# r4dl/StopThePop-Rasterization

Hardware: AMD Instinct MI355X
Metric: fwd+bwd frames/sec at 1920×1080, 1M Gaussians; PSNR vs reference (higher is better)
Workload: dtype f32

## Files before the change

include/stp_raster.h:

```cpp
#ifndef STP_RASTER_H_INCLUDED
#define STP_RASTER_H_INCLUDED

#include <stddef.h>
#include <stdint.h>

#ifdef __cplusplus
extern "C" {
#endif

#define STP_ABI_VERSION 7
#define STP_GRAD_RECORD_FLOATS 16
#define STP_GRAD_RECORD_USED 9
#define STP_GRAD_RECORD_ABS 9
#define STP_GRAD_RECORD_STATS 11
#define STP_GRAD_RECORD_INVDEPTH 14

typedef struct StpSettings {
    int32_t sort_mode;
    int32_t sort_order;
    int32_t queue_tile_4x4;
    int32_t queue_tile_2x2;
    int32_t queue_per_pixel;
    int32_t rect_bounding;
    int32_t tight_opacity_bounding;
    int32_t tile_based_culling;
    int32_t hierarchical_4x4_culling;
    int32_t load_balancing;
    int32_t proper_ewa_scaling;
    int32_t tile_y0;
    int32_t tile_y1;
    int32_t record_blend_log;
    int32_t debug_visualization;
} StpSettings;

#define STP_DEBUG_DISABLED 0
#define STP_DEBUG_DEPTH 1

typedef enum StpStatus {
    STP_OK = 0,
    STP_ERR_INVALID_ARGUMENT = -1,
    STP_ERR_NEEDS_SCALE_ROTATION = -2,
    STP_ERR_QUEUE_SIZE = -3,
    STP_ERR_SORT_MODE = -4,
    STP_ERR_NO_BACKWARD = -5,
    STP_ERR_HIP = -6,
    STP_ERR_ALLOC = -7,
    STP_ERR_PREFILTERED = -8
} StpStatus;

typedef void* (*stp_alloc_fn)(void* user, size_t bytes);

int stp_forward(stp_alloc_fn geometry_alloc, void* geometry_user,
                stp_alloc_fn binning_alloc, void* binning_user,
                stp_alloc_fn image_alloc, void* image_user,
                int P, int D, int M,
                const float* background, int width, int height,
                const StpSettings* settings,
                const float* means3D, const float* shs, const float* colors_precomp,
                const float* opacities, const float* scales, float scale_modifier,
                const float* rotations, const float* cov3D_precomp,
                const float* viewmatrix, const float* projmatrix, const float* inv_viewprojmatrix,
                const float* cam_pos, float tan_fovx, float tan_fovy, int prefiltered,
                float* out_color, int* radii, int debug, void* stream);

void stp_set_forward_split(int tile_row, void* event);

int stp_backward(int P, int D, int M, int R,
                 const float* background, int width, int height,
                 const StpSettings* settings,
                 const float* means3D, const float* shs, const float* opacities, const float* colors_precomp,
                 const float* scales, float scale_modifier, const float* rotations, const float* cov3D_precomp,
                 const float* viewmatrix, const float* projmatrix, const float* inv_viewprojmatrix,
                 const float* cam_pos, float tan_fovx, float tan_fovy,
                 const float* pixel_colors, const int* radii,
                 char* geom_buffer, char* binning_buffer, char* image_buffer,
                 const float* dL_dpix,
                 float* dL_dmean2D , float* grad_records , float* dL_dopacity ,
                 float* dL_dcolor , float* dL_dmean3D , float* dL_dcov3D ,
                 float* dL_dsh , float* dL_dscale , float* dL_drot ,
                 int debug, void* stream);

int stp_backward_phases(int phases, int P, int D, int M, int R,
                        const float* background, int width, int height,
                        const StpSettings* settings,
                        const float* means3D, const float* shs, const float* opacities, const float* colors_precomp,
                        const float* scales, float scale_modifier, const float* rotations, const float* cov3D_precomp,
                        const float* viewmatrix, const float* projmatrix, const float* inv_viewprojmatrix,
                        const float* cam_pos, float tan_fovx, float tan_fovy,
                        const float* pixel_colors, const int* radii,
                        char* geom_buffer, char* binning_buffer, char* image_buffer,
                        const float* dL_dpix,
                        float* dL_dmean2D, float* grad_records, float* dL_dopacity, float* dL_dcolor,
                        float* dL_dmean3D, float* dL_dcov3D, float* dL_dsh, float* dL_dscale, float* dL_drot,
                        int debug, void* stream);

size_t stp_camera_grad_workspace_bytes(int P);
void stp_set_backward_camera_grads(float* dL_dviewmatrix, float* dL_dprojmatrix, float* dL_dcampos, void* workspace, size_t workspace_bytes);

void stp_set_backward_absgrad(float* dL_dmean2D_abs );

void stp_set_backward_blend_stats(float* blend_stats );

void stp_set_forward_background(const float* bg_image , float* out_alpha );
void stp_set_backward_background(const float* bg_image , const float* dL_dalpha ,
                                 float* dL_dbackground );

void stp_set_forward_invdepth(float* out_invdepth );
void stp_set_backward_invdepth(const float* invdepth , const float* dL_dinvdepth );

void stp_set_forward_split_sh(const float* dc );
void stp_set_backward_split_sh(const float* dc , float* dL_ddc );

void stp_set_forward_sh_stash(int enable);

void stp_set_forward_raw_params(int mask);
void stp_set_backward_raw_params(int mask);
int stp_activate_params(int P, const float* scaling, const float* rotation, const float* opacity, float* scales, float* rotations,
                        float* opacities, void* stream);

int stp_mark_visible(int P, const float* means3D, const float* viewmatrix, const float* projmatrix,
                     uint8_t* present, void* stream);

typedef struct { float* param; const float* grad; float* exp_avg; float* exp_avg_sq; long long numel; float lr, eps; } StpAdamTensor;
int stp_sparse_adam(int n_tensors, const StpAdamTensor* tensors, int N, const void* visible, int visible_kind ,
                    float beta1, float beta2, void* stream);

int stp_mcmc_relocation(int n, const float* opacity_old, const float* scale_old, const void* N, int n_kind , int n_max,
                        float* opacity_new, float* scale_new, void* stream);
int stp_mcmc_add_noise(int P, float* xyz, const float* scales, const float* rotations, const float* opacities, const float* noise,
                       float noise_scale, float k, float x0, int raw, void* stream);

typedef struct { float grad_threshold, split_size, min_opacity, max_screen_size, max_world_size, split_shrink; int32_t raw, prune_big; } StpDensifyRule;
typedef struct { const float *param, *exp_avg, *exp_avg_sq; float *param_out, *exp_avg_out, *exp_avg_sq_out; int32_t row; int32_t role; } StpDensifyTensor;
int stp_densify_stats(int P, float* grad_accum, float* denom, float* max_radii2D , const float* grad2d, int grad_stride ,
                      const void* visible, int visible_kind, void* stream);
int stp_densify_plan(int P, const float* grad_accum, const float* denom, const float* scaling, const float* opacity,
                     const float* max_radii2D , const StpDensifyRule* rule, uint8_t* plan, void* stream);
size_t stp_densify_scratch_bytes(int P);
int stp_densify_scan(int P, const uint8_t* plan, void* scratch, size_t scratch_bytes, uint32_t* offsets , int64_t counts[3] , void* stream);
int stp_densify_apply(int P, const uint8_t* plan, const uint32_t* offsets, const int64_t counts[3], int n_tensors, const StpDensifyTensor* tensors,
                      const float* noise , float split_shrink, int raw, void* stream);

#define STP_KNN_BOX 256
size_t stp_knn_scratch_bytes(int P);
int stp_knn_mean_dist2(int P, const float* points , void* scratch, size_t scratch_bytes, float* mean_dist2 , void* stream);

#define STP_PHOTOMETRIC_TILE_W 64
#define STP_PHOTOMETRIC_TILE_H 16
size_t stp_photometric_workspace_floats(int planes, int H, int W);
int stp_photometric_forward(int planes, int H, int W, const float* image, const float* target,
                            float* out2 , float* maps ,
                            float* workspace, void* stream);
int stp_photometric_backward(int planes, int H, int W, const float* image, const float* target, const float* maps,
                             const float* dL_dout2 , float* dL_dimage, void* stream);

size_t stp_geometry_buffer_size(int P, const StpSettings* settings);
size_t stp_geometry_buffer_size_stash(int P, const StpSettings* settings);
size_t stp_binning_buffer_size(int R);
size_t stp_image_buffer_size(int width, int height);
size_t stp_blend_log_bytes(int width, int height);
size_t stp_blend_log_bytes_rows(int width, int height, int tile_y0, int tile_y1);
int stp_blend_log_depth(const void* image_buffer);
void stp_forget_buffer(const void* buffer);
size_t stp_blend_log_bytes_depth(int width, int height, int tile_y0, int tile_y1, int depth);

int stp_geometry_layout(int P, const StpSettings* settings, const char* name, size_t* offset, size_t* count);
int stp_binning_layout(int R, const char* name, size_t* offset, size_t* count);
int stp_binning_layout_count(const void* binning_buffer, int R);
void stp_reset_size_guesses(void);
void stp_set_run_ahead(int mode);
int stp_get_run_ahead(void);
int stp_image_layout(int width, int height, const char* name, size_t* offset, size_t* count);
int stp_image_layout_rows(int width, int height, int tile_y0, int tile_y1, const char* name, size_t* offset, size_t* count);
int stp_image_layout_depth(int width, int height, int tile_y0, int tile_y1, int log_depth, const char* name, size_t* offset, size_t* count);

void stp_timing_enable(int enabled);
int stp_timing_read(float* ms6);
int stp_timing_history(float* ms6, int capacity);
int stp_timing_history_host(float* ms6, int capacity);
size_t stp_timing_text(char* buf, size_t size);

int stp_hbm_probe(int kind, void* dst, const void* src, size_t bytes, int blocks, void* stream);

const char* stp_last_error(void);
int stp_abi_version(void);

#ifdef __cplusplus
}
#endif
#endif
```

stopthepop-rasterization_amd/csrc/host/stp_bind_raster.h:

```cpp
#pragma once

#include <tuple>

#include "stp_scratch_pool.h"
#include "stp_tensor_checks.h"

namespace {
StpSettings settings_from_dict(const py::dict& d, bool record_log)
{
    StpSettings s{};
    const py::dict ss = d["sort_settings"].cast<py::dict>(), cs = d["culling_settings"].cast<py::dict>(), q = ss["queue_sizes"].cast<py::dict>();
    s.sort_mode = ss["sort_mode"].cast<int>();
    s.sort_order = ss["sort_order"].cast<int>();
    s.queue_tile_4x4 = q["tile_4x4"].cast<int>();
    s.queue_tile_2x2 = q["tile_2x2"].cast<int>();
    s.queue_per_pixel = q["per_pixel"].cast<int>();
    s.rect_bounding = cs["rect_bounding"].cast<bool>();
    s.tight_opacity_bounding = cs["tight_opacity_bounding"].cast<bool>();
    s.tile_based_culling = cs["tile_based_culling"].cast<bool>();
    s.hierarchical_4x4_culling = cs["hierarchical_4x4_culling"].cast<bool>();
    s.load_balancing = d["load_balancing"].cast<bool>();
    s.proper_ewa_scaling = d["proper_ewa_scaling"].cast<bool>();
    if (setting_present(d, "_tile_rows")) {
        const py::tuple tr = py::tuple(d["_tile_rows"]);
        s.tile_y0 = tr[0].cast<int>();
        s.tile_y1 = tr[1].cast<int>();
    }
    s.record_blend_log = record_log ? 1 : 0;
    return s;
}

struct FrameInputs { torch::Tensor bg, m3, sh, col, op, sc, ro, c3, vm, pm, inv, cam; };
FrameInputs prep_frame(const torch::Device& dev, const torch::Tensor& background, const torch::Tensor& means3D, const torch::Tensor& sh,
                       const torch::Tensor& colors, const torch::Tensor& opacity, const torch::Tensor& scales, const torch::Tensor& rotations,
                       const torch::Tensor& cov3D_precomp, const torch::Tensor& viewmatrix, const torch::Tensor& projmatrix,
                       const torch::Tensor& inv_viewprojmatrix, const torch::Tensor& campos)
{
    return {prep(background, dev), prep(means3D, dev), prep(sh, dev), prep(colors, dev), prep(opacity, dev), prep(scales, dev), prep(rotations, dev),
            prep(cov3D_precomp, dev), prep(viewmatrix, dev), prep(projmatrix, dev), prep(inv_viewprojmatrix, dev), prep(campos, dev)};
}

bool per_pixel_background(const torch::Tensor& bg, int H, int W)
{
    return bg.defined() && bg.dim() == 3 && bg.size(0) == 3 && bg.size(1) == H && bg.size(2) == W;
}

int split_sh_total(const torch::Tensor& dc, const torch::Tensor& sh, const torch::Tensor& means3D)
{
    const int64_t P = means3D.size(0);
    if (!((dc.dim() == 3 && dc.size(1) == 1 && dc.size(2) == 3) || (dc.dim() == 2 && dc.size(1) == 3)))
        throw std::runtime_error("dc must have dimensions (num_points, 1, 3) or (num_points, 3)");
    if (dc.size(0) != P) throw std::runtime_error("dc must have one row per Gaussian: " + std::to_string(dc.size(0)) + " rows for " + std::to_string(P) + " points");
    if (dc.scalar_type() != torch::kFloat32) throw std::runtime_error("dc must be a float32 tensor");
    if (dc.device() != means3D.device()) throw std::runtime_error("dc must be on the device of means3D");
    if (sh.numel() == 0) return 1;
    if (!(sh.dim() == 3 && sh.size(0) == P && sh.size(2) == 3))
        throw std::runtime_error("with dc, shs is the rest of the coefficients and must have dimensions (num_points, M - 1, 3)");
    if (sh.scalar_type() != torch::kFloat32 || sh.device() != means3D.device()) throw std::runtime_error("with dc, shs must be a float32 tensor on the device of means3D");
    return (int)sh.size(1) + 1;
}

std::tuple<int, torch::Tensor, torch::Tensor, torch::Tensor, torch::Tensor, torch::Tensor, torch::Tensor, torch::Tensor>
rasterize_gaussians(const torch::Tensor& background, const torch::Tensor& means3D, const torch::Tensor& colors, const torch::Tensor& opacity,
                    const torch::Tensor& scales, const torch::Tensor& rotations, const float scale_modifier, const torch::Tensor& cov3D_precomp,
                    const torch::Tensor& viewmatrix, const torch::Tensor& projmatrix, const torch::Tensor& inv_viewprojmatrix, const float tan_fovx,
                    const float tan_fovy, const int image_height, const int image_width, const torch::Tensor& sh, const int degree,
                    const torch::Tensor& campos, const bool prefiltered, const py::dict& settings, const bool render_depth, const bool debug,
                    const bool record_log, const bool alpha, const bool invdepth, const c10::optional<torch::Tensor>& dc, const int raw)
{
    need_library();
    if (raw != 0) require(g_api.set_forward_raw_params, "raw");
    TORCH_CHECK(means3D.dim() == 2 && means3D.size(1) == 3, "means3D must have dimensions (num_points, 3)");
    TORCH_CHECK(means3D.is_cuda(), GPU_ONLY);
    const bool split = dc.has_value() && dc->defined() && colors.numel() == 0;
    if (split) require(g_api.set_forward_split_sh, "dc");
    const int M_split = split ? split_sh_total(*dc, sh, means3D) : 0;
    const torch::Device dev = means3D.device();
    const int P = (int)means3D.size(0), H = image_height, W = image_width;
    const auto fopt = means3D.options().dtype(torch::kFloat32), iopt = means3D.options().dtype(torch::kInt32), bopt = means3D.options().dtype(torch::kByte);
    const bool zero = P == 0 || setting_present(settings, "_tile_rows");
    torch::Tensor out_color = zero ? torch::zeros({3, H, W}, fopt) : torch::empty({3, H, W}, fopt);
    torch::Tensor radii = zero ? torch::zeros({P}, iopt) : torch::empty({P}, iopt);
    const bool bg_pixels = per_pixel_background(background, H, W);
    if (alpha || bg_pixels) require(g_api.set_forward_background, "alpha / background");
    torch::Tensor out_alpha;
    if (alpha) out_alpha = zero ? torch::zeros({1, H, W}, fopt) : torch::empty({1, H, W}, fopt);
    if (invdepth) {
        require(g_api.set_forward_invdepth, "invdepth");
        if (render_depth) throw std::runtime_error("the inverse-depth output is not available with render_depth (the debug depth visualisation)");
    }
    torch::Tensor out_invdepth;
    if (invdepth) out_invdepth = zero ? torch::zeros({1, H, W}, fopt) : torch::empty({1, H, W}, fopt);
    const bool sh_stash = (setting_flag(settings, "_record_blend_log") || setting_flag(settings, "_sh_stash")) && !setting_flag(settings, "_no_sh_stash") &&
                          !render_depth && g_api.set_forward_sh_stash != nullptr;
    Resizer geom{torch::empty({0}, bopt), false, false, 0}, binning{torch::empty({0}, bopt), true, false, 1}, img{torch::empty({0}, bopt), true, false, 2};
    int rendered = 0;
    if (P != 0) {
        const int M = split ? M_split : sh.numel() != 0 ? (int)sh.size(1) : 0;
        StpSettings s = settings_from_dict(settings, record_log);
        if (render_depth) {
            s.debug_visualization = STP_DEBUG_DEPTH;
            s.record_blend_log = 0;
        }
        const FrameInputs in = prep_frame(dev, background, means3D, sh, colors, opacity, scales, rotations, cov3D_precomp, viewmatrix, projmatrix,
                                          inv_viewprojmatrix, campos);
        torch::Tensor dc_;
        if (split) dc_ = prep(*dc, dev);
        const c10::hip::HIPGuard guard(dev.index());
        void* const stream = current_stream(dev);
        int rc;
        {
            py::gil_scoped_release nogil;
            if (alpha || bg_pixels)
                g_api.set_forward_background(bg_pixels ? fptr(in.bg) : nullptr, alpha ? out_alpha.data_ptr<float>() : nullptr);
            if (invdepth) g_api.set_forward_invdepth(out_invdepth.data_ptr<float>());
            if (split) g_api.set_forward_split_sh(dc_.data_ptr<float>());
            if (sh_stash) g_api.set_forward_sh_stash(1);
            if (raw != 0) g_api.set_forward_raw_params(raw);
            rc = g_api.forward(&Resizer::call, &geom, &Resizer::call, &binning, &Resizer::call, &img, P, degree, M, fptr(in.bg), W, H, &s, fptr(in.m3),
                               fptr(in.sh), fptr(in.col), fptr(in.op), fptr(in.sc), scale_modifier, fptr(in.ro), fptr(in.c3), fptr(in.vm), fptr(in.pm),
                               fptr(in.inv), fptr(in.cam), tan_fovx, tan_fovy, prefiltered ? 1 : 0, out_color.data_ptr<float>(), radii.data_ptr<int>(),
                               debug ? 1 : 0, stream);
        }
        rendered = checked(rc);
        remember_storage(geom.t);
        remember_storage(binning.t);
        remember_storage(img.t);
    }
    return std::make_tuple(rendered, out_color, radii, geom.t, binning.t, img.t, out_alpha, out_invdepth);
}

std::vector<torch::Tensor>
rasterize_gaussians_backward(const torch::Tensor& background, const torch::Tensor& means3D, const torch::Tensor& radii, const torch::Tensor& opacities,
                             const torch::Tensor& colors, const torch::Tensor& scales, const torch::Tensor& rotations, const float scale_modifier,
                             const torch::Tensor& cov3D_precomp, const torch::Tensor& viewmatrix, const torch::Tensor& projmatrix,
                             const torch::Tensor& inv_viewprojmatrix, const float tan_fovx, const float tan_fovy, const torch::Tensor& pixel_colors,
                             const torch::Tensor& dL_dout_color, const torch::Tensor& sh, const int degree, const torch::Tensor& campos,
                             const torch::Tensor& geomBuffer, const int R, const torch::Tensor& binningBuffer, const torch::Tensor& imageBuffer,
                             const py::dict& settings, const bool debug, const bool record_log, const int phases, const c10::optional<torch::Tensor>& partial,
                             const c10::optional<std::vector<torch::Tensor>>& outputs, const bool camera_grads, const bool absgrad, const bool blend_stats,
                             const c10::optional<torch::Tensor>& dL_dalpha, const bool bg_grad,
                             const c10::optional<torch::Tensor>& dL_dinvdepth, const c10::optional<torch::Tensor>& invdepth,
                             const c10::optional<torch::Tensor>& dc, const int raw_mask)
{
    need_library();
    TORCH_CHECK(means3D.is_cuda(), GPU_ONLY);
    const int raw = (phases & 2) ? raw_mask : 0;
    if (raw != 0) require(g_api.set_backward_raw_params, "raw");
    const bool split = dc.has_value() && dc->defined() && colors.numel() == 0 && (phases & 2);
    if (split) require(g_api.set_backward_split_sh, "dc");
    const int M_split = split ? split_sh_total(*dc, sh, means3D) : 0;
    if (camera_grads) {
        require(g_api.set_backward_camera_grads, "camera gradients");
        require(g_api.camera_grad_workspace_bytes, "camera gradients");
        TORCH_CHECK(phases & 2, "camera gradients come from the per-Gaussian half (phases bit 1)");
    }
    if (absgrad) {
        require(g_api.set_backward_absgrad, "absgrad");
        TORCH_CHECK((phases & 3) == 3, "absgrad needs both halves of the backward in one call (phases bits 0 and 1)");
    }
    if (blend_stats) {
        require(g_api.set_backward_blend_stats, "blend_stats");
        TORCH_CHECK((phases & 3) == 3, "blend_stats needs both halves of the backward in one call (phases bits 0 and 1)");
    }
    const torch::Device dev = means3D.device();
    const int P = (int)means3D.size(0);
    const int H = (int)dL_dout_color.size(1), W = (int)dL_dout_color.size(2);
    const bool bg_pixels = per_pixel_background(background, H, W);
    const bool have_dalpha = dL_dalpha.has_value() && dL_dalpha->defined();
    if (bg_pixels || have_dalpha || bg_grad) {
        require(g_api.set_backward_background, "alpha / background");
        TORCH_CHECK(phases & 1, "alpha gradient / per-pixel background / background gradient belong to the render half (phases bit 0)");
        TORCH_CHECK(!have_dalpha || dL_dalpha->numel() == (int64_t)H * W, "dL_dalpha must have H * W elements");
    }
    const bool have_dinv = dL_dinvdepth.has_value() && dL_dinvdepth->defined();
    if (have_dinv) {
        require(g_api.set_backward_invdepth, "invdepth");
        TORCH_CHECK((phases & 3) == 3, "the inverse-depth gradient needs both halves of the backward in one call (phases bits 0 and 1)");
        TORCH_CHECK(invdepth.has_value() && invdepth->defined(), "dL_dinvdepth needs the forward's invdepth");
        TORCH_CHECK(dL_dinvdepth->numel() == (int64_t)H * W && invdepth->numel() == (int64_t)H * W, "dL_dinvdepth and invdepth must have H * W elements");
    }
    const int M = split ? M_split : sh.numel() != 0 ? (int)sh.size(1) : 0;
    const auto fopt = means3D.options().dtype(torch::kFloat32);
    const int rec_floats = (phases & 4) ? STP_GRAD_RECORD_USED : STP_GRAD_RECORD_FLOATS;
    const torch::Tensor records = partial.has_value() ? *partial : torch::zeros({P, rec_floats}, fopt);
    TORCH_CHECK(records.dim() == 2 && records.size(0) == P && records.size(1) == rec_floats && records.scalar_type() == torch::kFloat32 &&
                    records.is_contiguous(), "partial must be a contiguous float32 (P,", rec_floats, ") tensor");
    torch::Tensor dL_dmeans2D, dL_dcolors, dL_dopacity, dL_dmeans3D, dL_dcov3D, dL_dsh, dL_dscales, dL_drotations, dL_ddc;
    if ((phases & 2) && outputs.has_value()) {
        TORCH_CHECK(outputs->size() == (split ? 9u : 8u), "outputs: the eight gradient tensors of an earlier chunk (and its dL_ddc behind them with dc)");
        if (split) {
            dL_ddc = (*outputs)[8];
            TORCH_CHECK(dL_ddc.scalar_type() == torch::kFloat32 && dL_ddc.is_contiguous() && dL_ddc.numel() == (int64_t)P * 3 &&
                            (*outputs)[5].is_contiguous() && (*outputs)[5].numel() == (int64_t)P * (M - 1) * 3,
                        "outputs: dL_dsh must be a contiguous (P,M-1,3) and dL_ddc a contiguous (P,3) float32 tensor with dc");
        }
        dL_dmeans2D = (*outputs)[0]; dL_dcolors = (*outputs)[1]; dL_dopacity = (*outputs)[2]; dL_dmeans3D = (*outputs)[3];
        dL_dcov3D = (*outputs)[4]; dL_dsh = (*outputs)[5]; dL_dscales = (*outputs)[6]; dL_drotations = (*outputs)[7];
    } else if (phases & 2) {
        const bool have_scales = scales.numel() != 0, may_omit = g_api.set_forward_sh_stash != nullptr;
        const bool no_dcolors = may_omit && setting_flag(settings, "_no_grad_colors") && colors.numel() == 0;
        const bool no_dcov3D = may_omit && setting_flag(settings, "_no_grad_cov3D") && cov3D_precomp.numel() == 0;
        dL_dmeans2D = torch::empty({P, 3}, fopt); if (!no_dcolors) dL_dcolors = torch::empty({P, 3}, fopt); dL_dopacity = torch::empty({P, 1}, fopt);
        dL_dmeans3D = torch::empty({P, 3}, fopt); if (!no_dcov3D) dL_dcov3D = torch::empty({P, 6}, fopt); dL_dsh = torch::empty({P, split ? M - 1 : M, 3}, fopt);
        if (split) dL_ddc = torch::empty({P, 3}, fopt);
        dL_dscales = have_scales ? torch::empty({P, 3}, fopt) : torch::zeros({P, 3}, fopt);
        dL_drotations = have_scales ? torch::empty({P, 4}, fopt) : torch::zeros({P, 4}, fopt);
    }
    const StpSettings s = settings_from_dict(settings, record_log);
    torch::Tensor dL_dview, dL_dproj, dL_dcam, cam_ws;
    if (camera_grads) {
        dL_dview = torch::empty(viewmatrix.sizes(), fopt); dL_dproj = torch::empty(projmatrix.sizes(), fopt); dL_dcam = torch::empty(campos.sizes(), fopt);
        TORCH_CHECK(dL_dview.numel() == 16 && dL_dproj.numel() == 16 && dL_dcam.numel() == 3, "camera gradients: viewmatrix and projmatrix must have 16 elements, campos 3");
        cam_ws = torch::empty({(int64_t)g_api.camera_grad_workspace_bytes(P)}, means3D.options().dtype(torch::kByte));
    }
    torch::Tensor dL_dmeans2D_abs, stats;
    if (absgrad) dL_dmeans2D_abs = torch::empty({P, 3}, fopt);
    if (blend_stats) stats = torch::empty({P, 3}, fopt);
    torch::Tensor dL_dbg, dal_, bgpix_;
    if (bg_grad) {
        const std::vector<int64_t> shape = bg_pixels ? std::vector<int64_t>{3, H, W} : std::vector<int64_t>{3};
        dL_dbg = (P == 0 || (bg_pixels && setting_present(settings, "_tile_rows"))) ? torch::zeros(shape, fopt) : torch::empty(shape, fopt);
    }
    if (have_dalpha) dal_ = prep(*dL_dalpha, dev);
    if (bg_pixels) bgpix_ = prep(background, dev);
    torch::Tensor dinv_, inv_out_;
    if (have_dinv) { dinv_ = prep(*dL_dinvdepth, dev); inv_out_ = prep(*invdepth, dev); }
    torch::Tensor dc_;
    if (split && P != 0) dc_ = prep(*dc, dev);
    auto make_requests = [&] {
        if ((bg_pixels || have_dalpha || bg_grad) && P != 0)
            g_api.set_backward_background(bg_pixels ? bgpix_.data_ptr<float>() : nullptr, have_dalpha ? dal_.data_ptr<float>() : nullptr,
                                          bg_grad ? dL_dbg.data_ptr<float>() : nullptr);
        if (have_dinv && P != 0) g_api.set_backward_invdepth(inv_out_.data_ptr<float>(), dinv_.data_ptr<float>());
        if (split && P != 0) g_api.set_backward_split_sh(dc_.data_ptr<float>(), dL_ddc.data_ptr<float>());
        if (raw != 0 && P != 0) g_api.set_backward_raw_params(raw);
        if (blend_stats && P != 0) g_api.set_backward_blend_stats(stats.data_ptr<float>());
        if (absgrad && P != 0) g_api.set_backward_absgrad(dL_dmeans2D_abs.data_ptr<float>());
        if (camera_grads) g_api.set_backward_camera_grads(dL_dview.data_ptr<float>(), dL_dproj.data_ptr<float>(), dL_dcam.data_ptr<float>(), cam_ws.data_ptr(), (size_t)cam_ws.numel());
    };
    if (P == 0 && camera_grads) {
        const c10::hip::HIPGuard guard(dev.index());
        void* const stream = current_stream(dev);
        make_requests();
        checked(g_api.backward_phases(phases, 0, degree, M, R, nullptr, W, H, &s, nullptr, nullptr, nullptr, nullptr, nullptr, scale_modifier, nullptr,
                                      nullptr, nullptr, nullptr, nullptr, nullptr, tan_fovx, tan_fovy, nullptr, nullptr, nullptr, nullptr, nullptr,
                                      nullptr, nullptr, nullptr, nullptr, nullptr, nullptr, nullptr, nullptr, nullptr, nullptr, debug ? 1 : 0, stream));
    }
    if (P != 0) {
        const FrameInputs in = prep_frame(dev, background, means3D, sh, colors, opacities, scales, rotations, cov3D_precomp, viewmatrix, projmatrix,
                                          inv_viewprojmatrix, campos);
        const torch::Tensor pix_ = prep(pixel_colors, dev), dl_ = prep(dL_dout_color, dev);
        const torch::Tensor radii_ = radii.contiguous();
        auto optf = [](const torch::Tensor& t) -> float* { return t.defined() && t.numel() != 0 ? t.data_ptr<float>() : nullptr; };
        auto optb = [](const torch::Tensor& t) -> char* { return t.defined() && t.numel() != 0 ? reinterpret_cast<char*>(t.data_ptr()) : nullptr; };
        const c10::hip::HIPGuard guard(dev.index());
        void* const stream = current_stream(dev);
        forget_unless_same_storage(geomBuffer);
        forget_unless_same_storage(binningBuffer);
        forget_unless_same_storage(imageBuffer);
        make_requests();
        checked(g_api.backward_phases(phases, P, degree, M, R, fptr(in.bg), W, H, &s, fptr(in.m3), fptr(in.sh), fptr(in.op), fptr(in.col), fptr(in.sc),
                                      scale_modifier, fptr(in.ro), fptr(in.c3), fptr(in.vm), fptr(in.pm), fptr(in.inv), fptr(in.cam), tan_fovx, tan_fovy,
                                      fptr(pix_), radii_.numel() ? radii_.data_ptr<int>() : nullptr, optb(geomBuffer), optb(binningBuffer),
                                      optb(imageBuffer), fptr(dl_), optf(dL_dmeans2D), records.data_ptr<float>(), optf(dL_dopacity), optf(dL_dcolors),
                                      optf(dL_dmeans3D), optf(dL_dcov3D), optf(dL_dsh), optf(dL_dscales), optf(dL_drotations), debug ? 1 : 0, stream));
    }
    if ((phases & 3) == 1) { if (bg_grad) return {records, dL_dbg}; return {records}; }
    std::vector<torch::Tensor> result{dL_dmeans2D, dL_dcolors, dL_dopacity, dL_dmeans3D, dL_dcov3D, dL_dsh, dL_dscales, dL_drotations};
    if (camera_grads) result.insert(result.end(), {dL_dview, dL_dproj, dL_dcam});
    if (absgrad) result.push_back(dL_dmeans2D_abs);
    if (blend_stats) result.push_back(stats);
    if (bg_grad) result.push_back(dL_dbg);
    if (split) result.push_back(dL_ddc);
    return result;
}

torch::Tensor mark_visible(const torch::Tensor& means3D, const torch::Tensor& viewmatrix, const torch::Tensor& projmatrix)
{
    need_library();
    TORCH_CHECK(means3D.is_cuda(), GPU_ONLY);
    const torch::Device dev = means3D.device();
    const int P = (int)means3D.size(0);
    torch::Tensor present = torch::zeros({P}, means3D.options().dtype(torch::kBool));
    if (P != 0) {
        const torch::Tensor m3_ = prep(means3D, dev), vm_ = prep(viewmatrix, dev), pm_ = prep(projmatrix, dev);
        const c10::hip::HIPGuard guard(dev.index());
        checked(g_api.mark_visible(P, fptr(m3_), fptr(vm_), fptr(pm_), reinterpret_cast<uint8_t*>(present.data_ptr()), current_stream(dev)));
    }
    return present;
}
}
```

stopthepop-rasterization_amd/csrc/host/stp_exports.h:

```cpp
#pragma once

#include <dlfcn.h>

#include <cstddef>
#include <cstring>
#include <stdexcept>
#include <string>

#include "../../../include/stp_raster.h"

#define STP_CORE "the C ABI of include/stp_raster.h"
#define STP_EXPORTS(X)                                                                     \
    X(forward, true, STP_CORE)                                                             \
    X(backward_phases, true, STP_CORE)                                                     \
    X(mark_visible, true, STP_CORE)                                                        \
    X(last_error, true, STP_CORE)                                                          \
    X(abi_version, true, STP_CORE)                                                         \
    X(forget_buffer, true, STP_CORE)                                                       \
    X(set_forward_split, true, STP_CORE)                                                   \
    X(camera_grad_workspace_bytes, false, "camera gradients")                              \
    X(set_backward_camera_grads, false, "camera gradients")                                \
    X(set_backward_absgrad, false, "absgrad")                                              \
    X(set_backward_blend_stats, false, "blend statistics")                                 \
    X(set_forward_background, false, "the alpha output and per-pixel background")          \
    X(set_backward_background, false, "the alpha output and per-pixel background")         \
    X(set_forward_invdepth, false, "the inverse-depth output")                             \
    X(set_backward_invdepth, false, "the inverse-depth output")                            \
    X(set_forward_split_sh, false, "split SH inputs")                                      \
    X(set_backward_split_sh, false, "split SH inputs")                                     \
    X(set_forward_raw_params, false, "raw parameter inputs")                               \
    X(set_backward_raw_params, false, "raw parameter inputs")                              \
    X(activate_params, false, "raw parameter inputs")                                      \
    X(set_forward_sh_stash, false, "the SH stash")  \
    X(sparse_adam, false, "the sparse Adam step")                                          \
    X(mcmc_relocation, false, "the 3DGS-MCMC kernels")                                     \
    X(mcmc_add_noise, false, "the 3DGS-MCMC kernels")                                      \
    X(knn_scratch_bytes, false, "the nearest-neighbour kernels")                           \
    X(knn_mean_dist2, false, "the nearest-neighbour kernels")                              \
    X(densify_stats, false, "the densification kernels")                                   \
    X(densify_plan, false, "the densification kernels")                                    \
    X(densify_scratch_bytes, false, "the densification kernels")                           \
    X(densify_scan, false, "the densification kernels")                                    \
    X(densify_apply, false, "the densification kernels")                                   \
    X(photometric_workspace_floats, false, "the photometric loss")                         \
    X(photometric_forward, false, "the photometric loss")                                  \
    X(photometric_backward, false, "the photometric loss")

namespace {
struct Api {
    void* handle = nullptr;
#define X(name, required, feature) decltype(&stp_##name) name = nullptr;
    STP_EXPORTS(X)
#undef X
} g_api;

struct Export { const char* symbol; bool required; const char* feature; size_t slot; };
const Export g_exports[] = {
#define X(name, required, feature) {"stp_" #name, required, feature, offsetof(Api, name)},
    STP_EXPORTS(X)
#undef X
};

[[noreturn]] void raise_missing(const Export& e, const std::string& who)
{
    throw std::runtime_error(who + ": the loaded libstp_raster.so does not export " + e.symbol + " (a library built before " + e.feature + "): rebuild it");
}

template <class F> void require(const F& fn, const char* who)
{
    if (fn) return;
    const size_t slot = reinterpret_cast<const char*>(&fn) - reinterpret_cast<const char*>(&g_api);
    for (const Export& e : g_exports)
        if (e.slot == slot) raise_missing(e, who);
    throw std::logic_error(std::string(who) + ": require() takes a member of g_api");
}

int load_library(const std::string& path)
{
    void* h = dlopen(path.c_str(), RTLD_NOW | RTLD_LOCAL);
    if (!h) throw std::runtime_error(std::string("cannot load ") + path + ": " + dlerror());
    Api a;
    a.handle = h;
    for (const Export& e : g_exports) {
        void* fn = dlsym(h, e.symbol);
        if (!fn && e.required) raise_missing(e, path);
        std::memcpy(reinterpret_cast<char*>(&a) + e.slot, &fn, sizeof fn);
    }
    if (a.abi_version() != STP_ABI_VERSION) throw std::runtime_error(path + ": ABI version mismatch");
    g_api = a;
    return a.abi_version();
}

void need_library()
{
    if (!g_api.forward) throw std::runtime_error("libstp_raster.so is not loaded (diff_gaussian_rasterization._C._load() does it); there is no CPU fallback");
}

[[noreturn]] void raise_last(int rc)
{
    const char* msg = g_api.last_error();
    throw std::runtime_error((msg && *msg) ? std::string(msg) : "libstp_raster error " + std::to_string(rc));
}
}
```

stopthepop-rasterization_amd/csrc/stp_api.hip:

```cpp
#include "stp_internal.h"

#include <mutex>
#include <string>
#include <utility>

namespace stp {

static thread_local std::string g_last_error;

int fail(int code, const std::string& msg) { g_last_error = msg; return code; }
int fail_hip(hipError_t e, const char* what) { return fail(STP_ERR_HIP, std::string(what) + ": " + hipGetErrorString(e)); }

int check_settings(const StpSettings& s, bool backward)
{
    if (s.sort_mode < MODE_GLOBAL || s.sort_mode > MODE_HIER) return fail(STP_ERR_SORT_MODE, "invalid sort mode");
    if (s.sort_order < ORDER_Z || s.sort_order > ORDER_PTD_MAX) return fail(STP_ERR_SORT_MODE, "invalid sort order");
    if (backward && s.sort_mode == MODE_FULL) return fail(STP_ERR_NO_BACKWARD, "Backward not supported for full per-pixel sort");
    if (s.sort_mode == MODE_HIER) {
        const int h = s.queue_per_pixel, m = s.queue_tile_2x2;
        if (!(m == 8 || m == 12 || m == 20)) return fail(STP_ERR_QUEUE_SIZE, "Not supported mid queue size");
        const bool head_ok = backward ? (h == 4 || h == 8 || h == 12 || h == 16) : (h == 4 || h == 8 || h == 16);
        if (!head_ok) return fail(STP_ERR_QUEUE_SIZE, "Not supported head queue size");
    }
    return 0;
}

void fill_frame(FrameParams& f, int P, int D, int M, const float* background, int width, int height, const StpSettings& s,
                const float* means3D, const float* shs, const float* colors_precomp, const float* opacities,
                const float* scales, float scale_modifier, const float* rotations, const float* cov3D_precomp,
                const float* viewmatrix, const float* projmatrix, const float* inv_viewprojmatrix, const float* cam_pos,
                float tan_fovx, float tan_fovy, int prefiltered)
{
    f.P = P; f.D = D; f.M = M; f.W = width; f.H = height;
    f.gx = (width + TILE - 1) / TILE; f.gy = (height + TILE - 1) / TILE;
    f.ty0 = s.tile_y0; f.ty1 = s.tile_y1;
    clamp_tile_rows(height, f.ty0, f.ty1);
    f.focal_y = (float)height / (2.0f * tan_fovy);
    f.focal_x = (float)width / (2.0f * tan_fovx);
    f.tan_fovx = tan_fovx; f.tan_fovy = tan_fovy; f.scale_modifier = scale_modifier; f.s = s;
    f.background = background; f.means3D = means3D; f.shs = shs; f.colors_precomp = colors_precomp; f.opacities = opacities;
    f.scales = scales; f.rotations = rotations; f.cov3D_precomp = cov3D_precomp; f.viewmatrix = viewmatrix; f.projmatrix = projmatrix;
    f.inv_viewprojmatrix = inv_viewprojmatrix; f.cam_pos = cam_pos; f.prefiltered = prefiltered;
    f.wild_cov = 1;
    f.log_depth = 0; f.log_need = nullptr; f.log_tag = 0;
}

int check_raw_params(int mask, const float* opacities, const float* scales, const float* rotations)
{
    if (mask < 0 || mask > 7) return fail(STP_ERR_INVALID_ARGUMENT, "raw parameters: mask " + std::to_string(mask) + " is outside 0..7 (bit 0 opacities, bit 1 scales, bit 2 rotations)");
    if ((mask & 1) && !opacities) return fail(STP_ERR_INVALID_ARGUMENT, "raw parameters: bit 0 (opacities) is set but opacities is NULL");
    if ((mask & 2) && !scales) return fail(STP_ERR_INVALID_ARGUMENT, "raw parameters: bit 1 (scales) is set but scales is NULL");
    if ((mask & 4) && !rotations) return fail(STP_ERR_INVALID_ARGUMENT, "raw parameters: bit 2 (rotations) is set but rotations is NULL");
    return 0;
}

struct BackwardBackground { const float* bg_image = nullptr; const float* dL_dalpha = nullptr; float* dL_dbackground = nullptr; };
struct BackwardInvdepth { const float* invdepth = nullptr; const float* dL_dinvdepth = nullptr; };
struct BackwardSplitSh { const float* dc = nullptr; float* dL_ddc = nullptr; };
struct BackwardRequests { CameraGradRequest cam; float* absgrad = nullptr; float* blend_stats = nullptr; BackwardBackground background; BackwardInvdepth invdepth; BackwardSplitSh split_sh; int raw_params = 0;  };
struct PendingRequests { ForwardRequests forward; BackwardRequests backward; };
static thread_local PendingRequests t_pending;

ForwardRequests take_forward_requests() { return std::exchange(t_pending.forward, ForwardRequests{}); }
static BackwardRequests take_backward_requests(int phases)
{
    BackwardRequests& p = t_pending.backward;
    BackwardRequests r;
    if (phases & 2) { r.cam = std::exchange(p.cam, CameraGradRequest{}); r.split_sh = std::exchange(p.split_sh, BackwardSplitSh{}); r.raw_params = std::exchange(p.raw_params, 0); }
    r.absgrad = std::exchange(p.absgrad, nullptr); r.blend_stats = std::exchange(p.blend_stats, nullptr);
    r.invdepth = std::exchange(p.invdepth, BackwardInvdepth{});
    if (phases & 1) r.background = std::exchange(p.background, BackwardBackground{});
    return r;
}
static void keep_for_per_gaussian_call(const BackwardRequests& r)
{
    t_pending.backward.absgrad = r.absgrad; t_pending.backward.blend_stats = r.blend_stats; t_pending.backward.invdepth = r.invdepth;
}

}

using namespace stp;

extern "C" {

int stp_abi_version(void) { return STP_ABI_VERSION; }
const char* stp_last_error(void) { return g_last_error.c_str(); }

void stp_set_forward_split(int tile_row, void* event) { t_pending.forward.split = ForwardSplit{tile_row, (hipEvent_t)event, event != nullptr}; }
void stp_set_forward_background(const float* bg_image, float* out_alpha) { t_pending.forward.background = ForwardBackground{bg_image, out_alpha}; }
size_t stp_camera_grad_workspace_bytes(int P) { return camera_grad_workspace_bytes(P); }
void stp_set_backward_camera_grads(float* dL_dviewmatrix, float* dL_dprojmatrix, float* dL_dcampos, void* workspace, size_t workspace_bytes)
{
    t_pending.backward.cam = CameraGradRequest{};
    if (!dL_dviewmatrix || !dL_dprojmatrix || !dL_dcampos) return;
    t_pending.backward.cam = CameraGradRequest{dL_dviewmatrix, dL_dprojmatrix, dL_dcampos, workspace, workspace_bytes};
}
void stp_set_backward_absgrad(float* dL_dmean2D_abs) { t_pending.backward.absgrad = dL_dmean2D_abs; }
void stp_set_backward_blend_stats(float* blend_stats) { t_pending.backward.blend_stats = blend_stats; }
void stp_set_backward_background(const float* bg_image, const float* dL_dalpha, float* dL_dbackground) { t_pending.backward.background = BackwardBackground{bg_image, dL_dalpha, dL_dbackground}; }
void stp_set_forward_invdepth(float* out_invdepth) { t_pending.forward.out_invdepth = out_invdepth; }
void stp_set_backward_invdepth(const float* invdepth, const float* dL_dinvdepth) { t_pending.backward.invdepth = BackwardInvdepth{invdepth, dL_dinvdepth}; }
void stp_set_forward_split_sh(const float* dc) { t_pending.forward.sh_dc = dc; }
void stp_set_forward_sh_stash(int enable) { t_pending.forward.sh_stash = enable != 0; }
void stp_set_backward_split_sh(const float* dc, float* dL_ddc) { t_pending.backward.split_sh = dc ? BackwardSplitSh{dc, dL_ddc} : BackwardSplitSh{}; }
void stp_set_forward_raw_params(int mask) { t_pending.forward.raw_params = mask; }
void stp_set_backward_raw_params(int mask) { t_pending.backward.raw_params = mask; }

namespace {
constexpr int BG_RING = 8;
struct BackgroundSlot { float* partials = nullptr; hipEvent_t done = nullptr; bool used = false; };
struct BackgroundScratch { BackgroundSlot slot[BG_RING]; unsigned next = 0; bool ready = false; };
BackgroundScratch g_background_scratch[MAX_DEVICES];
std::mutex g_background_mutex;
int acquire_background_scratch(BackgroundSlot** out, hipStream_t st)
{
    int device = 0;
    if (hipGetDevice(&device) != hipSuccess || device < 0 || device >= MAX_DEVICES) return fail(STP_ERR_HIP, "hipGetDevice failed");
    BackgroundScratch& r = g_background_scratch[device];
    if (!r.ready) {
        const size_t bytes = background_grad_partials() * sizeof(float);
        char* base = nullptr;
        if (hipMalloc(reinterpret_cast<void**>(&base), bytes * BG_RING) != hipSuccess) return fail(STP_ERR_HIP, "cannot create the background-gradient scratch");
        for (int i = 0; i < BG_RING; i++) {
            r.slot[i].partials = reinterpret_cast<float*>(base + bytes * i);
            if (hipEventCreateWithFlags(&r.slot[i].done, hipEventDisableTiming) != hipSuccess) { (void)hipFree(base); return fail(STP_ERR_HIP, "cannot create the background-gradient scratch"); }
        }
        r.ready = true;
    }
    BackgroundSlot& s = r.slot[r.next++ % BG_RING];
    if (s.used) STP_TRY(hipStreamWaitEvent(st, s.done, 0), "wait for the background-gradient scratch");
    *out = &s;
    return 0;
}
}

int stp_backward_phases(int phases, int P, int D, int M, int R, const float* background, int width, int height, const StpSettings* settings,
                 const float* means3D, const float* shs, const float* opacities, const float* colors_precomp, const float* scales,
                 float scale_modifier, const float* rotations, const float* cov3D_precomp, const float* viewmatrix,
                 const float* projmatrix, const float* inv_viewprojmatrix, const float* cam_pos, float tan_fovx, float tan_fovy,
                 const float* pixel_colors, const int* radii, char* geom_buffer, char* binning_buffer, char* image_buffer,
                 const float* dL_dpix, float* dL_dmean2D, float* grad_records, float* dL_dopacity, float* dL_dcolor,
                 float* dL_dmean3D, float* dL_dcov3D, float* dL_dsh, float* dL_dscale, float* dL_drot, int debug, void* stream)
{
    hipStream_t st = (hipStream_t)stream;
    const BackwardRequests req = take_backward_requests(phases);
    const CameraGradRequest& cam = req.cam;
    float* const absgrad = req.absgrad;
    float* const blend_stats = req.blend_stats;
    const BackwardBackground& bbg = req.background;
    if (absgrad) {
        if (phases & 4)
            return fail(STP_ERR_INVALID_ARGUMENT, "absgrad is not available with compact gradient records (phases bit 2): the 36-byte record has no room for the two extra sums");
        if (((phases >> 8) & 0xFF) > 1)
            return fail(STP_ERR_INVALID_ARGUMENT, "absgrad is not available from a chunked per-Gaussian half (phases bits 8-23)");
    }
    if (blend_stats) {
        if (phases & 4)
            return fail(STP_ERR_INVALID_ARGUMENT, "blend statistics are not available with compact gradient records (phases bit 2): the 36-byte record has no room for the three extra terms");
        if (((phases >> 8) & 0xFF) > 1)
            return fail(STP_ERR_INVALID_ARGUMENT, "blend statistics are not available from a chunked per-Gaussian half (phases bits 8-23)");
    }
    const BackwardInvdepth& binv = req.invdepth;
    if (binv.invdepth || binv.dL_dinvdepth) {
        if (!binv.invdepth || !binv.dL_dinvdepth)
            return fail(STP_ERR_INVALID_ARGUMENT, "inverse depth: the forward's invdepth and dL_dinvdepth must both be given");
        if (phases & 4)
            return fail(STP_ERR_INVALID_ARGUMENT, "the inverse-depth gradient is not available with compact gradient records (phases bit 2): the 36-byte record has no room for the extra sum");
        if (((phases >> 8) & 0xFF) > 1)
            return fail(STP_ERR_INVALID_ARGUMENT, "the inverse-depth gradient is not available from a chunked per-Gaussian half (phases bits 8-23)");
    }
    const BackwardSplitSh& bsh = req.split_sh;
    if (bsh.dc && colors_precomp) shs = nullptr;
    if (bsh.dc && !colors_precomp) {
        if (!bsh.dL_ddc) return fail(STP_ERR_INVALID_ARGUMENT, "split SH: dL_ddc must be given with dc");
        if (M > 1 && (!shs || !dL_dsh)) return fail(STP_ERR_INVALID_ARGUMENT, "split SH: M > 1 needs the rest of the coefficients (shs) and their gradient (dL_dsh)");
    }
    if (cam.dL_dview) {
        if (!cam.workspace || (reinterpret_cast<uintptr_t>(cam.workspace) & 15) != 0 || cam.workspace_bytes < camera_grad_workspace_bytes(P))
            return fail(STP_ERR_INVALID_ARGUMENT, "camera gradients: the workspace is null, not 16-byte aligned or smaller than stp_camera_grad_workspace_bytes(P)");
        if (((phases >> 8) & 0xFF) > 1)
            return fail(STP_ERR_INVALID_ARGUMENT, "camera gradients are not available from a chunked per-Gaussian half (phases bits 8-23)");
    }
    if (int rc = check_raw_params(req.raw_params, opacities, scales, rotations)) return rc;
    if (!settings) return fail(STP_ERR_INVALID_ARGUMENT, "null settings");
    if (P == 0) {
        if (cam.dL_dview) STP_TRY(launch_camera_grad_finalize(0, cam, st), "camera gradient launch");
        if (bbg.dL_dbackground && (!bbg.bg_image || (width > 0 && height > 0)))
            STP_TRY(hipMemsetAsync(bbg.dL_dbackground, 0, sizeof(float) * 3 * (bbg.bg_image ? (size_t)width * (size_t)height : (size_t)1), st), "background gradient fill");
        return 0;
    }
    if (int rc = check_settings(*settings, true)) return rc;
    if (!geom_buffer || !image_buffer || (R > 0 && !binning_buffer)) return fail(STP_ERR_INVALID_ARGUMENT, "null scratch buffer");
    if (!grad_records) return fail(STP_ERR_INVALID_ARGUMENT, "null gradient record buffer");
    if ((phases & 1) && (!dL_dpix || !pixel_colors)) return fail(STP_ERR_INVALID_ARGUMENT, "null image gradient");
    if ((phases & 2) && (!dL_dmean2D || !dL_dopacity || !dL_dmean3D || !dL_dscale || !dL_drot))
        return fail(STP_ERR_INVALID_ARGUMENT, "null gradient buffer");

    FrameParams f;
    fill_frame(f, P, D, M, background, width, height, *settings, means3D, shs, colors_precomp, opacities, scales, scale_modifier,
               rotations, cov3D_precomp, viewmatrix, projmatrix, inv_viewprojmatrix, cam_pos, tan_fovx, tan_fovy, 0);
    const bool with_inv = requires_depth_along_ray(*settings);
    bool with_stash = false;
    if ((phases & 2) && !colors_precomp && (shs || bsh.dc) && M > 0) { if (int rc = stash_of(geom_buffer, P, (int64_t)R, &with_stash, (hipStream_t)stream, true)) return rc; }
    float* sh_stash = nullptr;
    GeometryState g = carve_geometry(geom_buffer, (size_t)P, with_inv, nullptr, nullptr, nullptr, with_stash ? &sh_stash : nullptr);
    uint32_t bin_cap = 0, log_depth = 0;
    if (R > 0) { if (int rc = layout_of(binning_buffer, (uint32_t)R, &bin_cap, (hipStream_t)stream, true)) return rc; }
    if (uses_blend_log(*settings)) { if (int rc = log_depth_of(image_buffer, (int64_t)R, &log_depth, (hipStream_t)stream, true)) return rc; }
    BinningState b = carve_binning(binning_buffer, (size_t)bin_cap, nullptr);
    ImageState img = carve_image(image_buffer, width, height, f.ty0, f.ty1, (int)log_depth, nullptr);
    if (!radii) radii = g.internal_radii;

    BackwardParams bw;
    bw.cam = cam;
    bw.absgrad = absgrad;
    bw.blend_stats = blend_stats;
    bw.bg_image = bbg.bg_image; bw.dL_dalpha = bbg.dL_dalpha; bw.dL_dbackground = bbg.dL_dbackground;
    bw.invdepth = binv.invdepth; bw.dL_dinvdepth = binv.dL_dinvdepth;
    bw.sh_stash = sh_stash;
    if (bsh.dc && !colors_precomp) { f.sh_dc = bsh.dc; bw.dL_ddc = bsh.dL_ddc; }
    f.raw_params = req.raw_params;
    bw.pixel_colors = pixel_colors; bw.dL_dpix = dL_dpix; bw.dL_dmean2D = dL_dmean2D; bw.grad_rec = grad_records;
    bw.grad_stride = (phases & 4) ? STP_GRAD_RECORD_USED : STP_GRAD_RECORD_FLOATS;
    bw.clear_rec = (phases & 8) ? 1 : 0;
    bw.chunks = (phases >> 8) & 0xFF; bw.chunk = (phases >> 16) & 0xFF;
    if (bw.chunks > 1 && (bw.chunk >= bw.chunks || (phases & 1))) return fail(STP_ERR_INVALID_ARGUMENT, "chunked per-Gaussian half: chunk index out of range, or combined with the render half");
    bw.dL_dopacity = dL_dopacity; bw.dL_dcolor = dL_dcolor; bw.dL_dmean3D = dL_dmean3D; bw.dL_dcov3D = dL_dcov3D; bw.dL_dsh = dL_dsh;
    bw.dL_dscale = dL_dscale; bw.dL_drot = dL_drot;

    std::unique_lock<std::mutex> bg_lock;
    BackgroundSlot* bg_slot = nullptr;
    if ((phases & 1) && bw.dL_dbackground && !bw.bg_image) {
        bg_lock = std::unique_lock<std::mutex>(g_background_mutex);
        if (int rc = acquire_background_scratch(&bg_slot, st)) return rc;
    }
    if (phases & 1) {
        timer_begin_backward();
        timer_mark(5, st);
        std::string err;
        hipError_t e = launch_render_backward(f, g, b, img, bw, st, &err);
        if (e != hipSuccess) {
            if (!err.empty()) return fail(settings->sort_mode == MODE_FULL ? STP_ERR_NO_BACKWARD : STP_ERR_QUEUE_SIZE, err);
            return fail_hip(e, "backward render launch");
        }
        STP_DEBUG_SYNC("backward render");
        if (bw.dL_dbackground) {
            STP_TRY(launch_background_grad(f, img, bw, bg_slot ? bg_slot->partials : nullptr, st), "background gradient launch");
            if (bg_slot) {
                bg_slot->used = hipEventRecord(bg_slot->done, st) == hipSuccess;
                if (!bg_slot->used) STP_TRY(hipStreamSynchronize(st), "synchronize behind the background gradient");
                bg_lock.unlock();
            }
            STP_DEBUG_SYNC("background gradient");
        }
        timer_mark(6, st);
    }
    if (phases & 2) {
        if (!(phases & 1)) timer_mark(6, st);
        STP_TRY(launch_preprocess_backward(f, g, radii, bw, st), "backward preprocess launch");
        STP_DEBUG_SYNC("backward preprocess");
        timer_mark(7, st);
    }
    if (!(phases & 2)) keep_for_per_gaussian_call(req);
    return 0;
}

int stp_backward(int P, int D, int M, int R, const float* background, int width, int height, const StpSettings* settings,
                 const float* means3D, const float* shs, const float* opacities, const float* colors_precomp, const float* scales,
                 float scale_modifier, const float* rotations, const float* cov3D_precomp, const float* viewmatrix,
                 const float* projmatrix, const float* inv_viewprojmatrix, const float* cam_pos, float tan_fovx, float tan_fovy,
                 const float* pixel_colors, const int* radii, char* geom_buffer, char* binning_buffer, char* image_buffer,
                 const float* dL_dpix, float* dL_dmean2D, float* grad_records, float* dL_dopacity, float* dL_dcolor,
                 float* dL_dmean3D, float* dL_dcov3D, float* dL_dsh, float* dL_dscale, float* dL_drot, int debug, void* stream)
{
    return stp_backward_phases(3, P, D, M, R, background, width, height, settings, means3D, shs, opacities, colors_precomp, scales,
                               scale_modifier, rotations, cov3D_precomp, viewmatrix, projmatrix, inv_viewprojmatrix, cam_pos, tan_fovx,
                               tan_fovy, pixel_colors, radii, geom_buffer, binning_buffer, image_buffer, dL_dpix, dL_dmean2D, grad_records,
                               dL_dopacity, dL_dcolor, dL_dmean3D, dL_dcov3D, dL_dsh, dL_dscale, dL_drot, debug, stream);
}

int stp_activate_params(int P, const float* scaling, const float* rotation, const float* opacity, float* scales, float* rotations, float* opacities,
                        void* stream)
{
    if (P < 0) return fail(STP_ERR_INVALID_ARGUMENT, "stp_activate_params: negative P");
    if (P >= (1 << 29)) return fail(STP_ERR_INVALID_ARGUMENT, "stp_activate_params: P must be below 2^29");
    if (!scaling != !scales || !rotation != !rotations || !opacity != !opacities)
        return fail(STP_ERR_INVALID_ARGUMENT, "stp_activate_params: an input and its output must be given, or be NULL, together");
    if (P == 0) return 0;
    hipError_t e = hipSuccess;
    const int launches = launch_activate_params(P, scaling, rotation, opacity, scales, rotations, opacities, (hipStream_t)stream, &e);
    if (e != hipSuccess) return fail_hip(e, "activate_params launch");
    return launches;
}

int stp_mark_visible(int P, const float* means3D, const float* viewmatrix, const float* projmatrix, uint8_t* present, void* stream)
{
    (void)projmatrix;
    if (P == 0) return 0;
    if (!means3D || !viewmatrix || !present) return fail(STP_ERR_INVALID_ARGUMENT, "null input");
    STP_TRY(launch_mark_visible(P, means3D, viewmatrix, present, (hipStream_t)stream), "mark_visible launch");
    return 0;
}

int stp_sparse_adam(int n_tensors, const StpAdamTensor* tensors, int N, const void* visible, int visible_kind, float beta1, float beta2, void* stream)
{
    if (n_tensors < 0 || N < 0) return fail(STP_ERR_INVALID_ARGUMENT, "stp_sparse_adam: negative count");
    if (visible_kind != 0 && visible_kind != 1)
        return fail(STP_ERR_INVALID_ARGUMENT, "stp_sparse_adam: unknown visible_kind " + std::to_string(visible_kind) + " (0: N bytes, 1: N int32 radii)");
    if (n_tensors > 0 && !tensors) return fail(STP_ERR_INVALID_ARGUMENT, "stp_sparse_adam: null tensor table");
    bool any = false;
    for (int k = 0; k < n_tensors; k++) {
        const StpAdamTensor& t = tensors[k];
        const std::string which = "stp_sparse_adam: tensor " + std::to_string(k);
        if (t.numel < 0) return fail(STP_ERR_INVALID_ARGUMENT, which + ": negative numel");
        if (t.numel >= (1ll << 31)) return fail(STP_ERR_INVALID_ARGUMENT, which + ": numel " + std::to_string(t.numel) + " >= 2^31");
        if (t.numel == 0) continue;
        if (N == 0 || t.numel % N != 0)
            return fail(STP_ERR_INVALID_ARGUMENT, which + ": numel " + std::to_string(t.numel) + " is not a multiple of N = " + std::to_string(N));
        if (!t.param || !t.grad || !t.exp_avg || !t.exp_avg_sq) return fail(STP_ERR_INVALID_ARGUMENT, which + ": null pointer");
        any = true;
    }
    if (!any) return 0;
    if (!visible) return fail(STP_ERR_INVALID_ARGUMENT, "stp_sparse_adam: null visible");
    hipError_t e;
    const int launches = launch_sparse_adam(n_tensors, tensors, N, visible, visible_kind, beta1, beta2, (hipStream_t)stream, &e);
    if (e != hipSuccess) return fail_hip(e, "sparse_adam launch");
    return launches;
}

int stp_mcmc_relocation(int n, const float* opacity_old, const float* scale_old, const void* N, int n_kind, int n_max, float* opacity_new,
                        float* scale_new, void* stream)
{
    if (n < 0) return fail(STP_ERR_INVALID_ARGUMENT, "stp_mcmc_relocation: negative n");
    if (n_kind != 0 && n_kind != 1)
        return fail(STP_ERR_INVALID_ARGUMENT, "stp_mcmc_relocation: unknown n_kind " + std::to_string(n_kind) + " (0: int32, 1: int64)");
    if (n_max < 2 || n_max > 51)
        return fail(STP_ERR_INVALID_ARGUMENT, "stp_mcmc_relocation: n_max " + std::to_string(n_max) + " outside [2, 51] (N is clamped to [1, n_max - 1])");
    if (n == 0) return 0;
    if (!opacity_old || !scale_old || !N || !opacity_new || !scale_new) return fail(STP_ERR_INVALID_ARGUMENT, "stp_mcmc_relocation: null pointer");
    hipError_t e;
    const int launches = launch_mcmc_relocation(n, opacity_old, scale_old, N, n_kind, n_max, opacity_new, scale_new, (hipStream_t)stream, &e);
    if (e != hipSuccess) return fail_hip(e, "mcmc_relocation launch");
    return launches;
}

int stp_mcmc_add_noise(int P, float* xyz, const float* scales, const float* rotations, const float* opacities, const float* noise, float noise_scale,
                       float k, float x0, int raw, void* stream)
{
    if (P < 0) return fail(STP_ERR_INVALID_ARGUMENT, "stp_mcmc_add_noise: negative P");
    if (raw != 0 && raw != 1) return fail(STP_ERR_INVALID_ARGUMENT, "stp_mcmc_add_noise: raw must be 0 or 1, got " + std::to_string(raw));
    if (P == 0) return 0;
    if (!xyz || !scales || !rotations || !opacities || !noise) return fail(STP_ERR_INVALID_ARGUMENT, "stp_mcmc_add_noise: null pointer");
    hipError_t e;
    const int launches = launch_mcmc_add_noise(P, xyz, scales, rotations, opacities, noise, noise_scale, k, x0, raw, (hipStream_t)stream, &e);
    if (e != hipSuccess) return fail_hip(e, "mcmc_add_noise launch");
    return launches;
}

size_t stp_knn_scratch_bytes(int P) { return knn_scratch_bytes(P); }

int stp_knn_mean_dist2(int P, const float* points, void* scratch, size_t scratch_bytes, float* mean_dist2, void* stream)
{
    if (P < 0) return fail(STP_ERR_INVALID_ARGUMENT, "stp_knn_mean_dist2: negative P");
    if (P == 0) return 0;
    if (P < 4)
        return fail(STP_ERR_INVALID_ARGUMENT, "stp_knn_mean_dist2: P = " + std::to_string(P) + ": the mean over three neighbours needs at least 4 points");
    if (!points || !scratch || !mean_dist2) return fail(STP_ERR_INVALID_ARGUMENT, "stp_knn_mean_dist2: null pointer");
    const size_t need = knn_scratch_bytes(P);
    if (scratch_bytes < need)
        return fail(STP_ERR_INVALID_ARGUMENT, "stp_knn_mean_dist2: scratch of " + std::to_string(scratch_bytes) + " bytes, stp_knn_scratch_bytes(P) = " + std::to_string(need));
    if (reinterpret_cast<uintptr_t>(scratch) & 15u) return fail(STP_ERR_INVALID_ARGUMENT, "stp_knn_mean_dist2: scratch is not 16-byte aligned");
    hipError_t e;
    const int launches = launch_knn_mean_dist2(P, points, scratch, mean_dist2, (hipStream_t)stream, &e);
    if (e != hipSuccess) return fail_hip(e, "knn_mean_dist2");
    return launches;
}

static int check_densify_P(const char* who, int P)
{
    if (P < 0) return fail(STP_ERR_INVALID_ARGUMENT, std::string(who) + ": negative P");
    if (3ll * P >= (1ll << 31)) return fail(STP_ERR_INVALID_ARGUMENT, std::string(who) + ": 3 P = " + std::to_string(3ll * P) + " >= 2^31");
    return 0;
}

int stp_densify_stats(int P, float* grad_accum, float* denom, float* max_radii2D, const float* grad2d, int grad_stride, const void* visible,
                      int visible_kind, void* stream)
{
    if (const int rc = check_densify_P("stp_densify_stats", P)) return rc;
    if (grad_stride != 2 && grad_stride != 3)
        return fail(STP_ERR_INVALID_ARGUMENT, "stp_densify_stats: grad_stride must be 2 or 3, got " + std::to_string(grad_stride));
    if (visible_kind != 0 && visible_kind != 1)
        return fail(STP_ERR_INVALID_ARGUMENT, "stp_densify_stats: unknown visible_kind " + std::to_string(visible_kind) + " (0: P bytes, 1: P int32 radii)");
    if (max_radii2D && visible_kind == 0)
        return fail(STP_ERR_INVALID_ARGUMENT, "stp_densify_stats: max_radii2D needs the radii (visible_kind 1): bytes hold no radius to read");
    if (P == 0) return 0;
    if (!grad_accum || !denom || !grad2d || !visible) return fail(STP_ERR_INVALID_ARGUMENT, "stp_densify_stats: null pointer");
    hipError_t e;
    const int launches = launch_densify_stats(P, grad_accum, denom, max_radii2D, grad2d, grad_stride, visible, visible_kind, (hipStream_t)stream, &e);
    if (e != hipSuccess) return fail_hip(e, "densify_stats launch");
    return launches;
}

int stp_densify_plan(int P, const float* grad_accum, const float* denom, const float* scaling, const float* opacity, const float* max_radii2D,
                     const StpDensifyRule* rule, uint8_t* plan, void* stream)
{
    if (const int rc = check_densify_P("stp_densify_plan", P)) return rc;
    if (!rule) return fail(STP_ERR_INVALID_ARGUMENT, "stp_densify_plan: null rule");
    if (P == 0) return 0;
// ... 119 lines not shown
```

stopthepop-rasterization_amd/csrc/stp_forward.hip:

```cpp
#include "stp_internal.h"

#include <atomic>
#include <cstring>
#include <mutex>
#include <string>

using namespace stp;

namespace {
struct Mailbox { volatile uint32_t* host = nullptr; uint32_t* dev = nullptr; hipEvent_t ev = nullptr; hipEvent_t done = nullptr; int device = 0; uint32_t ticket = 0; };
constexpr int MAILBOX_RING = 8;
struct MailboxRing { Mailbox slot[MAILBOX_RING]; std::atomic<unsigned> next{0}; std::atomic<bool> ready{false};
                     uint32_t* log_need = nullptr;  };
MailboxRing g_mailboxes[MAX_DEVICES];
std::mutex g_mailbox_mutex;
constexpr int GUESS_SLOTS = 16;
struct SizeGuess { std::atomic<uint64_t> key{0}; std::atomic<uint32_t> R{0}; std::atomic<uint32_t> log_need{0}; };
SizeGuess g_guess[MAX_DEVICES][GUESS_SLOTS];
uint64_t guess_key(const FrameParams& f)
{
    uint64_t k = 0x9E3779B97F4A7C15ull;
    for (uint64_t v : {(uint64_t)f.P, (uint64_t)f.W, (uint64_t)f.H, (uint64_t)f.ty0, (uint64_t)f.ty1, (uint64_t)f.s.sort_mode,
                       (uint64_t)(f.s.tile_based_culling * 8 + f.s.rect_bounding * 4 + f.s.tight_opacity_bounding * 2 + (f.s.sort_order == ORDER_PTD_MAX))})
        k = (k ^ v) * 0xBF58476D1CE4E5B9ull, k ^= k >> 29;
    return k | 1ull;
}

struct SideStream { hipStream_t stream = nullptr; std::atomic<bool> ready{false}; };
SideStream g_side[MAX_DEVICES];
SideStream* side_stream(int device)
{
    if (!switches().side_stream || device < 0 || device >= MAX_DEVICES) return nullptr;
    SideStream& s = g_side[device];
    if (!s.ready.load(std::memory_order_acquire)) {
        std::lock_guard<std::mutex> lock(g_mailbox_mutex);
        if (!s.ready.load(std::memory_order_relaxed)) {
            if (hipStreamCreateWithFlags(&s.stream, hipStreamNonBlocking) != hipSuccess) { (void)hipGetLastError(); return nullptr; }
            s.ready.store(true, std::memory_order_release);
        }
    }
    return &s;
}
struct SideJoin {
    hipEvent_t done; hipStream_t st; bool pending;
    hipError_t join() { if (!pending) return hipSuccess; pending = false; return hipStreamWaitEvent(st, done, 0); }
    ~SideJoin() { (void)join(); }
};

inline void cpu_relax()
{
#if defined(__x86_64__) || defined(__i386__)
    __builtin_ia32_pause();
#elif defined(__aarch64__)
    asm volatile("yield" ::: "memory");
#else
    std::atomic_signal_fence(std::memory_order_seq_cst);
#endif
}

constexpr uint32_t RUN_AHEAD_AUTO_MAX = 1u << 18;
std::atomic<int> g_run_ahead{[] { const char* e = std::getenv("STP_RUN_AHEAD"); return (e && (e[0] == '0' || e[0] == '1')) ? e[0] - '0' : 2; }()};

int log_depth_for(const SizeGuess& slot, uint64_t key)
{
    const int fixed = switches().fixed_log_depth;
    if (fixed > 0) return blend_log_clamp_depth((fixed + 1) & ~1);
    const uint32_t need = slot.key.load(std::memory_order_acquire) == key ? slot.log_need.load(std::memory_order_relaxed) : 0u;
    if (need == 0) return blend_log_default_depth();
    return blend_log_clamp_depth((int)((need + need / 8 + 4 + 15) & ~15u));
}

int acquire_mailbox(Mailbox* out)
{
    int device = 0;
    if (hipGetDevice(&device) != hipSuccess || device < 0 || device >= MAX_DEVICES) return fail(STP_ERR_HIP, "hipGetDevice failed");
    MailboxRing& ring = g_mailboxes[device];
    if (!ring.ready.load(std::memory_order_acquire)) {
        std::lock_guard<std::mutex> lock(g_mailbox_mutex);
        if (!ring.ready.load(std::memory_order_relaxed)) {
            for (int i = 0; i < MAILBOX_RING; i++) {
                void* h = nullptr; void* d = nullptr;
                if (hipHostMalloc(&h, 64, hipHostMallocMapped | hipHostMallocCoherent) != hipSuccess || hipHostGetDevicePointer(&d, h, 0) != hipSuccess ||
                    hipEventCreateWithFlags(&ring.slot[i].ev, hipEventDisableTiming) != hipSuccess ||
                    hipEventCreateWithFlags(&ring.slot[i].done, hipEventDisableTiming) != hipSuccess)
                    return fail(STP_ERR_HIP, "cannot create the num_rendered mailbox");
                std::memset(h, 0, 64);
                ring.slot[i].host = static_cast<volatile uint32_t*>(h);
                ring.slot[i].dev = static_cast<uint32_t*>(d);
                ring.slot[i].device = device;
            }
            if (hipMalloc(reinterpret_cast<void**>(&ring.log_need), sizeof(uint32_t) * 64) != hipSuccess || hipMemset(ring.log_need, 0, sizeof(uint32_t) * 64) != hipSuccess)
                return fail(STP_ERR_HIP, "cannot create the blend-log depth words");
            ring.ready.store(true, std::memory_order_release);
        }
    }
    const unsigned seq = ring.next.fetch_add(1u);
    *out = ring.slot[seq % MAILBOX_RING];
    out->ticket = seq + 1u == 0u ? 1u : seq + 1u;
    return 0;
}

struct ForwardCall {
    const hipStream_t st; const int debug;
    FrameParams f;
    GeometryState g{}; ImageState img{}; char* img_ptr = nullptr; char* geom_base = nullptr; float* sh_stash = nullptr;
    Mailbox mb;
    SizeGuess* gslot = nullptr; uint64_t gkey = 0;
    uint32_t* log_need_word = nullptr; uint32_t log_tag = 0; int log_depth = 0; bool with_log = false;
    SideStream* side = nullptr;
    bool colour_started = true;
    char* bin_ptr = nullptr; size_t bin_have = 0;
    uint32_t cap = 0; bool ahead = false, run_ahead = false;
    int* radii; float* const out_color;
    struct Split { const ForwardSplit s; hipStream_t st; bool recorded; ~Split() { if (s.armed && !recorded) (void)hipEventRecord(s.event, st); } } split;
    SideJoin colours;

    ForwardCall(hipStream_t stream, int debug_, const ForwardSplit& split_, int* radii_, float* out_color_)
        : st(stream), debug(debug_), radii(radii_), out_color(out_color_), split{split_, stream, false}, colours{nullptr, stream, false} {}
    int carve_geometry_and_image(stp_alloc_fn geometry_alloc, void* geometry_user, stp_alloc_fn image_alloc, void* image_user, bool with_inv, bool with_stash);
    int launch_up_to_mailbox(); int colour_on_side();
    int request_binning(stp_alloc_fn binning_alloc, void* binning_user);
    int wait_mailbox(); int read_mailbox(int* R_out, bool* wild_out);
    int binning_and_render(const GeometryState& gd, const BinningState& b, int L, uint32_t dup_cap);
};

int ForwardCall::carve_geometry_and_image(stp_alloc_fn geometry_alloc, void* geometry_user, stp_alloc_fn image_alloc, void* image_user, bool with_inv, bool with_stash)
{
    size_t geom_bytes = 0;
    carve_geometry(nullptr, (size_t)f.P, with_inv, &geom_bytes, nullptr, nullptr, with_stash ? &sh_stash : nullptr);
    char* geom_ptr = (char*)geometry_alloc(geometry_user, geom_bytes);
    if (!geom_ptr) return fail(STP_ERR_ALLOC, "geometry allocator returned NULL");
    g = carve_geometry(geom_ptr, (size_t)f.P, with_inv, nullptr, nullptr, nullptr, with_stash ? &sh_stash : nullptr);
    geom_base = geom_ptr;
    if (!radii) radii = g.internal_radii;

    if (int rc = acquire_mailbox(&mb)) return rc;
    colours.done = mb.done;
    gkey = guess_key(f);
    const unsigned gidx = (unsigned)((gkey >> 1) % GUESS_SLOTS);
    gslot = &g_guess[mb.device][gidx];
    log_need_word = g_mailboxes[mb.device].log_need + gidx;
    size_t img_bytes = 0;
    with_log = uses_blend_log(f.s);
    log_depth = with_log ? log_depth_for(*gslot, gkey) : 0;
    f.log_depth = log_depth;
    f.log_need = with_log ? log_need_word : nullptr;
    log_tag = (uint32_t)((gkey >> 40) & 0xFFFFu) | 1u;
    f.log_tag = log_tag;
    carve_image(nullptr, f.W, f.H, f.ty0, f.ty1, log_depth, &img_bytes);
    img_ptr = (char*)image_alloc(image_user, img_bytes);
    if (!img_ptr) return fail(STP_ERR_ALLOC, "image allocator returned NULL");
    img = carve_image(img_ptr, f.W, f.H, f.ty0, f.ty1, log_depth, nullptr);
    return 0;
}

int ForwardCall::launch_up_to_mailbox()
{
    const bool atomic_bin = switches().atomic_bin, two_level_scan = switches().two_level_scan;
    timer_begin_forward();
    timer_mark(0, st);
    STP_TRY(launch_frame_init(g, img, f.gx * f.ty0, f.gx * (f.ty1 - f.ty0), with_log, atomic_bin, st), "frame init launch");
    STP_TRY(launch_preprocess(f, g, radii, atomic_bin ? img.tile_counts : nullptr, st), "preprocess launch");
    STP_DEBUG_SYNC("preprocess");
    if (!two_level_scan) STP_TRY(launch_scan(f, g, st), "inclusive scan");
    STP_DEBUG_SYNC("scan");
    if (atomic_bin) STP_TRY(launch_tile_scan(f, img, st), "tile scan");

    if (two_level_scan) STP_TRY(launch_block_prefix_mailbox(f, g, mb.dev, mb.ticket, log_need_word, st), "workgroup prefixes + mailbox launch");
    else STP_TRY(launch_mailbox(g.point_offsets + (f.P - 1), g.status + 1, mb.dev, mb.ticket, log_need_word, st), "mailbox launch");
    STP_TRY(hipEventRecord(mb.ev, st), "record mailbox event");
    side = side_stream(mb.device);
    colour_started = !(side && switches().colour_late);
    if (side) {
        if (colour_started) { if (int rc = colour_on_side()) return rc; }
    } else STP_TRY(launch_sh_color(f, g, radii, sh_stash, st), "SH colour launch");
    return 0;
}

int ForwardCall::colour_on_side()
{
    STP_TRY(hipStreamWaitEvent(side->stream, mb.ev, 0), "side stream wait");
    STP_TRY(launch_sh_color(f, g, radii, sh_stash, side->stream), "SH colour launch");
    if (hipError_t e = hipEventRecord(mb.done, side->stream); e != hipSuccess) {
        (void)hipStreamSynchronize(side->stream);
        return fail_hip(e, "record colour event");
    }
    colours.pending = true;
    return 0;
}

int ForwardCall::request_binning(stp_alloc_fn binning_alloc, void* binning_user)
{
    const Switches& sw = switches();
    const int run_ahead_mode = g_run_ahead.load(std::memory_order_relaxed);
    run_ahead = run_ahead_mode != 0;
    const uint32_t guess = (sw.speculative_binning && gslot->key.load(std::memory_order_acquire) == gkey) ? gslot->R.load(std::memory_order_relaxed) : 0u;
    ahead = run_ahead && guess > 0 && (run_ahead_mode == 1 || guess < RUN_AHEAD_AUTO_MAX) && sw.two_level_scan && !sw.atomic_bin && !debug;
    cap = guess + guess / 8 + (ahead ? 1024u : 0u);
    if (guess > 0) {
        carve_binning(nullptr, (size_t)cap, &bin_have);
        bin_ptr = (char*)binning_alloc(binning_user, bin_have);
        if (!bin_ptr) return fail(STP_ERR_ALLOC, "binning allocator returned NULL");
    }
    return 0;
}

int ForwardCall::wait_mailbox()
{
    const bool mbx_spin = switches().mailbox_spin;
    if (mbx_spin) {
        for (unsigned it = 1;; it++) {
            if (mb.host[2] == mb.ticket) break;
            if ((it & 255u) == 0u) {
                const hipError_t q = hipEventQuery(mb.ev);
                if (q == hipSuccess) break;
                if (q != hipErrorNotReady) return fail_hip(q, "query (num_rendered)");
                if (it > (1u << 22)) { STP_TRY(hipEventSynchronize(mb.ev), "synchronize (num_rendered)"); break; }
            }
            cpu_relax();
        }
        std::atomic_thread_fence(std::memory_order_acquire);
    } else STP_TRY(hipEventSynchronize(mb.ev), "synchronize (num_rendered)");
    return 0;
}

int ForwardCall::read_mailbox(int* R_out, bool* wild_out)
{
    if (int rc = wait_mailbox()) return rc;
    const uint32_t host_status[2] = {mb.host[0], mb.host[1]};
    const uint32_t word = mb.host[3];
    if (const uint32_t reported = (word >> 16) == log_tag ? (word & 0xFFFFu) : 0u) {
        const uint32_t known = gslot->key.load(std::memory_order_acquire) == gkey ? gslot->log_need.load(std::memory_order_relaxed) : 0u;
        const uint32_t keep = known - known / 32;
        gslot->log_need.store(reported > keep ? reported : keep, std::memory_order_relaxed);
    } else if (gslot->key.load(std::memory_order_acquire) != gkey) gslot->log_need.store(0u, std::memory_order_relaxed);
    if (host_status[1] & 1u) return fail(STP_ERR_PREFILTERED, "Point is filtered although prefiltered is set. This shouldn't happen!");
    *wild_out = (host_status[1] & 2u) != 0;
    *R_out = (int)host_status[0];
    const uint32_t prev = gslot->key.load(std::memory_order_acquire) == gkey ? gslot->R.load(std::memory_order_relaxed) : 0u;
    const uint32_t keep = run_ahead ? prev - prev / 32 : 0u;
    gslot->R.store((uint32_t)*R_out > keep ? (uint32_t)*R_out : keep, std::memory_order_relaxed);
    gslot->key.store(gkey, std::memory_order_release);
    return 0;
}

int ForwardCall::binning_and_render(const GeometryState& gd, const BinningState& b, int L, uint32_t dup_cap)
{
    const bool atomic_bin = switches().atomic_bin, tile_local_sort = switches().tile_local_sort;
    uint32_t* zero_ptr = nullptr; size_t zero_words = 0;
    if (!atomic_bin && tile_local_sort) sort_zero_region(b, (size_t)L, (uint32_t)(f.gx * f.gy), &zero_ptr, &zero_words);
    STP_TRY(launch_duplicate(f, gd, radii, b, atomic_bin ? img.tile_cursor : nullptr, dup_cap, (uint32_t)L, zero_ptr, zero_words, st), "duplicate launch");
    STP_DEBUG_SYNC("duplicate");
    timer_mark(2, st);
    if (!colour_started) {
        STP_TRY(hipEventRecord(mb.ev, st), "record event behind duplicate");
        if (int rc = colour_on_side()) return rc;
        colour_started = true;
    }
    if (atomic_bin) {
        STP_TRY(launch_bin_pad(b, img, L, st), "pad entries");
    } else {
        STP_TRY(launch_sort(f, b, L, tile_local_sort, zero_words != 0, st), "radix sort");
        STP_DEBUG_SYNC("sort");
        STP_TRY(launch_ranges(f, b, img, L, st), "tile ranges");
        STP_DEBUG_SYNC("ranges");
    }
    const bool order_wanted = !atomic_bin && tile_order_used(f);
#ifdef STP_ORDER_MAIN
    const bool order_on_side = false;
#else
    const bool order_on_side = order_wanted && side != nullptr && gather_order_mode() == 0 && f.gx * (f.ty1 - f.ty0) >= 16384;
#endif
    if (order_on_side) {
        STP_TRY(hipEventRecord(mb.ev, st), "record event behind the ranges");
        STP_TRY(hipStreamWaitEvent(side->stream, mb.ev, 0), "side stream wait (ranges)");
        STP_TRY(launch_tile_order(f, img, side->stream), "tile order");
    } else if (order_wanted) STP_TRY(launch_tile_order(f, img, st), "tile order");
    STP_TRY(colours.join(), "join colour stream");
    SideJoin ordering{mb.done, st, false};
    if (order_on_side) {
        if (hipError_t e = hipEventRecord(mb.done, side->stream); e != hipSuccess) {
            (void)hipStreamSynchronize(side->stream);
            return fail_hip(e, "record tile-order event");
        }
        ordering.pending = true;
    }
    if (tile_local_sort) STP_TRY(launch_tile_sort_gather(f, g, b, img, L, atomic_bin, st), "tile sort + entry gather");
    else STP_TRY(launch_gather_entries(f, g, b, L, st), "entry gather");
    STP_DEBUG_SYNC("entry gather");
    STP_TRY(ordering.join(), "join tile order");
    timer_mark(3, st);
    std::string err;
    hipError_t e;
    if (split.s.armed && split.s.row > f.ty0 && split.s.row < f.ty1 && f.s.debug_visualization == 0) {
        FrameParams f1 = f, f2 = f;
        f1.ty1 = split.s.row; f2.ty0 = split.s.row;
        f1.split_launch = f2.split_launch = 1;
        e = launch_render_forward(f1, g, b, img, out_color, st, &err);
        if (e == hipSuccess) { e = hipEventRecord(split.s.event, st); split.recorded = e == hipSuccess; }
        if (e == hipSuccess) e = launch_render_forward(f2, g, b, img, out_color, st, &err);
    } else e = launch_render_forward(f, g, b, img, out_color, st, &err);
    if (e != hipSuccess) {
        if (!err.empty()) return fail(STP_ERR_QUEUE_SIZE, err);
        return fail_hip(e, "render launch");
    }
    STP_DEBUG_SYNC("render");
    STP_TRY(launch_render_debug_finish(f, img, out_color, st), "debug visualisation");
    timer_mark(4, st);
    return 0;
}
}

extern "C" {

void stp_set_run_ahead(int mode) { g_run_ahead.store(mode < 0 ? 0 : (mode > 2 ? 2 : mode), std::memory_order_relaxed); }
int stp_get_run_ahead(void) { return g_run_ahead.load(std::memory_order_relaxed); }
void stp_reset_size_guesses(void)
{
    for (auto& dev : g_guess)
        for (auto& slot : dev) { slot.key.store(0, std::memory_order_release); slot.R.store(0u, std::memory_order_relaxed); slot.log_need.store(0u, std::memory_order_relaxed); }
    int cur = 0;
    if (hipGetDevice(&cur) != hipSuccess) return;
    for (int d = 0; d < MAX_DEVICES; d++)
        if (g_mailboxes[d].ready.load(std::memory_order_acquire) && g_mailboxes[d].log_need && hipSetDevice(d) == hipSuccess) {
            (void)hipDeviceSynchronize();
            (void)hipMemset(g_mailboxes[d].log_need, 0, sizeof(uint32_t) * 64);
        }
    (void)hipSetDevice(cur);
}

int stp_forward(stp_alloc_fn geometry_alloc, void* geometry_user, stp_alloc_fn binning_alloc, void* binning_user,
                stp_alloc_fn image_alloc, void* image_user, int P, int D, int M, const float* background, int width, int height,
                const StpSettings* settings, const float* means3D, const float* shs, const float* colors_precomp,
                const float* opacities, const float* scales, float scale_modifier, const float* rotations,
                const float* cov3D_precomp, const float* viewmatrix, const float* projmatrix, const float* inv_viewprojmatrix,
                const float* cam_pos, float tan_fovx, float tan_fovy, int prefiltered, float* out_color, int* radii, int debug,
                void* stream)
{
    const ForwardRequests req = take_forward_requests();
    ForwardCall c((hipStream_t)stream, debug, req.split, radii, out_color);
    const ForwardBackground& fbg = req.background;
    if (!settings || !geometry_alloc || !binning_alloc || !image_alloc) return fail(STP_ERR_INVALID_ARGUMENT, "null settings or allocator");
    if (P < 0 || width <= 0 || height <= 0) return fail(STP_ERR_INVALID_ARGUMENT, "bad sizes");
    if (P == 0) return 0;
    if (!means3D || !opacities || !background || !viewmatrix || !projmatrix || !inv_viewprojmatrix || !cam_pos || !out_color)
        return fail(STP_ERR_INVALID_ARGUMENT, "null required input");
    if (int rc = check_settings(*settings, false)) return rc;
    if ((fbg.bg_image || fbg.out_alpha) && settings->debug_visualization == STP_DEBUG_DEPTH)
        return fail(STP_ERR_INVALID_ARGUMENT, "alpha output / per-pixel background (stp_set_forward_background) are not available with the debug depth visualisation: its image is not C + T * background");
    if (req.out_invdepth && settings->debug_visualization == STP_DEBUG_DEPTH)
        return fail(STP_ERR_INVALID_ARGUMENT, "the inverse-depth output (stp_set_forward_invdepth) is not available with the debug depth visualisation");
    if (int rc = check_raw_params(req.raw_params, opacities, scales, rotations)) return rc;
    const float* const sh_dc = colors_precomp ? nullptr : req.sh_dc;
    if (sh_dc && M > 1 && !shs) return fail(STP_ERR_INVALID_ARGUMENT, "split SH (stp_set_forward_split_sh): M > 1 needs the rest of the coefficients in shs");
    if (!colors_precomp && !shs && !sh_dc) return fail(STP_ERR_INVALID_ARGUMENT, "neither SHs nor precomputed colours given");
    if (!cov3D_precomp && !(scales && rotations)) return fail(STP_ERR_INVALID_ARGUMENT, "neither scale/rotation nor precomputed covariance given");
    const bool with_inv = requires_depth_along_ray(*settings);
    if (with_inv && !(scales && rotations)) return fail(STP_ERR_NEEDS_SCALE_ROTATION, "sorted modes need scales and rotations");

    FrameParams& f = c.f;
    fill_frame(f, P, D, M, background, width, height, *settings, means3D, shs, colors_precomp, opacities, scales, scale_modifier,
               rotations, cov3D_precomp, viewmatrix, projmatrix, inv_viewprojmatrix, cam_pos, tan_fovx, tan_fovy, prefiltered);
    f.out_invdepth = req.out_invdepth;
    f.sh_dc = sh_dc;
    f.raw_params = req.raw_params;
    f.bg_image = fbg.bg_image; f.out_alpha = fbg.out_alpha;
    const bool with_stash = req.sh_stash && !colors_precomp && (shs || sh_dc) && M > 0;
    if (int rc = c.carve_geometry_and_image(geometry_alloc, geometry_user, image_alloc, image_user, with_inv, with_stash)) return rc;

    const Switches& sw = switches();
    f.fused_gather = sw.fused_gather && sw.tile_local_sort && !sw.atomic_bin && f.s.sort_mode == MODE_HIER && f.s.debug_visualization != STP_DEBUG_DEPTH ? 1 : 0;
    if (!sw.two_level_scan) { c.g.block_sums = nullptr; c.g.block_prefix = nullptr; }

    if (int rc = c.launch_up_to_mailbox()) return rc;
    if (int rc = c.request_binning(binning_alloc, binning_user)) return rc;

    const hipStream_t st = c.st;
    int R = 0;
    bool wild = false;
    GeometryState g_dup = c.g;
    if (c.ahead) {
        f.wild_cov = 0;
        timer_mark(1, st);
        const BinningState b = carve_binning(c.bin_ptr, (size_t)c.cap, nullptr);
        if (int rc = c.binning_and_render(g_dup, b, (int)c.cap, c.cap)) return rc;
        if (int rc = c.read_mailbox(&R, &wild)) return rc;
        if ((uint32_t)R <= c.cap && !wild) {
            remember_stash(c.geom_base, with_stash, R);
            remember_layout(c.bin_ptr, c.cap, R);
            remember_log_depth(c.img_ptr, (uint32_t)c.log_depth, R);
            return R;
        }
        g_dup.block_prefix = nullptr; g_dup.block_sums = nullptr;
        STP_TRY(launch_frame_init(c.g, c.img, f.gx * f.ty0, f.gx * (f.ty1 - f.ty0), c.with_log, sw.atomic_bin, st), "frame init launch");
        STP_TRY(launch_stash_mark(f, c.g, c.sh_stash, st), "stash mark launch");
    } else {
        if (int rc = c.read_mailbox(&R, &wild)) return rc;
        STP_DEBUG_SYNC("SH colour");
        timer_mark(1, st);
    }
    f.wild_cov = wild ? 1 : 0;
    size_t bin_bytes = 0;
    carve_binning(nullptr, (size_t)R, &bin_bytes);
    if (bin_bytes > c.bin_have) {
        c.bin_ptr = (char*)binning_alloc(binning_user, bin_bytes);
        if (!c.bin_ptr) return fail(STP_ERR_ALLOC, "binning allocator returned NULL");
    }
    const BinningState b = carve_binning(c.bin_ptr, (size_t)R, nullptr);
    if (int rc = c.binning_and_render(g_dup, b, R, 0xFFFFFFFFu)) return rc;
    remember_stash(c.geom_base, with_stash, R);
    if (c.bin_ptr) remember_layout(c.bin_ptr, (uint32_t)R, R);
    remember_log_depth(c.img_ptr, (uint32_t)c.log_depth, R);
    return R;
}
}
```

stopthepop-rasterization_amd/csrc/stp_internal.h:

```cpp
#pragma once

#include <hip/hip_runtime.h>
#include <cstdint>
#include <cstddef>
#include <cstdlib>
#include <string>

#include "../../include/stp_raster.h"
#include "stp_switches.h"

namespace stp {

constexpr int TILE = 16;
constexpr size_t ALIGN = 256;
static_assert(ALIGN == 256, "Switches::carve_skew (stp_switches.h) is masked to a multiple of 256");
constexpr int MAX_DEVICES = 32;

enum SortMode { MODE_GLOBAL = 0, MODE_FULL = 1, MODE_KBUFFER = 2, MODE_HIER = 3 };
enum SortOrder { ORDER_Z = 0, ORDER_DISTANCE = 1, ORDER_PTD_CENTER = 2, ORDER_PTD_MAX = 3 };

inline bool uses_blend_log(const StpSettings& s)
{
    return s.record_blend_log != 0 && s.debug_visualization == 0 && (s.sort_mode == MODE_HIER || s.sort_mode == MODE_KBUFFER);
}

inline int subtile_mask_kind(const StpSettings& s)
{
    if (s.sort_mode == MODE_HIER && s.hierarchical_4x4_culling) return 1;
    return s.sort_mode == MODE_KBUFFER ? 2 : 0;
}

inline bool requires_depth_along_ray(const StpSettings& s)
{
    return s.sort_mode != MODE_GLOBAL || s.sort_order == ORDER_PTD_CENTER || s.sort_order == ORDER_PTD_MAX;
}

struct Carver {
    char* base;
    size_t off = 0;
    explicit Carver(char* b) : base(b) {}
    static size_t skew() { return switches().carve_skew; }
    template <typename T> T* take(size_t count, size_t* off_out = nullptr)
    {
        off = (off + ALIGN - 1) & ~(ALIGN - 1);
        if (off) off += skew();
        if (off_out) *off_out = off;
        T* p = base ? reinterpret_cast<T*>(base + off) : nullptr;
        off += count * sizeof(T);
        return p;
    }
    size_t total() const { return ((off + ALIGN - 1) & ~(ALIGN - 1)) + ALIGN; }
};

struct GeometryState {
    uint32_t* status;
    float* depths;
    uint8_t* clamped;
    int32_t* internal_radii;
    float2* rects2D;
    float2* means2D;
    float* cov3D;
    float4* cov3D_inv;
    float4* gpack;
    float4* conic_opacity;
    float* rgb;
    uint32_t* tiles_touched;
    uint32_t* point_offsets;
    uint32_t* block_sums;
    uint32_t* block_prefix;
    char* scan_temp;
    size_t scan_temp_bytes;
    float* invz;
};
constexpr int STP_STASH_WORD = 8;
constexpr uint32_t STP_HEADER_MAGIC_STASH = 0x53505453u;

struct ImageState {
    float* final_T;
    uint32_t* n_contrib;
    uint2* ranges;
    uint32_t* dbg_minmax;
    uint32_t* tile_counts;
    uint32_t* tile_cursor;
    uint32_t* bin_total;
    uint32_t* header;
    uint32_t* tile_flags;
    uint32_t* blend_log;
    int log_depth;
};

struct BinningState {
    uint32_t* header;
    uint32_t* point_list;
    uint32_t* point_list_unsorted;
    uint64_t* keys;
    uint64_t* keys_unsorted;
    char* sort_temp;
    size_t sort_temp_bytes;
    float4* entA;
    float4* entB;
    float4* entC;
    float4* entD;
    float4* entF;
};

constexpr uint32_t STP_HEADER_MAGIC_BINNING = 0x42505453u, STP_HEADER_MAGIC_IMAGE = 0x49505453u;
struct NamedOffset { const char* name; size_t offset; size_t count; };

GeometryState carve_geometry(char* base, size_t P, bool with_inv, size_t* total, NamedOffset* names = nullptr, int* n_names = nullptr, float** sh_stash = nullptr);
ImageState carve_image(char* base, int W, int H, int ty0, int ty1, int log_depth , size_t* total, NamedOffset* names = nullptr, int* n_names = nullptr);
BinningState carve_binning(char* base, size_t R, size_t* total, NamedOffset* names = nullptr, int* n_names = nullptr);
void clamp_tile_rows(int height, int& y0, int& y1);

int fail(int code, const std::string& msg);
int fail_hip(hipError_t e, const char* what);
#define STP_TRY(expr, what) do { hipError_t _e = (expr); if (_e != hipSuccess) return fail_hip(_e, what); } while (0)
#define STP_DEBUG_SYNC(what)  STP_TRY(debug ? hipStreamSynchronize(st) : hipSuccess, what)

void timer_begin_forward();
void timer_begin_backward();
void timer_mark(int i, hipStream_t st);

void remember_layout(const void* binning, uint32_t count, int64_t R);
void remember_stash(const void* geometry, bool stash, int64_t R);
int stash_of(const char* geometry, int P, int64_t R, bool* stash, hipStream_t st, bool have_stream);
void remember_log_depth(const void* image, uint32_t depth, int64_t R);
int layout_of(const char* binning, uint32_t R, uint32_t* cap, hipStream_t st = nullptr, bool have_stream = false);
int log_depth_of(const char* image, int64_t R, uint32_t* depth, hipStream_t st = nullptr, bool have_stream = false);

int blend_log_rows(int depth);
int blend_log_default_depth();
int blend_log_clamp_depth(int d);
size_t scan_temp_bytes(size_t P);
size_t sort_temp_bytes(size_t R);

struct FrameParams {
    int P, D, M, W, H, gx, gy;
    int ty0, ty1;
    float focal_x, focal_y, tan_fovx, tan_fovy, scale_modifier;
    StpSettings s;
    const float* background;
    const float* means3D;
    const float* shs;
    const float* colors_precomp;
    const float* opacities;
    const float* scales;
    const float* rotations;
    const float* cov3D_precomp;
    const float* viewmatrix;
    const float* projmatrix;
    const float* inv_viewprojmatrix;
    const float* cam_pos;
    int prefiltered;
    int log_depth;
    uint32_t* log_need;
    uint32_t log_tag;
    int split_launch = 0;
    int fused_gather = 0;
    const float* bg_image = nullptr;
    float* out_alpha = nullptr;
    float* out_invdepth = nullptr;
    const float* sh_dc = nullptr;
    int raw_params = 0;
    int wild_cov;
};

struct CameraGradRequest {
    float* dL_dview = nullptr;
    float* dL_dproj = nullptr;
    float* dL_dcam = nullptr;
    void* workspace = nullptr;
    size_t workspace_bytes = 0;
};

struct BackwardParams {
    CameraGradRequest cam;
    float* absgrad = nullptr;
    float* blend_stats = nullptr;
    const float* bg_image = nullptr;
    const float* dL_dalpha = nullptr;
    float* dL_dbackground = nullptr;
    const float* invdepth = nullptr;
    const float* dL_dinvdepth = nullptr;
    const float* pixel_colors;
    const float* dL_dpix;
    float* grad_rec;
    int grad_stride;
    int clear_rec;
    int chunk, chunks;
    float* dL_dmean2D;
    float* dL_dopacity;
    float* dL_dcolor;
    float* dL_dmean3D;
    float* dL_dcov3D;
    float* dL_dsh;
    float* dL_dscale;
    float* dL_drot;
    const float* sh_stash = nullptr;
    float* dL_ddc = nullptr;
};

int check_settings(const StpSettings& s, bool backward);
void fill_frame(FrameParams& f, int P, int D, int M, const float* background, int width, int height, const StpSettings& s, const float* means3D,
                const float* shs, const float* colors_precomp, const float* opacities, const float* scales, float scale_modifier, const float* rotations,
                const float* cov3D_precomp, const float* viewmatrix, const float* projmatrix, const float* inv_viewprojmatrix, const float* cam_pos,
                float tan_fovx, float tan_fovy, int prefiltered);

struct ForwardSplit { int row = 0; hipEvent_t event = nullptr; bool armed = false; };
struct ForwardBackground { const float* bg_image = nullptr; float* out_alpha = nullptr; };
struct ForwardRequests { ForwardSplit split; ForwardBackground background; float* out_invdepth = nullptr;  const float* sh_dc = nullptr;  bool sh_stash = false;  int raw_params = 0;  };
ForwardRequests take_forward_requests();
int check_raw_params(int mask, const float* opacities, const float* scales, const float* rotations);

hipError_t launch_preprocess(const FrameParams& f, const GeometryState& g, int* radii, uint32_t* tile_counts, hipStream_t st);
hipError_t launch_frame_init(const GeometryState& g, const ImageState& img, int tile0, int n_tiles, bool with_log, bool tile_counters, hipStream_t st);
hipError_t launch_scan(const FrameParams& f, const GeometryState& g, hipStream_t st);
bool tile_order_enabled();
inline bool tile_order_used(const FrameParams& f) { return tile_order_enabled() && f.gx * (f.ty1 - f.ty0) > 1024; }
bool gather_order_enabled();
int gather_order_mode();
hipError_t launch_tile_order(const FrameParams& f, const ImageState& img, hipStream_t st);
hipError_t launch_sh_color(const FrameParams& f, const GeometryState& g, const int* radii, float* sh_stash, hipStream_t st);
hipError_t launch_stash_mark(const FrameParams& f, const GeometryState& g, float* sh_stash, hipStream_t st);
hipError_t launch_mailbox(const uint32_t* last_offset, const uint32_t* status, uint32_t* mailbox_dev, uint32_t ticket, uint32_t* log_need, hipStream_t st);
hipError_t launch_block_prefix_mailbox(const FrameParams& f, const GeometryState& g, uint32_t* mailbox_dev, uint32_t ticket, uint32_t* log_need, hipStream_t st);
hipError_t launch_duplicate(const FrameParams& f, const GeometryState& g, const int* radii, const BinningState& b, uint32_t* tile_cursor, uint32_t cap, uint32_t header_cap, uint32_t* zero_ptr, size_t zero_words, hipStream_t st);
hipError_t launch_tile_scan(const FrameParams& f, const ImageState& img, hipStream_t st);
hipError_t launch_bin_pad(const BinningState& b, const ImageState& img, int R, hipStream_t st);
hipError_t launch_sort(const FrameParams& f, const BinningState& b, int R, bool tile_bits_only, bool zeroed, hipStream_t st);
void sort_zero_region(const BinningState& b, size_t R, uint32_t tiles, uint32_t** ptr, size_t* words);
hipError_t launch_tile_sort_gather(const FrameParams& f, const GeometryState& g, const BinningState& b, const ImageState& img, int R, bool unordered, hipStream_t st);
hipError_t launch_ranges(const FrameParams& f, const BinningState& b, const ImageState& img, int R, hipStream_t st);
hipError_t launch_gather_entries(const FrameParams& f, const GeometryState& g, const BinningState& b, int R, hipStream_t st);
hipError_t launch_render_forward(const FrameParams& f, const GeometryState& g, const BinningState& b, const ImageState& img,
                                 float* out_color, hipStream_t st, std::string* err);
hipError_t launch_render_debug_finish(const FrameParams& f, const ImageState& img, float* out_color, hipStream_t st);
hipError_t launch_render_backward(const FrameParams& f, const GeometryState& g, const BinningState& b, const ImageState& img,
                                  const BackwardParams& bw, hipStream_t st, std::string* err);
size_t background_grad_partials();
hipError_t launch_background_grad(const FrameParams& f, const ImageState& img, const BackwardParams& bw, float* partials, hipStream_t st);
hipError_t launch_preprocess_backward(const FrameParams& f, const GeometryState& g, const int* radii, const BackwardParams& bw, hipStream_t st);
size_t camera_grad_workspace_bytes(int P);
hipError_t launch_camera_grad_finalize(int P, const CameraGradRequest& cam, hipStream_t st);
hipError_t launch_mark_visible(int P, const float* means3D, const float* viewmatrix, uint8_t* present, hipStream_t st);
int launch_sparse_adam(int n_tensors, const StpAdamTensor* tensors, int N, const void* visible, int visible_kind, float beta1, float beta2,
                       hipStream_t st, hipError_t* err);
int launch_activate_params(int P, const float* scaling, const float* rotation, const float* opacity, float* scales, float* rotations, float* opacities,
                           hipStream_t st, hipError_t* err);
int launch_mcmc_relocation(int n, const float* opacity_old, const float* scale_old, const void* N, int n_kind, int n_max, float* opacity_new,
                           float* scale_new, hipStream_t st, hipError_t* err);
int launch_mcmc_add_noise(int P, float* xyz, const float* scales, const float* rotations, const float* opacities, const float* noise, float noise_scale,
                          float k, float x0, int raw, hipStream_t st, hipError_t* err);
int launch_densify_stats(int P, float* grad_accum, float* denom, float* max_radii2D, const float* grad2d, int grad_stride, const void* visible,
                         int visible_kind, hipStream_t st, hipError_t* err);
int launch_densify_plan(int P, const float* grad_accum, const float* denom, const float* scaling, const float* opacity, const float* max_radii2D,
                        const StpDensifyRule& rule, uint8_t* plan, hipStream_t st, hipError_t* err);
size_t densify_scratch_bytes(int P);
int launch_densify_scan(int P, const uint8_t* plan, void* scratch, uint32_t* offsets, int64_t counts[3], hipStream_t st, hipError_t* err);
int launch_densify_apply(int P, const uint8_t* plan, const uint32_t* offsets, const int64_t counts[3], int n_tensors, const StpDensifyTensor* tensors,
                         const float* noise, float split_shrink, int raw, hipStream_t st, hipError_t* err);
uint32_t photometric_groups(int planes, int H, int W);
int launch_photometric_forward(int planes, int H, int W, const float* image, const float* target, float* out2, float* maps, float* workspace,
                               hipStream_t st, hipError_t* err);
int launch_photometric_backward(int planes, int H, int W, const float* image, const float* target, const float* maps, const float* dL_dout2,
                                float* dL_dimage, hipStream_t st, hipError_t* err);

size_t knn_scratch_bytes(int P);
int launch_knn_mean_dist2(int P, const float* points, void* scratch, float* mean_dist2, hipStream_t st, hipError_t* err);

uint32_t higher_msb(uint32_t n);

}
```

stopthepop-rasterization_amd/csrc/stp_preprocess.hip:

```cpp
#include "stp_internal.h"
#include "stp_device.h"
#include "stp_sh_dir.h"
#include "stp_activations.h"

namespace stp {

namespace {

struct PreArgs {
    int P, D, M, W, H, gx, gy, ty0, ty1;
    float focal_x, focal_y, tan_fovx, tan_fovy, scale_modifier;
    int sort_order, rect_bounding, tight_opacity_bounding, tile_based_culling, proper_ewa_scaling, prefiltered;
    int raw;
    const float* means3D;
    const float* scales;
    const float* rotations;
    const float* opacities;
    const float* shs;
    const float* cov3D_precomp;
    const float* colors_precomp;
    const float* view;
    const float* proj;
    const float* cam;
    int* radii;
// ... 452 lines not shown
        for (uint64_t i = (uint64_t)total + ((uint32_t)blockIdx.x - (uint32_t)nb) * 256u + threadIdx.x; i < (uint64_t)a.cap; i += (uint64_t)DUP_PAD_BLOCKS * 256u) {
            a.values[i] = 0xFFFFFFFFu;
            a.keys[i] = make_sort_key(INVALID_TILE_ID, FLT_MAX);
        }
        return;
    }
    const int idx = blockIdx.x * blockDim.x + threadIdx.x;
    const bool valid = idx < a.P && a.radii[idx] > 0;
    const bool tbc = a.tile_based_culling != 0;
    const bool per_tile_depth = a.sort_order == ORDER_PTD_CENTER || a.sort_order == ORDER_PTD_MAX;
    const bool eval_max = tbc || a.sort_order == ORDER_PTD_MAX;
    uint32_t off = 0, off_to = 0;
    int x0 = 0, y0 = 0, x1 = 0, y1 = 0;
    DupGaussian g{};
    float3 cam = make_float3(0, 0, 0);
    if (per_tile_depth) cam = make_float3(a.cam[0], a.cam[1], a.cam[2]);
    if (a.g.block_prefix != nullptr) {
        if (idx < a.P) {
            const uint32_t base = a.g.block_prefix[blockIdx.x];
            off = base + (threadIdx.x == 0 ? 0u : a.g.point_offsets[idx - 1]);
            off_to = base + a.g.point_offsets[idx];
        }
        __syncthreads();
        if (idx < a.P) a.g.point_offsets[idx] = off_to;
    } else if (valid) {
        off = (idx == 0) ? 0u : a.g.point_offsets[idx - 1];
        off_to = a.g.point_offsets[idx];
    }
    if (valid) {
        g.xy = a.g.means2D[idx];
        const float2 ext = a.g.rects2D[idx];
        get_rect(g.xy, ext, a.gx, a.gy, a.ty0, a.ty1, x0, y0, x1, y1);
        if (eval_max) {
            g.co = a.g.conic_opacity[idx];
            g.thr = log_rounded(g.co.w / ALPHA_THRESHOLD);
        }
        if (per_tile_depth) {
            g.p0 = f4_xyz(a.g.cov3D_inv[3 * (size_t)idx + 0]);
            g.p1 = f4_xyz(a.g.cov3D_inv[3 * (size_t)idx + 1]);
            g.p2 = f4_xyz(a.g.cov3D_inv[3 * (size_t)idx + 2]);
        }
        g.global_depth = a.g.depths[idx];
    }
    const bool coop = valid && a.tile_cursor == nullptr && (x1 - x0) * (y1 - y0) > COOP_TILES;
    if (valid && !coop) {
        for (int y = y0; y < y1; y++)
            for (int x = x0; x < x1; x++) {
                uint64_t key;
                if (duplicate_tile(a, g, cam, tbc, eval_max, per_tile_depth, x, y, key)) {
                    if (a.tile_cursor) {
                        const uint32_t slot = atomicAdd(&a.tile_cursor[(uint32_t)(key >> 32)], 1u);
                        a.values[slot] = (uint32_t)idx;
                        a.keys[slot] = key;
                    } else if (off < off_to && off < a.cap) {
                        a.values[off] = (uint32_t)idx;
                        a.keys[off] = key;
                    }
                    off++;
                }
            }
        if (!a.tile_cursor)
            for (; off < off_to && off < a.cap; off++) {
                a.values[off] = 0xFFFFFFFFu;
                a.keys[off] = make_sort_key(INVALID_TILE_ID, FLT_MAX);
            }
    }
    const int lane = wave_lane();
    unsigned long long todo = __ballot(coop);
    while (todo) {
        const int src = (int)__builtin_ctzll(todo);
        todo &= todo - 1ull;
        DupGaussian s;
        s.xy = make_float2(bcast_f(g.xy.x, src), bcast_f(g.xy.y, src));
        s.co = make_float4(bcast_f(g.co.x, src), bcast_f(g.co.y, src), bcast_f(g.co.z, src), bcast_f(g.co.w, src));
        s.thr = bcast_f(g.thr, src);
        s.p0 = make_float3(bcast_f(g.p0.x, src), bcast_f(g.p0.y, src), bcast_f(g.p0.z, src));
        s.p1 = make_float3(bcast_f(g.p1.x, src), bcast_f(g.p1.y, src), bcast_f(g.p1.z, src));
        s.p2 = make_float3(bcast_f(g.p2.x, src), bcast_f(g.p2.y, src), bcast_f(g.p2.z, src));
        s.global_depth = bcast_f(g.global_depth, src);
        const int sx0 = bcast_i(x0, src), sy0 = bcast_i(y0, src), sx1 = bcast_i(x1, src), sy1 = bcast_i(y1, src);
        const uint32_t s_to = (uint32_t)bcast_i((int)off_to, src), s_idx = (uint32_t)bcast_i(idx, src);
        uint32_t base = (uint32_t)bcast_i((int)off, src);
        const int w = sx1 - sx0, n = w * (sy1 - sy0);
        for (int t0 = 0; t0 < n; t0 += 64) {
            const int t = t0 + lane;
            const int ty = t / w;
            uint64_t key = 0;
            const bool wr = t < n && duplicate_tile(a, s, cam, tbc, eval_max, per_tile_depth, sx0 + (t - ty * w), sy0 + ty, key);
            const unsigned long long wm = __ballot(wr);
            const uint32_t slot = base + (uint32_t)lanes_below(wm);
            if (wr && slot < s_to && slot < a.cap) { a.values[slot] = s_idx; a.keys[slot] = key; }
            base += (uint32_t)__popcll(wm);
        }
        for (uint32_t p = base + (uint32_t)lane; p < s_to && p < a.cap; p += 64u) {
            a.values[p] = 0xFFFFFFFFu;
            a.keys[p] = make_sort_key(INVALID_TILE_ID, FLT_MAX);
        }
    }
}

__global__ void __launch_bounds__(256) tile_ranges_kernel(int L, const uint64_t* __restrict__ keys, uint2* __restrict__ ranges, uint32_t T)
{
    const int idx = blockIdx.x * blockDim.x + threadIdx.x;
    if (idx >= L) return;
    const uint32_t cur = (uint32_t)(keys[idx] >> 32);
    const bool valid = cur != INVALID_TILE_ID && cur < T;
    if (idx == 0) {
        if (valid) ranges[cur].x = 0;
    } else {
        const uint32_t prev = (uint32_t)(keys[idx - 1] >> 32);
        if (cur != prev) {
            if (prev < T) ranges[prev].y = (uint32_t)idx;
            if (valid) ranges[cur].x = (uint32_t)idx;
        }
    }
    if (idx == L - 1 && valid) ranges[cur].y = (uint32_t)L;
}

__global__ void __launch_bounds__(1024) tile_order_kernel(int tile0, int T, const uint2* __restrict__ ranges_, uint32_t* __restrict__ order, uint32_t* __restrict__ gather_order)
{
    __shared__ uint32_t s_hist[256];
    __shared__ uint32_t s_hx[8 * 256];
    const uint2* __restrict__ ranges = ranges_ + tile0;
    const int tid = (int)threadIdx.x;
    auto klass = [](uint32_t len) { return 255u - (len < 2048u ? (len >> 4) : min(127u, (len - 2048u) >> 7) + 128u); };
    const int xq = T >> 3, xr = T & 7;
    auto xcd_of = [&](int t) { const int cut = xr * (xq + 1); return t < cut ? t / (xq + 1) : xr + (xq ? (t - cut) / xq : 0); };
    if (tid < 256) s_hist[tid] = 0u;
    for (int i = tid; i < 8 * 256; i += 1024) s_hx[i] = 0u;
    __syncthreads();
    for (int t = tid; t < T; t += 1024) {
        const uint32_t c = klass(ranges[t].y - ranges[t].x);
        atomicAdd(&s_hist[c], 1u);
        if (gather_order) atomicAdd(&s_hx[xcd_of(t) * 256 + c], 1u);
    }
    __syncthreads();
    const int wv = tid >> 6, ln = tid & 63;
    if (wv < (gather_order ? 9 : 1)) {
        uint32_t* const h = wv == 0 ? s_hist : s_hx + (wv - 1) * 256;
        uint32_t c[4], sum = 0;
        for (int k = 0; k < 4; k++) { c[k] = h[4 * ln + k]; sum += c[k]; }
        uint32_t inc = sum;
        for (int o = 1; o < 64; o <<= 1) { const uint32_t v = __shfl_up(inc, o); if (ln >= o) inc += v; }
        uint32_t run = inc - sum;
        for (int k = 0; k < 4; k++) { h[4 * ln + k] = run; run += c[k]; }
    }
    __syncthreads();
    for (int t = tid; t < T; t += 1024) {
        const uint32_t c = klass(ranges[t].y - ranges[t].x);
        order[atomicAdd(&s_hist[c], 1u)] = (uint32_t)t;
        if (gather_order) { const int x = xcd_of(t); gather_order[8u * atomicAdd(&s_hx[x * 256 + c], 1u) + (uint32_t)x] = (uint32_t)t; }
    }
}

__global__ void __launch_bounds__(256) mark_visible_kernel(int P, const float* __restrict__ means3D, const float* __restrict__ view, uint8_t* __restrict__ present)
{
#pragma clang fp contract(off)
    const int idx = blockIdx.x * blockDim.x + threadIdx.x;
    if (idx >= P) return;
    const float z = view[2] * means3D[3 * (size_t)idx] + view[6] * means3D[3 * (size_t)idx + 1] + view[10] * means3D[3 * (size_t)idx + 2] + view[14] * 1.0f;
    present[idx] = z > 0.2f ? 1 : 0;
}

}

hipError_t launch_preprocess(const FrameParams& f, const GeometryState& g, int* radii, uint32_t* tile_counts, hipStream_t st)
{
    PreArgs a;
    a.P = f.P; a.D = f.D; a.M = f.M; a.W = f.W; a.H = f.H; a.gx = f.gx; a.gy = f.gy; a.ty0 = f.ty0; a.ty1 = f.ty1;
    a.focal_x = f.focal_x; a.focal_y = f.focal_y; a.tan_fovx = f.tan_fovx; a.tan_fovy = f.tan_fovy; a.scale_modifier = f.scale_modifier;
    a.sort_order = f.s.sort_order; a.rect_bounding = f.s.rect_bounding; a.tight_opacity_bounding = f.s.tight_opacity_bounding;
    a.tile_based_culling = f.s.tile_based_culling; a.proper_ewa_scaling = f.s.proper_ewa_scaling; a.prefiltered = f.prefiltered;
    a.raw = f.raw_params;
    a.means3D = f.means3D; a.scales = f.scales; a.rotations = f.rotations; a.opacities = f.opacities; a.shs = f.shs;
    a.cov3D_precomp = f.cov3D_precomp; a.colors_precomp = f.colors_precomp; a.view = f.viewmatrix; a.proj = f.projmatrix; a.cam = f.cam_pos;
    a.radii = radii; a.g = g; a.tile_counts = tile_counts;
    if (f.out_invdepth == nullptr) a.g.invz = nullptr;
    hipLaunchKernelGGL(preprocess_kernel, dim3((f.P + 255) / 256), dim3(256), 0, st, a);
    return hipGetLastError();
}

hipError_t launch_duplicate(const FrameParams& f, const GeometryState& g, const int* radii, const BinningState& b, uint32_t* tile_cursor, uint32_t cap, uint32_t header_cap,
                            uint32_t* zero_ptr, size_t zero_words, hipStream_t st)
{
    DupArgs a;
    a.P = f.P; a.W = f.W; a.H = f.H; a.gx = f.gx; a.gy = f.gy; a.ty0 = f.ty0; a.ty1 = f.ty1;
    a.sort_order = f.s.sort_order; a.tile_based_culling = f.s.tile_based_culling;
    a.inv_vp = f.inv_viewprojmatrix; a.cam = f.cam_pos; a.radii = radii; a.g = g;
    a.tile_cursor = tile_cursor;
    a.keys = tile_cursor ? b.keys : b.keys_unsorted; a.values = tile_cursor ? b.point_list : b.point_list_unsorted;
    const bool capped = cap != 0xFFFFFFFFu && g.block_prefix != nullptr && tile_cursor == nullptr;
    a.cap = capped ? cap : 0xFFFFFFFFu;
    a.n_gauss_blocks = (f.P + 255) / 256;
    a.n_pad_blocks = capped ? DUP_PAD_BLOCKS : 0;
    a.zero_ptr = zero_ptr; a.zero_words = (uint32_t)zero_words;
    a.header = b.header; a.header_cap = header_cap;
    hipLaunchKernelGGL(duplicate_kernel, dim3(a.n_gauss_blocks + a.n_pad_blocks + (zero_words ? DUP_ZERO_BLOCKS : 0)), dim3(256), 0, st, a);
    return hipGetLastError();
}

hipError_t launch_sh_color(const FrameParams& f, const GeometryState& g, const int* radii, float* sh_stash, hipStream_t st)
{
    const bool split = f.sh_dc != nullptr;
    if (f.colors_precomp != nullptr || (f.shs == nullptr && !split) || f.M <= 0) return hipSuccess;
    ShArgs a;
    a.P = f.P; a.D = f.D; a.M = f.M; a.means3D = f.means3D; a.shs = f.shs; a.cam = f.cam_pos; a.radii = radii; a.clamped = g.clamped; a.rgb = g.rgb;
    a.dc = f.sh_dc;
    const bool stash = sh_stash != nullptr;
    a.stash = sh_stash; a.mark = g.status + STP_STASH_WORD;
    using Kernel = void (*)(const ShArgs);
    static const Kernel kernels[4] = {sh_color_kernel<false, false>, sh_color_kernel<true, false>, sh_color_kernel<false, true>, sh_color_kernel<true, true>};
    const Kernel kernel = kernels[(stash ? 2 : 0) + (split ? 1 : 0)];
    const size_t lds = (size_t)SH_BLOCK * (3 * a.M + 1) * sizeof(float);
    if (lds > 64 * 1024) {
        hipError_t e = hipFuncSetAttribute(reinterpret_cast<const void*>(kernel), hipFuncAttributeMaxDynamicSharedMemorySize, (int)lds);
        if (e != hipSuccess) return e;
    }
    hipLaunchKernelGGL(kernel, dim3((f.P + SH_BLOCK - 1) / SH_BLOCK), dim3(SH_BLOCK), lds, st, a);
    return hipGetLastError();
}

hipError_t launch_stash_mark(const FrameParams& f, const GeometryState& g, float* sh_stash, hipStream_t st)
{
    if (sh_stash == nullptr) return hipSuccess;
    hipLaunchKernelGGL(stash_mark_kernel, dim3(1), dim3(1), 0, st, g.status + STP_STASH_WORD, (uint32_t)f.P);
    return hipGetLastError();
}

__global__ void mailbox_kernel(const uint32_t* __restrict__ last_offset, const uint32_t* __restrict__ status, volatile uint32_t* mailbox, uint32_t ticket,
                               uint32_t* log_need)
{
    mailbox[0] = *last_offset;
    mailbox[1] = *status;
    mailbox[3] = log_need ? atomicExch(log_need, 0u) : 0u;
    __threadfence_system();
    mailbox[2] = ticket;
    __threadfence_system();
}

__global__ void __launch_bounds__(1024) block_prefix_mailbox_kernel(const uint32_t* __restrict__ block_sums, uint32_t* __restrict__ block_prefix, int n_blocks,
                                                                     const uint32_t* __restrict__ status, volatile uint32_t* mailbox, uint32_t ticket,
                                                                     uint32_t* log_need)
{
    __shared__ uint32_t s_wave_total[16];
    const int tid = (int)threadIdx.x, lane = tid & 63, wave = tid >> 6;
    const int per = (n_blocks + 1023) / 1024, i0 = min(tid * per, n_blocks), i1 = min(i0 + per, n_blocks);
    uint32_t mine = 0u;
    for (int i = i0; i < i1; i++) mine += block_sums[i];
    uint32_t v = mine;
#pragma unroll
    for (int d = 1; d < 64; d <<= 1) {
        const uint32_t t = (uint32_t)__shfl_up((int)v, d);
        if (lane >= d) v += t;
    }
    if (lane == 63) s_wave_total[wave] = v;
    __syncthreads();
    for (int k = 0; k < wave; k++) v += s_wave_total[k];
    uint32_t run = v - mine;
    for (int i = i0; i < i1; i++) { block_prefix[i] = run; run += block_sums[i]; }
    if (tid == 1023) {
        mailbox[0] = v;
        mailbox[1] = status[1];
        mailbox[3] = log_need ? atomicExch(log_need, 0u) : 0u;
        __threadfence_system();
        mailbox[2] = ticket;
        __threadfence_system();
    }
}

hipError_t launch_block_prefix_mailbox(const FrameParams& f, const GeometryState& g, uint32_t* mailbox_dev, uint32_t ticket, uint32_t* log_need, hipStream_t st)
{
    hipLaunchKernelGGL(block_prefix_mailbox_kernel, dim3(1), dim3(1024), 0, st, g.block_sums, g.block_prefix, (f.P + 255) / 256, g.status, mailbox_dev, ticket, log_need);
    return hipGetLastError();
}

hipError_t launch_mailbox(const uint32_t* last_offset, const uint32_t* status, uint32_t* mailbox_dev, uint32_t ticket, uint32_t* log_need, hipStream_t st)
{
    hipLaunchKernelGGL(mailbox_kernel, dim3(1), dim3(1), 0, st, last_offset, status, mailbox_dev, ticket, log_need);
    return hipGetLastError();
}

__global__ void __launch_bounds__(256) frame_init_kernel(uint32_t* __restrict__ status, uint2* __restrict__ ranges, uint32_t* __restrict__ tile_flags,
                                                          uint32_t flag_value, uint32_t* __restrict__ tile_counts, int tile0, int T,
                                                          uint32_t* __restrict__ header, uint32_t log_depth)
{
    const int i = blockIdx.x * blockDim.x + threadIdx.x;
    if (i < 64) status[i] = 0u;
    if (i == 0) { header[0] = STP_HEADER_MAGIC_IMAGE; header[1] = log_depth; header[2] = ~log_depth; header[3] = 0u; }
    if (i < T) {
        ranges[tile0 + i] = make_uint2(0u, 0u);
        tile_flags[tile0 + i] = flag_value;
        if (tile_counts) tile_counts[tile0 + i] = 0u;
    }
}

hipError_t launch_frame_init(const GeometryState& g, const ImageState& img, int tile0, int T, bool with_log, bool tile_counters, hipStream_t st)
{
    const int n = T > 64 ? T : 64;
    hipLaunchKernelGGL(frame_init_kernel, dim3((n + 255) / 256), dim3(256), 0, st, g.status, img.ranges, img.tile_flags, with_log ? 0u : 0xFFFFFFFFu,
                       tile_counters ? img.tile_counts : nullptr, tile0, T, img.header, (uint32_t)(with_log ? img.log_depth : 0));
    return hipGetLastError();
}

hipError_t launch_ranges(const FrameParams& f, const BinningState& b, const ImageState& img, int R, hipStream_t st)
{
    const size_t T = (size_t)f.gx * f.gy;
    hipError_t e = hipSuccess;
    if (R > 0) {
        hipLaunchKernelGGL(tile_ranges_kernel, dim3((R + 255) / 256), dim3(256), 0, st, R, b.keys, img.ranges, (uint32_t)T);
        e = hipGetLastError();
    }
    return e;
}

bool tile_order_enabled() { return switches().tile_order; }
bool gather_order_enabled() { return gather_order_mode() != 0; }
int gather_order_mode() { return switches().gather_order; }
hipError_t launch_tile_order(const FrameParams& f, const ImageState& img, hipStream_t st)
{
    const int T = f.gx * (f.ty1 - f.ty0);
    if (T <= 0) return hipSuccess;
    hipLaunchKernelGGL(tile_order_kernel, dim3(1), dim3(1024), 0, st, f.gx * f.ty0, T, img.ranges, img.tile_cursor + f.gx * f.ty0,
                       gather_order_enabled() ? img.tile_counts + f.gx * f.ty0 : nullptr);
    return hipGetLastError();
}

__global__ void __launch_bounds__(256) gather_entries_kernel(int R, const uint32_t* __restrict__ point_list, const uint64_t* __restrict__ keys,
                                                             const float4* __restrict__ gpack, const float* __restrict__ features,
                                                             float4* __restrict__ entA, float4* __restrict__ entB, float4* __restrict__ entC,
                                                             float4* __restrict__ entD, float4* __restrict__ entF, int mask_kind, int gx, uint32_t T)
{
    const int i = blockIdx.x * blockDim.x + threadIdx.x;
    if (i >= R) return;
    const int id = (int)point_list[i];
    if (id < 0) return;
    const float4* __restrict__ gp = gpack + 4 * (size_t)id;
    const float4 pa = gp[0], pb = gp[1], pc = gp[2], pd = gp[3];
    entA[i] = pa;
    entB[i] = pb;
    entC[i] = make_float4(pc.x, pc.y, pc.z, __int_as_float(id));
    entD[i] = pd;
    float spare = 0.0f;
    const uint32_t tile = (uint32_t)(keys[i] >> 32);
    if (mask_kind && tile < T) spare = __uint_as_float(subtile_mask(mask_kind, pd, make_float2(pc.y, pc.z), (int)(tile % (uint32_t)gx), (int)(tile / (uint32_t)gx)));
    entF[i] = make_float4(features[3 * (size_t)id], features[3 * (size_t)id + 1], features[3 * (size_t)id + 2], spare);
}

hipError_t launch_gather_entries(const FrameParams& f, const GeometryState& g, const BinningState& b, int R, hipStream_t st)
{
    if (R <= 0 || (f.s.sort_mode != MODE_HIER && f.s.sort_mode != MODE_KBUFFER)) return hipSuccess;
    const float* features = f.colors_precomp ? f.colors_precomp : g.rgb;
    hipLaunchKernelGGL(gather_entries_kernel, dim3((R + 255) / 256), dim3(256), 0, st, R, b.point_list, b.keys, g.gpack, features, b.entA, b.entB, b.entC,
                       b.entD, b.entF, subtile_mask_kind(f.s), f.gx, (uint32_t)(f.gx * f.gy));
    return hipGetLastError();
}

hipError_t launch_mark_visible(int P, const float* means3D, const float* viewmatrix, uint8_t* present, hipStream_t st)
{
    hipLaunchKernelGGL(mark_visible_kernel, dim3((P + 255) / 256), dim3(256), 0, st, P, means3D, viewmatrix, present);
    return hipGetLastError();
}

}
```

stopthepop-rasterization_amd/diff_gaussian_rasterization/_C.py:

```python
from __future__ import annotations

import ctypes
import os
from typing import Tuple

import torch

_HERE = os.path.dirname(os.path.abspath(__file__))
_LIB_NAME = "libstp_raster.so"
_lib = None
_host = None


GRAD_RECORD_FLOATS = 16


class StpSettings(ctypes.Structure):
    _fields_ = [(n, ctypes.c_int32) for n in (
        "sort_mode", "sort_order", "queue_tile_4x4", "queue_tile_2x2", "queue_per_pixel",
        "rect_bounding", "tight_opacity_bounding", "tile_based_culling", "hierarchical_4x4_culling",
        "load_balancing", "proper_ewa_scaling", "tile_y0", "tile_y1", "record_blend_log", "debug_visualization")]


_lib_override = None

_OPTIONAL_SYMBOLS = {
    "stp_camera_grad_workspace_bytes": ([ctypes.c_int], ctypes.c_size_t, "camera gradients"),
    "stp_set_backward_camera_grads": ([ctypes.c_void_p] * 4 + [ctypes.c_size_t], None, "camera gradients"),
    "stp_set_backward_absgrad": ([ctypes.c_void_p], None, "absgrad"),
    "stp_set_backward_blend_stats": ([ctypes.c_void_p], None, "blend statistics"),
    "stp_set_forward_background": ([ctypes.c_void_p] * 2, None, "the alpha output and per-pixel background"),
    "stp_set_backward_background": ([ctypes.c_void_p] * 3, None, "the alpha output and per-pixel background"),
    "stp_set_forward_invdepth": ([ctypes.c_void_p], None, "the inverse-depth output"),
    "stp_set_backward_invdepth": ([ctypes.c_void_p] * 2, None, "the inverse-depth output"),
    "stp_set_forward_split_sh": ([ctypes.c_void_p], None, "split SH inputs"),
    "stp_set_backward_split_sh": ([ctypes.c_void_p] * 2, None, "split SH inputs"),
    "stp_set_forward_sh_stash": ([ctypes.c_int], None, "the SH stash"),
    "stp_set_forward_raw_params": ([ctypes.c_int], None, "raw parameter inputs"),
    "stp_set_backward_raw_params": ([ctypes.c_int], None, "raw parameter inputs"),
    "stp_activate_params": ([ctypes.c_int] + [ctypes.c_void_p] * 7, ctypes.c_int, "raw parameter inputs"),
    "stp_geometry_buffer_size_stash": ([ctypes.c_int, ctypes.POINTER(StpSettings)], ctypes.c_size_t, "the SH stash"),
    "stp_sparse_adam": ([ctypes.c_int, ctypes.c_void_p, ctypes.c_int, ctypes.c_void_p, ctypes.c_int, ctypes.c_float, ctypes.c_float, ctypes.c_void_p],
                        ctypes.c_int, "the sparse Adam step"),
    "stp_mcmc_relocation": ([ctypes.c_int] + [ctypes.c_void_p] * 3 + [ctypes.c_int] * 2 + [ctypes.c_void_p] * 3, ctypes.c_int, "the 3DGS-MCMC kernels"),
    "stp_mcmc_add_noise": ([ctypes.c_int] + [ctypes.c_void_p] * 5 + [ctypes.c_float] * 3 + [ctypes.c_int, ctypes.c_void_p], ctypes.c_int, "the 3DGS-MCMC kernels"),
    "stp_knn_scratch_bytes": ([ctypes.c_int], ctypes.c_size_t, "the nearest-neighbour kernels"),
    "stp_knn_mean_dist2": ([ctypes.c_int] + [ctypes.c_void_p] * 2 + [ctypes.c_size_t] + [ctypes.c_void_p] * 2, ctypes.c_int, "the nearest-neighbour kernels"),
    "stp_densify_stats": ([ctypes.c_int] + [ctypes.c_void_p] * 4 + [ctypes.c_int, ctypes.c_void_p, ctypes.c_int, ctypes.c_void_p], ctypes.c_int, "the densification kernels"),
    "stp_densify_plan": ([ctypes.c_int] + [ctypes.c_void_p] * 8, ctypes.c_int, "the densification kernels"),
    "stp_densify_scratch_bytes": ([ctypes.c_int], ctypes.c_size_t, "the densification kernels"),
    "stp_densify_scan": ([ctypes.c_int] + [ctypes.c_void_p] * 2 + [ctypes.c_size_t] + [ctypes.c_void_p] * 3, ctypes.c_int, "the densification kernels"),
    "stp_densify_apply": ([ctypes.c_int] + [ctypes.c_void_p] * 3 + [ctypes.c_int] + [ctypes.c_void_p] * 2 + [ctypes.c_float, ctypes.c_int, ctypes.c_void_p],
                          ctypes.c_int, "the densification kernels"),
    "stp_photometric_workspace_floats": ([ctypes.c_int] * 3, ctypes.c_size_t, "the photometric loss"),
    "stp_photometric_forward": ([ctypes.c_int] * 3 + [ctypes.c_void_p] * 6, ctypes.c_int, "the photometric loss"),
    "stp_photometric_backward": ([ctypes.c_int] * 3 + [ctypes.c_void_p] * 6, ctypes.c_int, "the photometric loss"),
}
_SYMBOL_FEATURE = {name: entry[2] for name, entry in _OPTIONAL_SYMBOLS.items()}


def _require(name: str):
    L = _load()
    if not hasattr(L, name):
        raise RuntimeError(f"{library_path()} does not export {name} (a library built before {_OPTIONAL_SYMBOLS[name][2]}): rebuild it")
    return getattr(L, name)


def camera_grad_workspace_bytes(P: int) -> int:
    return int(_require("stp_camera_grad_workspace_bytes")(int(P)))


def library_path() -> str:
    p = _lib_override or os.environ.get("STP_RASTER_LIB", os.path.join(_HERE, _LIB_NAME))
    return os.path.join(_HERE, "libstp_raster_fma.so") if p == "fma" else p


def use_library(path=None) -> None:
    global _lib, _host, _lib_override
    if path in ("fma", "default"):
        path = os.path.join(_HERE, "libstp_raster_fma.so" if path == "fma" else _LIB_NAME)
    _lib, _host, _lib_override = None, None, path


def _load():
    global _lib
    if _lib is not None:
        return _lib
    path = library_path()
    if not os.path.exists(path):
        raise ImportError(
            f"{path} not found: build it with `make -C stopthepop-rasterization_amd/csrc` "
            f"(or python -c 'import __graft_entry__ as g; g.build()'). There is no CPU fallback.")
    L = ctypes.CDLL(path)
    vp, ci, cf = ctypes.c_void_p, ctypes.c_int, ctypes.c_float
    L.stp_last_error.restype = ctypes.c_char_p
    L.stp_abi_version.restype = ci
    for name in ("stp_geometry_buffer_size", "stp_binning_buffer_size", "stp_image_buffer_size"):
        getattr(L, name).restype = ctypes.c_size_t
    L.stp_geometry_buffer_size.argtypes = [ci, ctypes.POINTER(StpSettings)]
    L.stp_binning_buffer_size.argtypes = [ci]
    L.stp_image_buffer_size.argtypes = [ci, ci]
    L.stp_blend_log_bytes.argtypes = [ci, ci]
    L.stp_blend_log_bytes.restype = ctypes.c_size_t
    szp = ctypes.POINTER(ctypes.c_size_t)
    L.stp_geometry_layout.argtypes = [ci, ctypes.POINTER(StpSettings), ctypes.c_char_p, szp, szp]
    L.stp_binning_layout.argtypes = [ci, ctypes.c_char_p, szp, szp]
    L.stp_image_layout.argtypes = [ci, ci, ctypes.c_char_p, szp, szp]
    L.stp_timing_enable.argtypes = [ci]
    L.stp_timing_enable.restype = None
    L.stp_timing_read.argtypes = [ctypes.POINTER(ctypes.c_float)]
    L.stp_timing_read.restype = ci
    L.stp_hbm_probe.argtypes = [ci, ctypes.c_void_p, ctypes.c_void_p, ctypes.c_size_t, ci, ctypes.c_void_p]
    L.stp_hbm_probe.restype = ci
    L.stp_timing_history.argtypes = [ctypes.POINTER(ctypes.c_float), ci]
    L.stp_timing_history.restype = ci
    L.stp_timing_history_host.argtypes = [ctypes.POINTER(ctypes.c_float), ci]
    L.stp_timing_history_host.restype = ci
    L.stp_timing_text.argtypes = [ctypes.c_char_p, ctypes.c_size_t]
    L.stp_timing_text.restype = ctypes.c_size_t
    L.stp_binning_layout_count.argtypes = [vp, ci]
    L.stp_binning_layout_count.restype = ci
    L.stp_forget_buffer.argtypes = [vp]
    L.stp_forget_buffer.restype = None
    for name in _OPTIONAL_SYMBOLS:
        if hasattr(L, name):
            fn = getattr(L, name)
            fn.argtypes, fn.restype = _OPTIONAL_SYMBOLS[name][:2]
    if L.stp_abi_version() != 7:
        raise ImportError("libstp_raster.so ABI version mismatch")
    _lib = L
    return L


def _native():
    global _host
    if _host is not None:
        return _host
    _load()
    try:
        from . import _stp_host
    except ImportError as ex:
        raise ImportError(f"the native host binding diff_gaussian_rasterization._stp_host is missing ({ex}): build it with "
                          f"`python stopthepop-rasterization_amd/csrc/host/build_host.py` (or python -c 'import __graft_entry__ as g; "
                          f"g.build()').  There is no pure-Python fallback.") from ex
    _stp_host.load_library(library_path())
    global _atexit_registered
    if not _atexit_registered:
        import atexit
        atexit.register(lambda: _stp_host.clear_scratch_pool(-1))
        _atexit_registered = True
    _host = _stp_host
    return _host


_atexit_registered = False


def settings_from_dict(d: dict, tile_rows=None) -> StpSettings:
    ss, cs = d["sort_settings"], d["culling_settings"]
    q = ss["queue_sizes"]
    s = StpSettings()
    s.sort_mode = int(ss["sort_mode"])
    s.sort_order = int(ss["sort_order"])
    s.queue_tile_4x4 = int(q["tile_4x4"])
    s.queue_tile_2x2 = int(q["tile_2x2"])
    s.queue_per_pixel = int(q["per_pixel"])
    s.rect_bounding = int(bool(cs["rect_bounding"]))
    s.tight_opacity_bounding = int(bool(cs["tight_opacity_bounding"]))
    s.tile_based_culling = int(bool(cs["tile_based_culling"]))
    s.hierarchical_4x4_culling = int(bool(cs["hierarchical_4x4_culling"]))
    s.load_balancing = int(bool(d["load_balancing"]))
    s.proper_ewa_scaling = int(bool(d["proper_ewa_scaling"]))
    tr = tile_rows if tile_rows is not None else d.get("_tile_rows")
    if tr is not None:
        s.tile_y0, s.tile_y1 = int(tr[0]), int(tr[1])
    if _records_log(d):
        s.record_blend_log = 1
    return s


_BACKWARD_MODES = ("replay", "resort", "auto")
_backward_mode = os.environ.get("STP_BACKWARD", "replay")
if _backward_mode not in _BACKWARD_MODES:
    raise ImportError(f"STP_BACKWARD={_backward_mode!r}: expected one of {_BACKWARD_MODES}")
_log_budget_bytes = int(float(os.environ.get("STP_LOG_BUDGET_GB", "16")) * (1 << 30))
_log_live = {}


def set_backward_mode(mode: str, log_budget_bytes=None) -> None:
    global _backward_mode, _log_budget_bytes
    if mode not in _BACKWARD_MODES:
        raise ValueError(f"backward mode {mode!r}: expected one of {_BACKWARD_MODES}")
    _backward_mode = mode
    if log_budget_bytes is not None:
        _log_budget_bytes = int(log_budget_bytes)


def backward_mode() -> str:
    return _backward_mode


def blend_log_bytes(width: int, height: int, tile_rows=None, depth=None) -> int:
    L = _load()
    y0, y1 = (0, 0) if tile_rows is None else (int(tile_rows[0]), int(tile_rows[1]))
    if depth is not None:
        L.stp_blend_log_bytes_depth.argtypes = [ctypes.c_int] * 5
        L.stp_blend_log_bytes_depth.restype = ctypes.c_size_t
        return int(L.stp_blend_log_bytes_depth(int(width), int(height), y0, y1, int(depth)))
    if tile_rows is None:
        return int(L.stp_blend_log_bytes(int(width), int(height)))
    L.stp_blend_log_bytes_rows.argtypes = [ctypes.c_int] * 4
    L.stp_blend_log_bytes_rows.restype = ctypes.c_size_t
    return int(L.stp_blend_log_bytes_rows(int(width), int(height), y0, y1))


class LogLease:

    def __init__(self, index: int, nbytes: int):
        self.index, self.nbytes = index, int(nbytes)
        _log_live[index] = _log_live.get(index, 0) + self.nbytes

    def resize(self, nbytes: int) -> None:
        if self.nbytes:
            _log_live[self.index] = _log_live.get(self.index, 0) - self.nbytes + int(nbytes)
            self.nbytes = int(nbytes)

    def release(self) -> None:
        if self.nbytes:
            _log_live[self.index] = _log_live.get(self.index, 0) - self.nbytes
            self.nbytes = 0

    __del__ = release


def live_log_bytes(device=None) -> int:
    return _log_live.get(_device_index(device), 0)


def decide_recording(mode, device, width: int, height: int, tile_rows=None) -> bool:
    mode = mode or _backward_mode
    if mode not in _BACKWARD_MODES:
        raise ValueError(f"backward mode {mode!r}: expected one of {_BACKWARD_MODES}")
    if mode != "auto":
        return mode == "replay"
    idx = _device_index(device)
    need = blend_log_bytes(width, height, tile_rows, depth=0)
    pooled = list(_native().pooled_sizes(idx))
    reuse = any(need <= n for n in pooled)
    return _log_live.get(idx, 0) + sum(pooled) + (0 if reuse else need) <= _log_budget_bytes


def _on_device(device):
    import contextlib
    return torch.cuda.device(_device_index(device)) if torch.cuda.is_available() else contextlib.nullcontext()


def _device_index(device) -> int:
    if device is None:
        return torch.cuda.current_device()
    if isinstance(device, int):
        return device
    d = torch.device(device)
    return torch.cuda.current_device() if d.index is None else d.index


def _raise_last(rc: int):
    msg = _load().stp_last_error()
    raise RuntimeError((msg.decode() if msg else "") or f"libstp_raster error {rc}")


def clear_scratch_pool(device=None) -> int:
    return int(_native().clear_scratch_pool(-1 if device is None else _device_index(device)))


def set_scratch_pool_limit(max_buffers: int = 4, max_bytes=None) -> None:
    _native().set_scratch_pool_limit(int(max_buffers), -1 if max_bytes is None else int(max_bytes))


def scratch_generation(buf: torch.Tensor) -> int:
    return int(_native().scratch_generation(buf))


def check_scratch(buf: torch.Tensor, generation: int) -> None:
    _native().check_scratch(buf, int(generation))


def set_forward_split(tile_row: int, event) -> None:
    _native().set_forward_split(int(tile_row), 0 if event is None else int(event.cuda_event))


def release_scratch(buf: torch.Tensor) -> None:
    _native().release_scratch(buf)


def _records_log(d: dict) -> bool:
    return bool(d.get("_record_blend_log")) and d.get("_backward_mode", _backward_mode) != "resort"


def rasterize_gaussians(background, means3D, colors, opacity, scales, rotations, scale_modifier, cov3D_precomp,
                        viewmatrix, projmatrix, inv_viewprojmatrix, tan_fovx, tan_fovy, image_height, image_width,
                        sh, degree, campos, prefiltered, settings_dict, render_depth, debug, alpha=False, invdepth=False,
                        raw=0, dc=None) -> Tuple[int, torch.Tensor, torch.Tensor, torch.Tensor, torch.Tensor, torch.Tensor]:
    if means3D.dim() != 2 or means3D.size(1) != 3:
        raise RuntimeError("means3D must have dimensions (num_points, 3)")
    if alpha or _per_pixel_background(background, image_height, image_width):
        _require("stp_set_forward_background")
    if invdepth:
        _require("stp_set_forward_invdepth")
        if render_depth:
            raise RuntimeError("the inverse-depth output (_invdepth) is not available with render_depth (the debug depth visualisation)")
    if dc is not None:
        _require("stp_set_forward_split_sh")
    if raw:
        _require("stp_set_forward_raw_params")
    out = (_host or _native()).rasterize_gaussians(
        background, means3D, colors, opacity, scales, rotations, scale_modifier, cov3D_precomp, viewmatrix, projmatrix,
        inv_viewprojmatrix, tan_fovx, tan_fovy, int(image_height), int(image_width), sh, int(degree), campos, bool(prefiltered),
        settings_dict, bool(render_depth), bool(debug), _records_log(settings_dict), bool(alpha), bool(invdepth), dc, int(raw))
    return tuple(out[:6]) + ((out[6],) if alpha else ()) + ((out[7],) if invdepth else ())


def _per_pixel_background(background, height, width) -> bool:
    return isinstance(background, torch.Tensor) and tuple(background.shape) == (3, int(height), int(width))


def rasterize_gaussians_backward(background, means3D, radii, opacities, colors, scales, rotations, scale_modifier,
                                 cov3D_precomp, viewmatrix, projmatrix, inv_viewprojmatrix, tan_fovx, tan_fovy,
                                 pixel_colors, dL_dout_color, sh, degree, campos, geomBuffer, R, binningBuffer,
                                 imageBuffer, settings_dict, debug, phases=3, partial=None, chunk=None, outputs=None,
                                 camera_grads=False, absgrad=False, blend_stats=False, dL_dalpha=None, bg_grad=False,
                                 dL_dinvdepth=None, invdepth=None, raw=0, dc=None):
    if chunk is not None:
        k, K = int(chunk[0]), int(chunk[1])
        if not (0 <= k < K <= 255) or (int(phases) & 1):
            raise ValueError("chunk = (k, K) with 0 <= k < K <= 255, per-Gaussian half only")
        phases = int(phases) | (K << 8) | (k << 16)
    if camera_grads:
        _require("stp_set_backward_camera_grads")
    if absgrad:
        _require("stp_set_backward_absgrad")
    if blend_stats:
        _require("stp_set_backward_blend_stats")
    if dL_dinvdepth is not None:
        _require("stp_set_backward_invdepth")
    if dc is not None:
        _require("stp_set_backward_split_sh")
    if raw:
        _require("stp_set_backward_raw_params")
    if dL_dalpha is not None or bg_grad or _per_pixel_background(background, dL_dout_color.shape[-2], dL_dout_color.shape[-1]):
        _require("stp_set_backward_background")
    out = (_host or _native()).rasterize_gaussians_backward(
        background, means3D, radii, opacities, colors, scales, rotations, scale_modifier, cov3D_precomp, viewmatrix, projmatrix,
        inv_viewprojmatrix, tan_fovx, tan_fovy, pixel_colors, dL_dout_color, sh, int(degree), campos, geomBuffer, int(R), binningBuffer,
        imageBuffer, settings_dict, bool(debug), _records_log(settings_dict), int(phases), partial, None if outputs is None else list(outputs),
        bool(camera_grads), bool(absgrad), bool(blend_stats), dL_dalpha, bool(bg_grad), dL_dinvdepth, invdepth, dc, int(raw))
    return out[0] if (int(phases) & 3) == 1 and not bg_grad else tuple(out)


def mark_visible(means3D, viewmatrix, projmatrix) -> torch.Tensor:
    return (_host or _native()).mark_visible(means3D, viewmatrix, projmatrix)


def sparse_adam(params, grads, exp_avgs, exp_avg_sqs, visible, lrs, epss, beta1, beta2, N) -> int:
    _require("stp_sparse_adam")
    return int((_host or _native()).sparse_adam(list(params), list(grads), list(exp_avgs), list(exp_avg_sqs), visible, [float(x) for x in lrs],
                                                [float(x) for x in epss], float(beta1), float(beta2), int(N)))


def adamUpdate(param, grad, exp_avg, exp_avg_sq, visible, lr, b1, b2, eps, N, M) -> None:
    if int(N) * int(M) != param.numel():
        raise RuntimeError(f"adamUpdate: param has {param.numel()} elements, N * M = {int(N) * int(M)}")
    sparse_adam([param], [grad], [exp_avg], [exp_avg_sq], visible, [lr], [eps], b1, b2, N)


RELOCATION_N_MAX = 51


def compute_relocation(opacity_old, scale_old, N, binoms=None, n_max=RELOCATION_N_MAX):
    _require("stp_mcmc_relocation")
    return tuple((_host or _native()).compute_relocation(opacity_old, scale_old, N, binoms, int(n_max)))


def mcmc_add_noise(xyz, scales, rotations, opacities, noise, noise_scale, k, x0, raw) -> int:
    _require("stp_mcmc_add_noise")
    return int((_host or _native()).mcmc_add_noise(xyz, scales, rotations, opacities, noise, float(noise_scale), float(k), float(x0), bool(raw)))


def activate_params(scaling=None, rotation=None, opacity=None):
    if scaling is None and rotation is None and opacity is None:
        return None, None, None
    _require("stp_activate_params")
    out = (_host or _native()).activate_params(scaling, rotation, opacity)
    return tuple(o if given is not None else None for o, given in zip(out, (scaling, rotation, opacity)))


KNN_BOX = 256


def knn_scratch_bytes(P: int) -> int:
    return int(_require("stp_knn_scratch_bytes")(int(P)))


def knn_mean_dist2(points):
    _require("stp_knn_mean_dist2")
    return (_host or _native()).knn_mean_dist2(points)


class StpDensifyRule(ctypes.Structure):
    _fields_ = [(name, ctypes.c_float) for name in ("grad_threshold", "split_size", "min_opacity", "max_screen_size", "max_world_size", "split_shrink")] + \
               [("raw", ctypes.c_int32), ("prune_big", ctypes.c_int32)]


class StpDensifyTensor(ctypes.Structure):
    _fields_ = [(name, ctypes.c_void_p) for name in ("param", "exp_avg", "exp_avg_sq", "param_out", "exp_avg_out", "exp_avg_sq_out")] + \
               [("row", ctypes.c_int32), ("role", ctypes.c_int32)]


DENSIFY_ROLES = {"plain": 0, "xyz": 1, "scaling": 2, "rotation": 3}


def densify_stats(xyz_gradient_accum, denom, max_radii2D, grad2d, radii) -> int:
    _require("stp_densify_stats")
    return int((_host or _native()).densify_stats(xyz_gradient_accum, denom, max_radii2D, grad2d, radii))


def densify_plan(xyz_gradient_accum, denom, scaling, opacity, max_radii2D, rule, raw, prune_big):
    _require("stp_densify_plan")
    return (_host or _native()).densify_plan(xyz_gradient_accum, denom, scaling, opacity, max_radii2D, [float(x) for x in rule], bool(raw), bool(prune_big))


def densify_scan(plan):
    _require("stp_densify_scan")
    offsets, nK, nC, nS = (_host or _native()).densify_scan(plan)
    return offsets, (int(nK), int(nC), int(nS))


def densify_apply(plan, offsets, counts, tensors, roles, exp_avgs, exp_avg_sqs, noise, split_shrink, raw):
    _require("stp_densify_apply")
    out = (_host or _native()).densify_apply(plan, offsets, [int(c) for c in counts], list(tensors), [int(r) for r in roles], list(exp_avgs),
                                             list(exp_avg_sqs), noise, float(split_shrink), bool(raw))
    return list(out[0]), list(out[1]), list(out[2])


def photometric_forward(image, target, want_maps):
    for name in ("stp_photometric_workspace_floats", "stp_photometric_forward", "stp_photometric_backward"):
        _require(name)
    out2, maps = (_host or _native()).photometric_forward(image, target, bool(want_maps))
    return out2, (maps if want_maps else None)


def photometric_backward(image, target, maps, grad_out2):
    _require("stp_photometric_backward")
    return (_host or _native()).photometric_backward(image, target, maps, grad_out2)


_GEOM_TYPES = {"depths": torch.float32, "clamped": torch.uint8, "radii": torch.int32, "rects2D": torch.float32,
               "means2D": torch.float32, "cov3D": torch.float32, "cov3D_inv": torch.float32,
               "conic_opacity": torch.float32, "rgb": torch.float32, "tiles_touched": torch.int32,
               "point_offsets": torch.int32, "invz": torch.float32,
               "sh_stash": torch.float32}
_BIN_TYPES = {"point_list": torch.int32, "point_list_unsorted": torch.int32, "keys": torch.int64, "keys_unsorted": torch.int64}
_IMG_TYPES = {"final_T": torch.float32, "n_contrib": torch.int32, "ranges": torch.int32, "tile_flags": torch.int32,
              "blend_log": torch.int16}


def timing_text(device=None) -> str:
    buf = ctypes.create_string_buffer(512)
    with _on_device(device):
        _load().stp_timing_text(buf, 512)
    return buf.value.decode()


def _view(buf: torch.Tensor, off: int, count: int, dtype) -> torch.Tensor:
    nbytes = count * torch.empty((), dtype=dtype).element_size()
    return buf[off:off + nbytes].view(dtype)


def has_sh_stash(geomBuffer, P, settings_dict) -> bool:
    if geomBuffer.numel() < 48:
        return False
    w = geomBuffer[32:44].view(torch.int32).cpu().tolist()
    return (w[0] & 0xFFFFFFFF) == 0x53505453 and (w[1] & 0xFFFFFFFF) == int(P) and (w[2] & 0xFFFFFFFF) == (~int(P) & 0xFFFFFFFF)


def geometry_array(geomBuffer, P, settings_dict, name):
    s = settings_from_dict(settings_dict)
    off, cnt = ctypes.c_size_t(), ctypes.c_size_t()
    if _load().stp_geometry_layout(int(P), ctypes.byref(s), name.encode(), ctypes.byref(off), ctypes.byref(cnt)) != 0:
        raise KeyError(name)
    return _view(geomBuffer, off.value, cnt.value, _GEOM_TYPES[name])


def binning_array(binningBuffer, R, name):
    off, cnt = ctypes.c_size_t(), ctypes.c_size_t()
    L = _load()
    if binningBuffer.is_cuda:
        _native().forget_unless_same_storage(binningBuffer)
    lay = int(L.stp_binning_layout_count(ctypes.c_void_p(binningBuffer.data_ptr()), int(R))) if int(R) > 0 else 0
    if lay < 0:
        _raise_last(lay)
    if L.stp_binning_layout(lay, name.encode(), ctypes.byref(off), ctypes.byref(cnt)) != 0:
        raise KeyError(name)
    n = cnt.value // lay * int(R) if lay > 0 else cnt.value
    return _view(binningBuffer, off.value, n, _BIN_TYPES[name])


def image_array(imgBuffer, W, H, name, tile_rows=None):
    off, cnt = ctypes.c_size_t(), ctypes.c_size_t()
    L = _load()
    L.stp_image_layout_depth.argtypes = [ctypes.c_int] * 5 + [ctypes.c_char_p, ctypes.POINTER(ctypes.c_size_t), ctypes.POINTER(ctypes.c_size_t)]
    y0, y1 = (0, 0) if tile_rows is None else (int(tile_rows[0]), int(tile_rows[1]))
    depth = blend_log_depth(imgBuffer) if name == "blend_log" else 0
    if L.stp_image_layout_depth(int(W), int(H), y0, y1, depth, name.encode(), ctypes.byref(off), ctypes.byref(cnt)) != 0:
        raise KeyError(name)
    return _view(imgBuffer, off.value, cnt.value, _IMG_TYPES[name])


def blend_log_depth(imgBuffer) -> int:
    L = _load()
    L.stp_blend_log_depth.argtypes = [ctypes.c_void_p]
    L.stp_blend_log_depth.restype = ctypes.c_int
    if imgBuffer.is_cuda:
        _native().forget_unless_same_storage(imgBuffer)
    d = int(L.stp_blend_log_depth(ctypes.c_void_p(imgBuffer.data_ptr())))
    if d < 0:
        _raise_last(d)
    return d


def set_run_ahead(mode) -> int:
    L = _load()
    L.stp_set_run_ahead.argtypes = [ctypes.c_int]
    L.stp_set_run_ahead.restype = None
    L.stp_get_run_ahead.restype = ctypes.c_int
    prev = int(L.stp_get_run_ahead())
    L.stp_set_run_ahead(int(mode))
    return prev


def reset_size_guesses() -> None:
    L = _load()
    L.stp_reset_size_guesses.restype = None
    L.stp_reset_size_guesses()


def timing_enable(flag: bool) -> None:
    _load().stp_timing_enable(int(bool(flag)))


def hbm_probe(kind: str, dst, src, blocks: int = 4096, nontemporal: bool = False) -> None:
    import torch
    t = src if src is not None else dst
    k = {"read": 0, "write": 1, "copy": 2}[kind] + (4 if nontemporal else 0)
    with _on_device(t.device):
        rc = _load().stp_hbm_probe(k, None if dst is None else dst.data_ptr(), None if src is None else src.data_ptr(),
                                   t.numel() * t.element_size(), int(blocks), torch.cuda.current_stream(t.device).cuda_stream)
    if rc < 0:
        raise RuntimeError(f"stp_hbm_probe failed ({rc})")


def timing_history(device=None, capacity=1024, host=False):
    arr = (ctypes.c_float * (6 * capacity))()
    with _on_device(device):
        n = (_load().stp_timing_history_host if host else _load().stp_timing_history)(arr, capacity)
    if n < 0:
        _raise_last(n)
    names = ("Preprocess", "Duplicate", "Sort", "Render", "BwdRender", "BwdPreprocess")
    return [{nm: float(arr[6 * k + i]) for i, nm in enumerate(names) if arr[6 * k + i] >= 0.0} for k in range(n)]


def timing_read(device=None):
    arr = (ctypes.c_float * 6)()
    with _on_device(device):
        rc = _load().stp_timing_read(arr)
    if rc < 0:
        _raise_last(rc)
    names = ("Preprocess", "Duplicate", "Sort", "Render", "BwdRender", "BwdPreprocess")
    return {n: float(v) for n, v in zip(names, arr)}
```

stopthepop-rasterization_amd/diff_gaussian_rasterization/__init__.py:

```python
from __future__ import annotations

import json
from dataclasses import asdict, dataclass, field, fields
from enum import IntEnum
from typing import NamedTuple, Optional

import torch
import torch.nn as nn

from . import _C

__all__ = ["rasterize_gaussians", "SortMode", "GlobalSortOrder", "SortQueueSizes", "SortSettings", "CullingSettings",
           "ExtendedSettings", "GaussianRasterizationSettings", "GaussianRasterizer", "SparseGaussianAdam",
           "photometric_terms", "fused_ssim", "photometric_loss", "compute_relocation", "mcmc_add_noise_",
           "knn_mean_dist2", "distCUDA2", "dist_cuda2", "activate_params",
           "densification_stats_", "densify_plan", "densify_tensors", "densify_and_prune"]


def enum_dict_factory(data):
    return {k: (v.value if isinstance(v, IntEnum) else v) for k, v in data}


def cpu_deep_copy_tuple(input_tuple):
    return tuple(item.cpu().clone() if isinstance(item, torch.Tensor) else item for item in input_tuple)


def rasterize_gaussians(means3D, means2D, sh, colors_precomp, opacities, scales, rotations, cov3Ds_precomp,
                        raster_settings, dc=None, raw=0):
    if raw:
        raster_settings = _with_raw_mask(raster_settings, int(raw))
    rs = raster_settings
    if torch.is_grad_enabled() and isinstance(rs.bg, torch.Tensor) and rs.bg.requires_grad:
        return _RasterizeGaussiansBackground.apply(means3D, means2D, sh, colors_precomp, opacities, scales, rotations, cov3Ds_precomp,
                                                   rs.bg, rs.viewmatrix, rs.projmatrix, rs.campos, raster_settings, dc)
    if torch.is_grad_enabled() and any(isinstance(t, torch.Tensor) and t.requires_grad for t in (rs.viewmatrix, rs.projmatrix, rs.campos)):
        return _RasterizeGaussiansCamera.apply(means3D, means2D, sh, colors_precomp, opacities, scales, rotations, cov3Ds_precomp,
                                               rs.viewmatrix, rs.projmatrix, rs.campos, raster_settings, dc)
    return _RasterizeGaussians.apply(means3D, means2D, sh, colors_precomp, opacities, scales, rotations,
                                     cov3Ds_precomp, raster_settings, dc)


def _forward_body(ctx, means3D, means2D, sh, colors_precomp, opacities, scales, rotations, cov3Ds_precomp, viewmatrix, projmatrix, campos, rs,
                  save_camera=False, bg=None, dc=None):
    sdict = rs.settings.to_dict()
    save_bg = bg is not None
    if bg is None:
        bg = rs.bg
    ctx.alpha = bool(sdict.get("_alpha"))
    if rs.render_depth and (ctx.alpha or save_bg or _C._per_pixel_background(bg, rs.image_height, rs.image_width)):
        raise RuntimeError("the alpha output (settings._alpha), a per-pixel background and a background that requires grad are not available "
                           "with render_depth=True: the depth visualisation's image is not C + T * background")
    ctx.invdepth = bool(sdict.get("_invdepth"))
    if ctx.invdepth and rs.render_depth:
        raise RuntimeError("the inverse-depth output (settings._invdepth) is not available with render_depth=True: the depth visualisation "
                           "replaces the image and has no backward")
    ctx.log_lease = None
    ctx.absgrad_target = None
    if sdict.get("_absgrad"):
        if rs.render_depth:
            raise RuntimeError("absgrad (settings._absgrad) is not available with render_depth=True: the depth visualisation has no "
                               "backward that could produce it")
        ctx.absgrad_target = means2D
    ctx.blend_stats_target = None
    if sdict.get("_blend_stats"):
        if rs.render_depth:
            raise RuntimeError("blend statistics (settings._blend_stats) are not available with render_depth=True: the depth visualisation "
                               "has no backward that could produce them")
        ctx.blend_stats_target = means2D
    if any(ctx.needs_input_grad) and not rs.render_depth:
        mode = sdict.get("_backward_mode")
        uses_log = int(sdict["sort_settings"]["sort_mode"]) in (2, 3)
        if uses_log and means3D.is_cuda and means3D.size(0) != 0 and _C.decide_recording(mode, means3D.device, rs.image_width, rs.image_height):
            sdict["_record_blend_log"] = True
            sdict["_backward_mode"] = "replay"
            ctx.log_lease = _C.LogLease(_C._device_index(means3D.device), _C.blend_log_bytes(rs.image_width, rs.image_height))
        else:
            sdict["_backward_mode"] = "resort"
        sdict["_sh_stash"] = True
    if colors_precomp.numel() == 0:
        sdict["_no_grad_colors"] = True
    if cov3Ds_precomp.numel() == 0:
        sdict["_no_grad_cov3D"] = True
    ctx.settings_dict = sdict
    args = (bg, means3D, colors_precomp, opacities, scales, rotations, rs.scale_modifier, cov3Ds_precomp,
            viewmatrix, projmatrix, rs.inv_viewprojmatrix, rs.tanfovx, rs.tanfovy, rs.image_height,
            rs.image_width, sh, rs.sh_degree, campos, rs.prefiltered, sdict, rs.render_depth,
            rs.debug)
    kw = {"alpha": True} if ctx.alpha else {}
    if ctx.invdepth:
        kw["invdepth"] = True
    ctx.dc_index = None
    if dc is not None and colors_precomp.numel() == 0:
        kw["dc"] = dc
        ctx.dc_index = 12 + (3 if save_camera else 0) + (1 if save_bg else 0)
    ctx.raw = int(getattr(rs, "raw_mask", 0))
    if ctx.raw:
        kw["raw"] = ctx.raw
    if rs.debug:
        cpu_args = cpu_deep_copy_tuple(args + ((dc,) if "dc" in kw else ()) + ((ctx.raw,) if ctx.raw else ()))
        try:
            num_rendered, color, radii, geomBuffer, binningBuffer, imgBuffer, *extra = _C.rasterize_gaussians(*args, **kw)
        except Exception as ex:
            torch.save(cpu_args, "snapshot_fw.dump")
            print("\nAn error occured in forward. Please forward snapshot_fw.dump for debugging.")
            raise ex
    else:
        num_rendered, color, radii, geomBuffer, binningBuffer, imgBuffer, *extra = _C.rasterize_gaussians(*args, **kw)

    if ctx.log_lease is not None:
        ctx.log_lease.resize(_C.blend_log_bytes(rs.image_width, rs.image_height, depth=_C.blend_log_depth(imgBuffer)))
    ctx.raster_settings = rs
    ctx.num_rendered = num_rendered
    ctx.img_generation = _C.scratch_generation(imgBuffer)
    ctx.bin_generation = _C.scratch_generation(binningBuffer)
    ctx.save_for_backward(colors_precomp, means3D, opacities, scales, rotations, cov3Ds_precomp, radii, sh, color,
                          geomBuffer, binningBuffer, imgBuffer, *((viewmatrix, projmatrix, campos) if save_camera else ()),
                          *((bg,) if save_bg else ()), *((dc,) if ctx.dc_index is not None else ()),
                          *((extra[-1],) if ctx.invdepth else ()))
    ctx.mark_non_differentiable(radii)
    ctx.set_materialize_grads(False)
    return (color, radii, *extra)


def _grad_alpha(ctx, rest):
    return rest[0] if ctx.alpha and rest else None


def _grad_invdepth(ctx, rest):
    i = 1 if ctx.alpha else 0
    return rest[i] if ctx.invdepth and len(rest) > i else None


def _backward_body(ctx, grad_out_color, viewmatrix, projmatrix, campos, camera_grads=False, grad_alpha=None, bg=None, grad_invdepth=None):
    num_rendered = ctx.num_rendered
    rs = ctx.raster_settings
    (colors_precomp, means3D, opacities, scales, rotations, cov3Ds_precomp, radii, sh, color, geomBuffer,
     binningBuffer, imgBuffer) = ctx.saved_tensors[:12]
    _C.check_scratch(imgBuffer, ctx.img_generation)
    _C.check_scratch(binningBuffer, ctx.bin_generation)
    if grad_out_color is None:
        grad_out_color = torch.zeros_like(color)
    bg_grad = bg is not None
    if bg is None:
        bg = rs.bg
    args = (bg, means3D, radii, opacities, colors_precomp, scales, rotations, rs.scale_modifier, cov3Ds_precomp,
            viewmatrix, projmatrix, rs.inv_viewprojmatrix, rs.tanfovx, rs.tanfovy, color, grad_out_color, sh,
            rs.sh_degree, campos, geomBuffer, num_rendered, binningBuffer, imgBuffer, ctx.settings_dict,
            rs.debug)
    kw = {"camera_grads": True} if camera_grads else {}
    if ctx.absgrad_target is not None:
        kw["absgrad"] = True
    if ctx.blend_stats_target is not None:
        kw["blend_stats"] = True
    if grad_alpha is not None:
        kw["dL_dalpha"] = grad_alpha
    if bg_grad:
        kw["bg_grad"] = True
    if grad_invdepth is not None:
        kw["dL_dinvdepth"] = grad_invdepth
        kw["invdepth"] = ctx.saved_tensors[-1]
    dc = ctx.saved_tensors[ctx.dc_index] if ctx.dc_index is not None else None
    if dc is not None:
        kw["dc"] = dc
    if ctx.raw:
        kw["raw"] = ctx.raw
    if rs.debug:
        cpu_args = cpu_deep_copy_tuple(args + ((dc,) if dc is not None else ()) + ((ctx.raw,) if ctx.raw else ()))
        try:
            out = _C.rasterize_gaussians_backward(*args, **kw)
        except Exception as ex:
            torch.save(cpu_args, "snapshot_bw.dump")
            print("\nAn error occured in backward. Writing snapshot_bw.dump for debugging.\n")
            raise ex
    else:
        out = _C.rasterize_gaussians_backward(*args, **kw)
    _C.release_scratch(imgBuffer); _C.release_scratch(binningBuffer)
    if ctx.log_lease is not None:
        ctx.log_lease.release()
    ctx.grad_dc = None
    if dc is not None:
        ctx.grad_dc = out[-1].view(dc.shape)
        out = out[:-1]
    grad_bg = None
    if bg_grad:
        grad_bg = out[-1]
        out = out[:-1]
        if grad_bg.shape != bg.shape:
            full = torch.zeros(bg.numel(), dtype=grad_bg.dtype, device=grad_bg.device)
            full[:3] = grad_bg
            grad_bg = full.reshape(bg.shape)
    if ctx.blend_stats_target is not None:
        ctx.blend_stats_target.blend_stats = out[-1]
        out = out[:-1]
    if ctx.absgrad_target is not None:
        ctx.absgrad_target.absgrad = out[-1]
        out = out[:-1]
    if ctx.raw:
        out = list(out)
        for i, t in ((2, opacities), (6, scales), (7, rotations)):
            if out[i] is not None and t.numel() != 0:
                out[i] = out[i].view(t.shape)
        out = tuple(out)
    return out + (grad_bg,) if bg_grad else out


def _split_grad_sh(ctx, grad_sh):
    return grad_sh if ctx.needs_input_grad[2] else None


def _split_grad_dc(ctx):
    return ctx.grad_dc if ctx.dc_index is not None and ctx.needs_input_grad[-1] else None


class _RasterizeGaussians(torch.autograd.Function):
    @staticmethod
    def forward(ctx, means3D, means2D, sh, colors_precomp, opacities, scales, rotations, cov3Ds_precomp,
                raster_settings, dc=None):
        rs = raster_settings
        return _forward_body(ctx, means3D, means2D, sh, colors_precomp, opacities, scales, rotations, cov3Ds_precomp, rs.viewmatrix,
                             rs.projmatrix, rs.campos, rs, dc=dc)

    @staticmethod
    def backward(ctx, grad_out_color, _, *rest):
        rs = ctx.raster_settings
        (grad_means2D, grad_colors_precomp, grad_opacities, grad_means3D, grad_cov3Ds_precomp, grad_sh, grad_scales,
         grad_rotations) = _backward_body(ctx, grad_out_color, rs.viewmatrix, rs.projmatrix, rs.campos, grad_alpha=_grad_alpha(ctx, rest),
                                          grad_invdepth=_grad_invdepth(ctx, rest))
        if ctx.dc_index is None:
            return (grad_means3D, grad_means2D, grad_sh, grad_colors_precomp, grad_opacities, grad_scales, grad_rotations,
                    grad_cov3Ds_precomp, None, None)
        return (grad_means3D, grad_means2D, _split_grad_sh(ctx, grad_sh), grad_colors_precomp, grad_opacities, grad_scales, grad_rotations,
                grad_cov3Ds_precomp, None, _split_grad_dc(ctx))


class _RasterizeGaussiansCamera(torch.autograd.Function):

    @staticmethod
    def forward(ctx, means3D, means2D, sh, colors_precomp, opacities, scales, rotations, cov3Ds_precomp, viewmatrix, projmatrix, campos,
                raster_settings, dc=None):
        return _forward_body(ctx, means3D, means2D, sh, colors_precomp, opacities, scales, rotations, cov3Ds_precomp, viewmatrix, projmatrix,
                             campos, raster_settings, save_camera=True, dc=dc)

    @staticmethod
    def backward(ctx, grad_out_color, _, *rest):
        viewmatrix, projmatrix, campos = ctx.saved_tensors[12:15]
        (grad_means2D, grad_colors_precomp, grad_opacities, grad_means3D, grad_cov3Ds_precomp, grad_sh, grad_scales,
         grad_rotations, grad_view, grad_proj, grad_campos) = _backward_body(ctx, grad_out_color, viewmatrix, projmatrix, campos, True,
                                                                             grad_alpha=_grad_alpha(ctx, rest),
                                                                             grad_invdepth=_grad_invdepth(ctx, rest))
        grads = (grad_means3D, grad_means2D, grad_sh, grad_colors_precomp, grad_opacities, grad_scales, grad_rotations,
                 grad_cov3Ds_precomp, grad_view, grad_proj, grad_campos)
        return tuple(g if need else None for g, need in zip(grads, ctx.needs_input_grad)) + (None, _split_grad_dc(ctx))


class _RasterizeGaussiansBackground(torch.autograd.Function):

    @staticmethod
    def forward(ctx, means3D, means2D, sh, colors_precomp, opacities, scales, rotations, cov3Ds_precomp, bg, viewmatrix, projmatrix, campos,
                raster_settings, dc=None):
        return _forward_body(ctx, means3D, means2D, sh, colors_precomp, opacities, scales, rotations, cov3Ds_precomp, viewmatrix, projmatrix,
                             campos, raster_settings, save_camera=True, bg=bg, dc=dc)

    @staticmethod
    def backward(ctx, grad_out_color, _, *rest):
        viewmatrix, projmatrix, campos, bg = ctx.saved_tensors[12:16]
        camera_grads = any(ctx.needs_input_grad[9:12])
        out = _backward_body(ctx, grad_out_color, viewmatrix, projmatrix, campos, camera_grads, grad_alpha=_grad_alpha(ctx, rest), bg=bg,
                             grad_invdepth=_grad_invdepth(ctx, rest))
        (grad_means2D, grad_colors_precomp, grad_opacities, grad_means3D, grad_cov3Ds_precomp, grad_sh, grad_scales, grad_rotations) = out[:8]
        grad_view, grad_proj, grad_campos = out[8:11] if camera_grads else (None, None, None)
        grads = (grad_means3D, grad_means2D, grad_sh, grad_colors_precomp, grad_opacities, grad_scales, grad_rotations,
                 grad_cov3Ds_precomp, out[-1], grad_view, grad_proj, grad_campos)
        return tuple(g if need else None for g, need in zip(grads, ctx.needs_input_grad)) + (None, _split_grad_dc(ctx))


class SortMode(IntEnum):
    GLOBAL = 0
    PPX_FULL = 1
    PPX_KBUFFER = 2
    HIER = 3

    def __str__(self):
        return self.name


class GlobalSortOrder(IntEnum):
    Z_DEPTH = 0
    DISTANCE = 1
    PTD_CENTER = 2
    PTD_MAX = 3

    def __str__(self):
        return self.name


class _Settable:
    _children = ()

    def set_value(self, key, value):
        if key in {f.name for f in fields(self)}:
            setattr(self, key, value)
        else:
            for child in self._children:
                getattr(self, child).set_value(key, value)


@dataclass
class SortQueueSizes(_Settable):
    tile_4x4: int = 64
    tile_2x2: int = 8
    per_pixel: int = 4


@dataclass
class SortSettings(_Settable):
    queue_sizes: SortQueueSizes = field(default_factory=SortQueueSizes)
    sort_mode: SortMode = SortMode.GLOBAL
    sort_order: GlobalSortOrder = GlobalSortOrder.Z_DEPTH
    _children = ("queue_sizes",)


@dataclass
class CullingSettings(_Settable):
    rect_bounding: bool = False
    tight_opacity_bounding: bool = False
    tile_based_culling: bool = False
    hierarchical_4x4_culling: bool = False


@dataclass
class ExtendedSettings(_Settable):
    sort_settings: SortSettings = field(default_factory=SortSettings)
    culling_settings: CullingSettings = field(default_factory=CullingSettings)
    load_balancing: bool = False
    proper_ewa_scaling: bool = False
    _children = ("culling_settings", "sort_settings")

    def to_dict(self):
        ss, cs, q = self.sort_settings, self.culling_settings, self.sort_settings.queue_sizes
        as_int = lambda v: v.value if isinstance(v, IntEnum) else v
        return {"sort_settings": {"queue_sizes": {"tile_4x4": q.tile_4x4, "tile_2x2": q.tile_2x2, "per_pixel": q.per_pixel},
                                  "sort_mode": as_int(ss.sort_mode), "sort_order": as_int(ss.sort_order)},
                "culling_settings": {"rect_bounding": cs.rect_bounding, "tight_opacity_bounding": cs.tight_opacity_bounding,
                                     "tile_based_culling": cs.tile_based_culling, "hierarchical_4x4_culling": cs.hierarchical_4x4_culling},
                "load_balancing": self.load_balancing, "proper_ewa_scaling": self.proper_ewa_scaling,
                **({"_backward_mode": self._backward_mode} if getattr(self, "_backward_mode", None) else {}),
                **({"_absgrad": True} if getattr(self, "_absgrad", False) else {}),
                **({"_blend_stats": True} if getattr(self, "_blend_stats", False) else {}),
                **({"_alpha": True} if getattr(self, "_alpha", False) else {}),
                **({"_invdepth": True} if getattr(self, "_invdepth", False) else {})}

    def to_json(self):
        return json.dumps(self.to_dict())

    @staticmethod
    def from_dict(dict):
        try:
            import dacite
            return dacite.from_dict(data_class=ExtendedSettings, data=dict, config=dacite.Config(cast=[IntEnum]))
        except ImportError:
            ss, cs = dict["sort_settings"], dict["culling_settings"]
            return ExtendedSettings(
                sort_settings=SortSettings(queue_sizes=SortQueueSizes(**ss["queue_sizes"]), sort_mode=SortMode(ss["sort_mode"]),
                                           sort_order=GlobalSortOrder(ss["sort_order"])),
                culling_settings=CullingSettings(**cs), load_balancing=dict["load_balancing"],
                proper_ewa_scaling=dict["proper_ewa_scaling"])

    @staticmethod
    def from_json(json_filename):
        return ExtendedSettings.from_dict(json.load(open(json_filename)))


class GaussianRasterizationSettings(NamedTuple):
    image_height: int
    image_width: int
    tanfovx: float
    tanfovy: float
    bg: torch.Tensor
    scale_modifier: float
    viewmatrix: torch.Tensor
    projmatrix: torch.Tensor
    inv_viewprojmatrix: torch.Tensor
    sh_degree: int
    campos: torch.Tensor
    prefiltered: bool
    settings: ExtendedSettings
    render_depth: bool
    debug: bool


def _check_split_sh(dc, shs, means3D):
    if not isinstance(dc, torch.Tensor):
        raise RuntimeError(f"dc must be a tensor, got {type(dc).__name__}")
    P = means3D.shape[0]
    if not ((dc.dim() == 3 and dc.shape[1] == 1 and dc.shape[2] == 3) or (dc.dim() == 2 and dc.shape[1] == 3)):
        raise RuntimeError(f"dc must have dimensions (num_points, 1, 3) or (num_points, 3), got {tuple(dc.shape)}")
    if dc.shape[0] != P:
        raise RuntimeError(f"dc must have one row per Gaussian: {dc.shape[0]} rows for {P} points")
    if dc.dtype != torch.float32:
        raise RuntimeError(f"dc must be a float32 tensor, got {dc.dtype}")
    if dc.device != means3D.device:
        raise RuntimeError(f"dc must be on the device of means3D ({means3D.device}), got {dc.device}")
    if shs is not None and shs.numel() != 0:
        if shs.dim() != 3 or shs.shape[0] != P or shs.shape[2] != 3 or shs.dtype != torch.float32 or shs.device != means3D.device:
            raise RuntimeError(f"with dc, shs is the rest of the coefficients: a float32 (num_points, M - 1, 3) tensor on the device of "
                               f"means3D, got {tuple(shs.shape)} {shs.dtype} on {shs.device}")


class _RawRasterizationSettings(GaussianRasterizationSettings):
    """The settings tuple of one call with raw parameter inputs: the caller's fields, and the mask as the attribute raw_mask."""


def _with_raw_mask(rs, mask):
    out = _RawRasterizationSettings(*rs)
    out.raw_mask = int(mask)
    return out


RAW_PARAM_BITS = {"opacities": 1, "scales": 2, "rotations": 4}


def _raw_mask(raw, opacities, scales, rotations) -> int:
    given = {"opacities": opacities is not None, "scales": scales is not None, "rotations": rotations is not None}
    if raw is None or raw is False:
        return 0
    if raw is True:
        return sum(bit for name, bit in RAW_PARAM_BITS.items() if given[name])
    if isinstance(raw, str):
        raw = (raw,)
    try:
        names = list(raw)
    except TypeError:
        raise RuntimeError(f"raw must be True, False or an iterable of names out of {sorted(RAW_PARAM_BITS)}, got {type(raw).__name__}") from None
    mask = 0
    for name in names:
        if name not in RAW_PARAM_BITS:
            raise RuntimeError(f"raw: unknown name {name!r}: expected names out of {sorted(RAW_PARAM_BITS)}")
        if not given[name]:
            raise RuntimeError(f"raw: {name!r} is named but no {name} are given (with cov3D_precomp there are no scales and rotations to activate)")
        mask |= RAW_PARAM_BITS[name]
    return mask


def activate_params(scaling=None, rotation=None, opacity=None):
    return _C.activate_params(*(None if t is None else t.detach() for t in (scaling, rotation, opacity)))


class GaussianRasterizer(nn.Module):

    def __init__(self, raster_settings, raw=False):
        super().__init__()
        self.raster_settings = raster_settings
        self.raw = raw

    def markVisible(self, positions):
        with torch.no_grad():
            rs = self.raster_settings
            return _C.mark_visible(positions, rs.viewmatrix, rs.projmatrix)

    def forward(self, means3D, means2D, opacities, shs=None, colors_precomp=None, scales=None, rotations=None,
                cov3D_precomp=None, dc=None):
        rs = self.raster_settings
        have_sh = shs is not None or dc is not None
        if (not have_sh and colors_precomp is None) or (have_sh and colors_precomp is not None):
            raise Exception('Please provide excatly one of either SHs or precomputed colors!')
        if dc is not None:
            _check_split_sh(dc, shs, means3D)
        mask = _raw_mask(self.raw, opacities, scales, rotations)
        if ((scales is None or rotations is None) and cov3D_precomp is None) or \
                ((scales is not None or rotations is not None) and cov3D_precomp is not None):
            raise Exception('Please provide exactly one of either scale/rotation pair or precomputed 3D covariance!')
        empty = lambda t: torch.Tensor([]) if t is None else t
        return rasterize_gaussians(means3D, means2D, empty(shs), empty(colors_precomp), opacities, empty(scales),
                                   empty(rotations), empty(cov3D_precomp), rs, dc, *((mask,) if mask else ()))


class SparseGaussianAdam(torch.optim.Adam):

    _REFUSED = ("weight_decay", "amsgrad", "maximize", "capturable", "fused", "foreach")

    def __init__(self, params, lr, eps, betas=(0.9, 0.999), **options):
        for name, value in options.items():
            if name not in self._REFUSED:
                raise TypeError(f"SparseGaussianAdam got an unexpected option {name!r}")
            self._refuse(name, value)
        super().__init__(params=params, lr=lr, eps=eps, betas=betas)
        for group in self.param_groups:
            for name in self._REFUSED:
                self._refuse(name, group.get(name))
            self._one_tensor(group)
        self.last_launches = 0

    @staticmethod
    def _refuse(name, value):
        if value is not None and value is not False and value != 0:
            raise ValueError(f"SparseGaussianAdam does not support {name} (got {name}={value!r}): the fused step is plain Adam without bias "
                             "correction on the visible rows")

    @staticmethod
    def _one_tensor(group):
        if len(group["params"]) != 1:
            raise AssertionError("more than one tensor in group")

    @torch.no_grad()
    def step(self, visibility, N):
        params, grads, exp_avgs, exp_avg_sqs, lrs, epss = [], [], [], [], [], []
        betas = None
        for group in self.param_groups:
            self._one_tensor(group)
            param = group["params"][0]
            if param.grad is None:
                continue
            if betas is None:
                betas = tuple(group["betas"])
            elif tuple(group["betas"]) != betas:
                raise ValueError(f"SparseGaussianAdam steps all groups in one kernel launch: betas must agree, got {betas} and {tuple(group['betas'])}")
            state = self.state[param]
            if len(state) == 0:
                state["step"] = torch.tensor(0.0, dtype=torch.float32)
                state["exp_avg"] = torch.zeros_like(param, memory_format=torch.preserve_format)
                state["exp_avg_sq"] = torch.zeros_like(param, memory_format=torch.preserve_format)
            state["step"] += 1
            params.append(param)
            grads.append(param.grad)
            exp_avgs.append(state["exp_avg"])
            exp_avg_sqs.append(state["exp_avg_sq"])
            lrs.append(float(group["lr"]))
            epss.append(float(group["eps"]))
        self.last_launches = _C.sparse_adam(params, grads, exp_avgs, exp_avg_sqs, visibility, lrs, epss, betas[0], betas[1], N) if params else 0


class _PhotometricTerms(torch.autograd.Function):

    @staticmethod
    def forward(ctx, image, target, want_maps):
        out2, maps = _C.photometric_forward(image, target, want_maps)
        ctx.has_maps = maps is not None
        if ctx.has_maps:
            ctx.save_for_backward(image, target, maps)
        return out2

    @staticmethod
    def backward(ctx, grad_out2):
        if not ctx.has_maps:
            raise RuntimeError("photometric_terms: this forward stored no derivative maps (fused_ssim(train=False)): it cannot be differentiated")
        image, target, maps = ctx.saved_tensors
        return _C.photometric_backward(image, target, maps, grad_out2), None, None


def _photometric(image, target, store_maps=True) -> torch.Tensor:
    want_maps = bool(store_maps) and torch.is_grad_enabled() and isinstance(image, torch.Tensor) and image.requires_grad
    return _PhotometricTerms.apply(image, target, want_maps)


def photometric_terms(image: torch.Tensor, target: torch.Tensor) -> torch.Tensor:
    return _photometric(image, target)


def fused_ssim(img1: torch.Tensor, img2: torch.Tensor, padding: str = "same", train: bool = True) -> torch.Tensor:
    if padding != "same":
        raise ValueError(f"fused_ssim: padding={padding!r} is not supported, only \"same\" (zero padding of 5; \"valid\" is not built)")
    return _photometric(img1, img2, store_maps=train)[1]


def photometric_loss(image: torch.Tensor, target: torch.Tensor, lambda_dssim: float = 0.2) -> torch.Tensor:
    terms = _photometric(image, target)
    return (1.0 - lambda_dssim) * terms[0] + lambda_dssim * (1.0 - terms[1])


def compute_relocation(opacity_old: torch.Tensor, scale_old: torch.Tensor, N: torch.Tensor):
    return _C.compute_relocation(opacity_old.detach(), scale_old.detach(), N, None, _C.RELOCATION_N_MAX)


def mcmc_add_noise_(xyz: torch.Tensor, scales: torch.Tensor, rotations: torch.Tensor, opacities: torch.Tensor, noise: torch.Tensor,
                    noise_scale: float, *, raw: bool = False, k: float = 100.0, x0: float = 0.995) -> torch.Tensor:
    _C.mcmc_add_noise(xyz.detach(), scales.detach(), rotations.detach(), opacities.detach(), noise.detach(), noise_scale, k, x0, raw)
    return xyz


def knn_mean_dist2(points: torch.Tensor) -> torch.Tensor:
    return _C.knn_mean_dist2(points.detach())


dist_cuda2 = distCUDA2 = knn_mean_dist2


def _f32(x) -> float:
    return float(torch.tensor(float(x), dtype=torch.float32))


def densification_stats_(xyz_gradient_accum: torch.Tensor, denom: torch.Tensor, max_radii2D: Optional[torch.Tensor], grad2d: torch.Tensor,
                         radii: torch.Tensor) -> None:
    _C.densify_stats(xyz_gradient_accum.detach(), denom.detach(), None if max_radii2D is None else max_radii2D.detach(), grad2d.detach(), radii)


def densify_plan(xyz_gradient_accum: torch.Tensor, denom: torch.Tensor, scaling: torch.Tensor, opacity: torch.Tensor,
                 max_radii2D: Optional[torch.Tensor] = None, *, grad_threshold: float, percent_dense: float = 0.01, extent: float,
                 min_opacity: float = 0.005, max_screen_size: Optional[float] = None, raw: bool = True) -> torch.Tensor:
    big = max_screen_size is not None
    rule = (_f32(grad_threshold), _f32(float(percent_dense) * float(extent)), _f32(min_opacity), _f32(max_screen_size if big else 0.0),
            _f32(0.1 * float(extent)), _f32(0.8 * 2))
    return _C.densify_plan(xyz_gradient_accum.detach(), denom.detach(), scaling.detach(), opacity.detach(),
                           None if max_radii2D is None else max_radii2D.detach(), rule, raw, big)


def densify_tensors(plan: torch.Tensor, tensors, roles=None, exp_avgs=None, exp_avg_sqs=None, noise: Optional[torch.Tensor] = None, *,
                    split_shrink: float = 1.6, raw: bool = True):
    tensors = [t.detach() for t in tensors]
    n = len(tensors)
    roles = [0] * n if roles is None else [_C.DENSIFY_ROLES[r] if isinstance(r, str) else int(r) for r in roles]
    exp_avgs = [None] * n if exp_avgs is None else [None if m is None else m.detach() for m in exp_avgs]
    exp_avg_sqs = [None] * n if exp_avg_sqs is None else [None if v is None else v.detach() for v in exp_avg_sqs]
    offsets, counts = _C.densify_scan(plan)
    if noise is None and counts[2] > 0:
        noise = torch.randn(2 * counts[2], 3, device=plan.device, dtype=torch.float32)
    new_t, new_m, new_v = _C.densify_apply(plan, offsets, counts, tensors, roles, exp_avgs, exp_avg_sqs, noise, split_shrink, raw)
    return new_t, new_m, new_v, counts


def densify_and_prune(optimizer, plan: torch.Tensor, *, noise: Optional[torch.Tensor] = None, split_shrink: float = 1.6, raw: bool = True,
                      names=("xyz", "scaling", "rotation")):
    role_of = dict(zip(names, ("xyz", "scaling", "rotation")))
    groups = list(optimizer.param_groups)
    params, roles, ms, vs = [], [], [], []
    for group in groups:
        if len(group["params"]) != 1 or "name" not in group:
            raise ValueError("densify_and_prune: every group must hold one tensor and carry a \"name\"")
        p = group["params"][0]
        state = optimizer.state.get(p, {})
        params.append(p)
        roles.append(role_of.get(group["name"], "plain"))
        ms.append(state.get("exp_avg"))
        vs.append(state.get("exp_avg_sq"))
    new_t, new_m, new_v, _ = densify_tensors(plan, params, roles, ms, vs, noise, split_shrink=split_shrink, raw=raw)
    out = {}
    for group, old, t, m, v in zip(groups, params, new_t, new_m, new_v):
        new = torch.nn.Parameter(t.requires_grad_(old.requires_grad))
        state = optimizer.state.pop(old, None)
        if state is not None and len(state) > 0:
            if m is not None:
                state["exp_avg"], state["exp_avg_sq"] = m, v
            optimizer.state[new] = state
        group["params"][0] = new
        out[group["name"]] = new
    return out
```

Baseline: 458.0.

## Zero gradient records on side stream during forward render instead of in backward

The per-Gaussian gradient record buffer (P×16 floats) is now allocated in the forward pass and cleared by a vectorized zero-fill kernel on a side stream that overlaps the render kernel. The buffer is handed to backward, which skips its own torch::zeros. This moves a large memset off the backward critical path and hides it behind rendering. In exchange it adds cross-call plumbing, keeps the buffer alive between forward and backward, and the fill may compete with render for memory bandwidth.

```diff
diff --git a/include/stp_raster.h b/include/stp_raster.h
--- a/include/stp_raster.h
+++ b/include/stp_raster.h
@@ -113,6 +113,9 @@
 
 void stp_set_forward_sh_stash(int enable);
 
+void stp_set_forward_zero_fill(void* buffer, size_t bytes);
+int stp_forward_zero_filled(void);
+
 void stp_set_forward_raw_params(int mask);
 void stp_set_backward_raw_params(int mask);
 int stp_activate_params(int P, const float* scaling, const float* rotation, const float* opacity, float* scales, float* rotations,
diff --git a/stopthepop-rasterization_amd/csrc/host/stp_bind_raster.h b/stopthepop-rasterization_amd/csrc/host/stp_bind_raster.h
--- a/stopthepop-rasterization_amd/csrc/host/stp_bind_raster.h
+++ b/stopthepop-rasterization_amd/csrc/host/stp_bind_raster.h
@@ -60,7 +60,7 @@
     return (int)sh.size(1) + 1;
 }
 
-std::tuple<int, torch::Tensor, torch::Tensor, torch::Tensor, torch::Tensor, torch::Tensor, torch::Tensor, torch::Tensor>
+std::tuple<int, torch::Tensor, torch::Tensor, torch::Tensor, torch::Tensor, torch::Tensor, torch::Tensor, torch::Tensor, torch::Tensor>
 rasterize_gaussians(const torch::Tensor& background, const torch::Tensor& means3D, const torch::Tensor& colors, const torch::Tensor& opacity,
                     const torch::Tensor& scales, const torch::Tensor& rotations, const float scale_modifier, const torch::Tensor& cov3D_precomp,
                     const torch::Tensor& viewmatrix, const torch::Tensor& projmatrix, const torch::Tensor& inv_viewprojmatrix, const float tan_fovx,
@@ -93,6 +93,10 @@
     if (invdepth) out_invdepth = zero ? torch::zeros({1, H, W}, fopt) : torch::empty({1, H, W}, fopt);
     const bool sh_stash = (setting_flag(settings, "_record_blend_log") || setting_flag(settings, "_sh_stash")) && !setting_flag(settings, "_no_sh_stash") &&
                           !render_depth && g_api.set_forward_sh_stash != nullptr;
+    const bool prefill = sh_stash && P != 0 && setting_flag(settings, "_prefill_records") && g_api.set_forward_zero_fill != nullptr &&
+                         g_api.forward_zero_filled != nullptr;
+    torch::Tensor records;
+    if (prefill) records = torch::empty({P, STP_GRAD_RECORD_FLOATS}, fopt);
     Resizer geom{torch::empty({0}, bopt), false, false, 0}, binning{torch::empty({0}, bopt), true, false, 1}, img{torch::empty({0}, bopt), true, false, 2};
     int rendered = 0;
     if (P != 0) {
@@ -117,17 +121,19 @@
             if (split) g_api.set_forward_split_sh(dc_.data_ptr<float>());
             if (sh_stash) g_api.set_forward_sh_stash(1);
             if (raw != 0) g_api.set_forward_raw_params(raw);
+            if (prefill) g_api.set_forward_zero_fill(records.data_ptr(), (size_t)records.numel() * sizeof(float));
             rc = g_api.forward(&Resizer::call, &geom, &Resizer::call, &binning, &Resizer::call, &img, P, degree, M, fptr(in.bg), W, H, &s, fptr(in.m3),
                                fptr(in.sh), fptr(in.col), fptr(in.op), fptr(in.sc), scale_modifier, fptr(in.ro), fptr(in.c3), fptr(in.vm), fptr(in.pm),
                                fptr(in.inv), fptr(in.cam), tan_fovx, tan_fovy, prefiltered ? 1 : 0, out_color.data_ptr<float>(), radii.data_ptr<int>(),
                                debug ? 1 : 0, stream);
+            if (prefill && !(rc >= 0 && g_api.forward_zero_filled())) records = torch::Tensor();
         }
         rendered = checked(rc);
         remember_storage(geom.t);
         remember_storage(binning.t);
         remember_storage(img.t);
     }
-    return std::make_tuple(rendered, out_color, radii, geom.t, binning.t, img.t, out_alpha, out_invdepth);
+    return std::make_tuple(rendered, out_color, radii, geom.t, binning.t, img.t, out_alpha, out_invdepth, records);
 }
 
 std::vector<torch::Tensor>
@@ -141,7 +147,7 @@
                              const c10::optional<std::vector<torch::Tensor>>& outputs, const bool camera_grads, const bool absgrad, const bool blend_stats,
                              const c10::optional<torch::Tensor>& dL_dalpha, const bool bg_grad,
                              const c10::optional<torch::Tensor>& dL_dinvdepth, const c10::optional<torch::Tensor>& invdepth,
-                             const c10::optional<torch::Tensor>& dc, const int raw_mask)
+                             const c10::optional<torch::Tensor>& dc, const int raw_mask, const c10::optional<torch::Tensor>& prefilled)
 {
     need_library();
     TORCH_CHECK(means3D.is_cuda(), GPU_ONLY);
@@ -183,7 +189,10 @@
     const int M = split ? M_split : sh.numel() != 0 ? (int)sh.size(1) : 0;
     const auto fopt = means3D.options().dtype(torch::kFloat32);
     const int rec_floats = (phases & 4) ? STP_GRAD_RECORD_USED : STP_GRAD_RECORD_FLOATS;
-    const torch::Tensor records = partial.has_value() ? *partial : torch::zeros({P, rec_floats}, fopt);
+    const bool use_prefilled = !partial.has_value() && prefilled.has_value() && prefilled->defined();
+    if (use_prefilled)
+        TORCH_CHECK((phases & ~8) == 3 && prefilled->device() == dev,"prefilled records serve one whole backward on padded records (phases = 3) on the forward's device");
+    const torch::Tensor records = partial.has_value() ? *partial : use_prefilled ? *prefilled : torch::zeros({P, rec_floats}, fopt);
     TORCH_CHECK(records.dim() == 2 && records.size(0) == P && records.size(1) == rec_floats && records.scalar_type() == torch::kFloat32 &&
                     records.is_contiguous(), "partial must be a contiguous float32 (P,", rec_floats, ") tensor");
     torch::Tensor dL_dmeans2D, dL_dcolors, dL_dopacity, dL_dmeans3D, dL_dcov3D, dL_dsh, dL_dscales, dL_drotations, dL_ddc;
diff --git a/stopthepop-rasterization_amd/csrc/host/stp_exports.h b/stopthepop-rasterization_amd/csrc/host/stp_exports.h
--- a/stopthepop-rasterization_amd/csrc/host/stp_exports.h
+++ b/stopthepop-rasterization_amd/csrc/host/stp_exports.h
@@ -32,6 +32,8 @@
     X(set_backward_raw_params, false, "raw parameter inputs")                              \
     X(activate_params, false, "raw parameter inputs")                                      \
     X(set_forward_sh_stash, false, "the SH stash")  \
+    X(set_forward_zero_fill, false, "the gradient records cleared during the forward")     \
+    X(forward_zero_filled, false, "the gradient records cleared during the forward")       \
     X(sparse_adam, false, "the sparse Adam step")                                          \
     X(mcmc_relocation, false, "the 3DGS-MCMC kernels")                                     \
     X(mcmc_add_noise, false, "the 3DGS-MCMC kernels")                                      \
diff --git a/stopthepop-rasterization_amd/csrc/stp_api.hip b/stopthepop-rasterization_amd/csrc/stp_api.hip
--- a/stopthepop-rasterization_amd/csrc/stp_api.hip
+++ b/stopthepop-rasterization_amd/csrc/stp_api.hip
@@ -104,6 +104,7 @@
 void stp_set_forward_sh_stash(int enable) { t_pending.forward.sh_stash = enable != 0; }
 void stp_set_backward_split_sh(const float* dc, float* dL_ddc) { t_pending.backward.split_sh = dc ? BackwardSplitSh{dc, dL_ddc} : BackwardSplitSh{}; }
 void stp_set_forward_raw_params(int mask) { t_pending.forward.raw_params = mask; }
+void stp_set_forward_zero_fill(void* buffer, size_t bytes) { t_pending.forward.zero_fill = buffer && bytes ? ForwardZeroFill{buffer, bytes} : ForwardZeroFill{}; }
 void stp_set_backward_raw_params(int mask) { t_pending.backward.raw_params = mask; }
 
 namespace {
diff --git a/stopthepop-rasterization_amd/csrc/stp_forward.hip b/stopthepop-rasterization_amd/csrc/stp_forward.hip
--- a/stopthepop-rasterization_amd/csrc/stp_forward.hip
+++ b/stopthepop-rasterization_amd/csrc/stp_forward.hip
@@ -100,6 +100,8 @@
     return 0;
 }
 
+thread_local bool t_zero_filled = false;
+
 struct ForwardCall {
     const hipStream_t st; const int debug;
     FrameParams f;
@@ -109,6 +111,7 @@
     uint32_t* log_need_word = nullptr; uint32_t log_tag = 0; int log_depth = 0; bool with_log = false;
     SideStream* side = nullptr;
     bool colour_started = true;
+    ForwardZeroFill zero_fill;
     char* bin_ptr = nullptr; size_t bin_have = 0;
     uint32_t cap = 0; bool ahead = false, run_ahead = false;
     int* radii; float* const out_color;
@@ -290,6 +293,18 @@
     STP_DEBUG_SYNC("entry gather");
     STP_TRY(ordering.join(), "join tile order");
     timer_mark(3, st);
+    SideJoin filling{mb.done, st, false};
+    if (zero_fill.ptr && side && !t_zero_filled) {
+        STP_TRY(hipEventRecord(mb.ev, st), "record event in front of the render");
+        STP_TRY(hipStreamWaitEvent(side->stream, mb.ev, 0), "side stream wait (render)");
+        STP_TRY(launch_zero_fill(zero_fill.ptr, zero_fill.bytes, side->stream), "zero fill launch");
+        if (hipError_t e2 = hipEventRecord(mb.done, side->stream); e2 != hipSuccess) {
+            (void)hipStreamSynchronize(side->stream);
+            return fail_hip(e2, "record zero-fill event");
+        }
+        filling.pending = true;
+        t_zero_filled = true;
+    }
     std::string err;
     hipError_t e;
     if (split.s.armed && split.s.row > f.ty0 && split.s.row < f.ty1 && f.s.debug_visualization == 0) {
@@ -304,6 +319,7 @@
         if (!err.empty()) return fail(STP_ERR_QUEUE_SIZE, err);
         return fail_hip(e, "render launch");
     }
+    STP_TRY(filling.join(), "join zero fill");
     STP_DEBUG_SYNC("render");
     STP_TRY(launch_render_debug_finish(f, img, out_color, st), "debug visualisation");
     timer_mark(4, st);
@@ -315,6 +331,7 @@
 
 void stp_set_run_ahead(int mode) { g_run_ahead.store(mode < 0 ? 0 : (mode > 2 ? 2 : mode), std::memory_order_relaxed); }
 int stp_get_run_ahead(void) { return g_run_ahead.load(std::memory_order_relaxed); }
+int stp_forward_zero_filled(void) { return t_zero_filled ? 1 : 0; }
 void stp_reset_size_guesses(void)
 {
     for (auto& dev : g_guess)
@@ -339,6 +356,8 @@
 {
     const ForwardRequests req = take_forward_requests();
     ForwardCall c((hipStream_t)stream, debug, req.split, radii, out_color);
+    t_zero_filled = false;
+    if ((reinterpret_cast<uintptr_t>(req.zero_fill.ptr) & 15u) == 0 && req.zero_fill.bytes % 16 == 0) c.zero_fill = req.zero_fill;
     const ForwardBackground& fbg = req.background;
     if (!settings || !geometry_alloc || !binning_alloc || !image_alloc) return fail(STP_ERR_INVALID_ARGUMENT, "null settings or allocator");
     if (P < 0 || width <= 0 || height <= 0) return fail(STP_ERR_INVALID_ARGUMENT, "bad sizes");
diff --git a/stopthepop-rasterization_amd/csrc/stp_internal.h b/stopthepop-rasterization_amd/csrc/stp_internal.h
--- a/stopthepop-rasterization_amd/csrc/stp_internal.h
+++ b/stopthepop-rasterization_amd/csrc/stp_internal.h
@@ -208,7 +208,8 @@
 
 struct ForwardSplit { int row = 0; hipEvent_t event = nullptr; bool armed = false; };
 struct ForwardBackground { const float* bg_image = nullptr; float* out_alpha = nullptr; };
-struct ForwardRequests { ForwardSplit split; ForwardBackground background; float* out_invdepth = nullptr;  const float* sh_dc = nullptr;  bool sh_stash = false;  int raw_params = 0;  };
+struct ForwardZeroFill { void* ptr = nullptr; size_t bytes = 0; };
+struct ForwardRequests { ForwardSplit split; ForwardBackground background; float* out_invdepth = nullptr;  const float* sh_dc = nullptr;  bool sh_stash = false;  int raw_params = 0;  ForwardZeroFill zero_fill; };
 ForwardRequests take_forward_requests();
 int check_raw_params(int mask, const float* opacities, const float* scales, const float* rotations);
 
@@ -222,6 +223,7 @@
 hipError_t launch_tile_order(const FrameParams& f, const ImageState& img, hipStream_t st);
 hipError_t launch_sh_color(const FrameParams& f, const GeometryState& g, const int* radii, float* sh_stash, hipStream_t st);
 hipError_t launch_stash_mark(const FrameParams& f, const GeometryState& g, float* sh_stash, hipStream_t st);
+hipError_t launch_zero_fill(void* ptr, size_t bytes, hipStream_t st);
 hipError_t launch_mailbox(const uint32_t* last_offset, const uint32_t* status, uint32_t* mailbox_dev, uint32_t ticket, uint32_t* log_need, hipStream_t st);
 hipError_t launch_block_prefix_mailbox(const FrameParams& f, const GeometryState& g, uint32_t* mailbox_dev, uint32_t ticket, uint32_t* log_need, hipStream_t st);
 hipError_t launch_duplicate(const FrameParams& f, const GeometryState& g, const int* radii, const BinningState& b, uint32_t* tile_cursor, uint32_t cap, uint32_t header_cap, uint32_t* zero_ptr, size_t zero_words, hipStream_t st);
diff --git a/stopthepop-rasterization_amd/csrc/stp_preprocess.hip b/stopthepop-rasterization_amd/csrc/stp_preprocess.hip
--- a/stopthepop-rasterization_amd/csrc/stp_preprocess.hip
+++ b/stopthepop-rasterization_amd/csrc/stp_preprocess.hip
@@ -778,6 +778,28 @@
     return hipGetLastError();
 }
 
+constexpr int FILL_UNROLL = 8;
+__global__ void __launch_bounds__(256) zero_fill_kernel(float4* __restrict__ p, size_t n16)
+{
+    const size_t stride = (size_t)gridDim.x * 256;
+    size_t i = (size_t)blockIdx.x * 256 + threadIdx.x;
+    const float4 z = make_float4(0.0f, 0.0f, 0.0f, 0.0f);
+    for (; i + (FILL_UNROLL - 1) * stride < n16; i += FILL_UNROLL * stride) {
+#pragma unroll
+        for (int u = 0; u < FILL_UNROLL; u++) p[i + u * stride] = z;
+    }
+    for (; i < n16; i += stride) p[i] = z;
+}
+
+hipError_t launch_zero_fill(void* ptr, size_t bytes, hipStream_t st)
+{
+    const size_t n16 = bytes / 16;
+    if (n16 == 0) return hipSuccess;
+    const size_t want = (n16 + 256 * FILL_UNROLL - 1) / (256 * FILL_UNROLL);
+    hipLaunchKernelGGL(zero_fill_kernel, dim3((unsigned)(want < 2048 ? want : 2048)), dim3(256), 0, st, static_cast<float4*>(ptr), n16);
+    return hipGetLastError();
+}
+
 hipError_t launch_ranges(const FrameParams& f, const BinningState& b, const ImageState& img, int R, hipStream_t st)
 {
     const size_t T = (size_t)f.gx * f.gy;
diff --git a/stopthepop-rasterization_amd/diff_gaussian_rasterization/_C.py b/stopthepop-rasterization_amd/diff_gaussian_rasterization/_C.py
--- a/stopthepop-rasterization_amd/diff_gaussian_rasterization/_C.py
+++ b/stopthepop-rasterization_amd/diff_gaussian_rasterization/_C.py
@@ -36,6 +36,8 @@
     "stp_set_forward_split_sh": ([ctypes.c_void_p], None, "split SH inputs"),
     "stp_set_backward_split_sh": ([ctypes.c_void_p] * 2, None, "split SH inputs"),
     "stp_set_forward_sh_stash": ([ctypes.c_int], None, "the SH stash"),
+    "stp_set_forward_zero_fill": ([ctypes.c_void_p, ctypes.c_size_t], None, "the gradient records cleared during the forward"),
+    "stp_forward_zero_filled": ([], ctypes.c_int, "the gradient records cleared during the forward"),
     "stp_set_forward_raw_params": ([ctypes.c_int], None, "raw parameter inputs"),
     "stp_set_backward_raw_params": ([ctypes.c_int], None, "raw parameter inputs"),
     "stp_activate_params": ([ctypes.c_int] + [ctypes.c_void_p] * 7, ctypes.c_int, "raw parameter inputs"),
@@ -300,7 +302,7 @@
 def rasterize_gaussians(background, means3D, colors, opacity, scales, rotations, scale_modifier, cov3D_precomp,
                         viewmatrix, projmatrix, inv_viewprojmatrix, tan_fovx, tan_fovy, image_height, image_width,
                         sh, degree, campos, prefiltered, settings_dict, render_depth, debug, alpha=False, invdepth=False,
-                        raw=0, dc=None) -> Tuple[int, torch.Tensor, torch.Tensor, torch.Tensor, torch.Tensor, torch.Tensor]:
+                        records=False, raw=0, dc=None) -> Tuple[int, torch.Tensor, torch.Tensor, torch.Tensor, torch.Tensor, torch.Tensor]:
     if means3D.dim() != 2 or means3D.size(1) != 3:
         raise RuntimeError("means3D must have dimensions (num_points, 3)")
     if alpha or _per_pixel_background(background, image_height, image_width):
@@ -317,7 +319,7 @@
         background, means3D, colors, opacity, scales, rotations, scale_modifier, cov3D_precomp, viewmatrix, projmatrix,
         inv_viewprojmatrix, tan_fovx, tan_fovy, int(image_height), int(image_width), sh, int(degree), campos, bool(prefiltered),
         settings_dict, bool(render_depth), bool(debug), _records_log(settings_dict), bool(alpha), bool(invdepth), dc, int(raw))
-    return tuple(out[:6]) + ((out[6],) if alpha else ()) + ((out[7],) if invdepth else ())
+    return tuple(out[:6]) + ((out[6],) if alpha else ()) + ((out[7],) if invdepth else ()) + ((out[8],) if records else ())
 
 
 def _per_pixel_background(background, height, width) -> bool:
@@ -329,7 +331,7 @@
                                  pixel_colors, dL_dout_color, sh, degree, campos, geomBuffer, R, binningBuffer,
                                  imageBuffer, settings_dict, debug, phases=3, partial=None, chunk=None, outputs=None,
                                  camera_grads=False, absgrad=False, blend_stats=False, dL_dalpha=None, bg_grad=False,
-                                 dL_dinvdepth=None, invdepth=None, raw=0, dc=None):
+                                 dL_dinvdepth=None, invdepth=None, prefilled=None, raw=0, dc=None):
     if chunk is not None:
         k, K = int(chunk[0]), int(chunk[1])
         if not (0 <= k < K <= 255) or (int(phases) & 1):
@@ -353,7 +355,7 @@
         background, means3D, radii, opacities, colors, scales, rotations, scale_modifier, cov3D_precomp, viewmatrix, projmatrix,
         inv_viewprojmatrix, tan_fovx, tan_fovy, pixel_colors, dL_dout_color, sh, int(degree), campos, geomBuffer, int(R), binningBuffer,
         imageBuffer, settings_dict, bool(debug), _records_log(settings_dict), int(phases), partial, None if outputs is None else list(outputs),
-        bool(camera_grads), bool(absgrad), bool(blend_stats), dL_dalpha, bool(bg_grad), dL_dinvdepth, invdepth, dc, int(raw))
+        bool(camera_grads), bool(absgrad), bool(blend_stats), dL_dalpha, bool(bg_grad), dL_dinvdepth, invdepth, dc, int(raw), prefilled)
     return out[0] if (int(phases) & 3) == 1 and not bg_grad else tuple(out)
 
 
diff --git a/stopthepop-rasterization_amd/diff_gaussian_rasterization/__init__.py b/stopthepop-rasterization_amd/diff_gaussian_rasterization/__init__.py
--- a/stopthepop-rasterization_amd/diff_gaussian_rasterization/__init__.py
+++ b/stopthepop-rasterization_amd/diff_gaussian_rasterization/__init__.py
@@ -77,6 +77,7 @@
         else:
             sdict["_backward_mode"] = "resort"
         sdict["_sh_stash"] = True
+        sdict.setdefault("_prefill_records", True)
     if colors_precomp.numel() == 0:
         sdict["_no_grad_colors"] = True
     if cov3Ds_precomp.numel() == 0:
@@ -96,6 +97,9 @@
     ctx.raw = int(getattr(rs, "raw_mask", 0))
     if ctx.raw:
         kw["raw"] = ctx.raw
+    prefill = bool(sdict.get("_prefill_records")) and bool(sdict.get("_sh_stash"))
+    if prefill:
+        kw["records"] = True
     if rs.debug:
         cpu_args = cpu_deep_copy_tuple(args + ((dc,) if "dc" in kw else ()) + ((ctx.raw,) if ctx.raw else ()))
         try:
@@ -107,6 +111,7 @@
     else:
         num_rendered, color, radii, geomBuffer, binningBuffer, imgBuffer, *extra = _C.rasterize_gaussians(*args, **kw)
 
+    ctx.prefilled_records = extra.pop() if prefill else None
     if ctx.log_lease is not None:
         ctx.log_lease.resize(_C.blend_log_bytes(rs.image_width, rs.image_height, depth=_C.blend_log_depth(imgBuffer)))
     ctx.raster_settings = rs
@@ -164,6 +169,9 @@
         kw["dc"] = dc
     if ctx.raw:
         kw["raw"] = ctx.raw
+    records, ctx.prefilled_records = getattr(ctx, "prefilled_records", None), None
+    if records is not None:
+        kw["prefilled"] = records
     if rs.debug:
         cpu_args = cpu_deep_copy_tuple(args + ((dc,) if dc is not None else ()) + ((ctx.raw,) if ctx.raw else ()))
         try:
@@ -348,7 +356,8 @@
                 **({"_absgrad": True} if getattr(self, "_absgrad", False) else {}),
                 **({"_blend_stats": True} if getattr(self, "_blend_stats", False) else {}),
                 **({"_alpha": True} if getattr(self, "_alpha", False) else {}),
-                **({"_invdepth": True} if getattr(self, "_invdepth", False) else {})}
+                **({"_invdepth": True} if getattr(self, "_invdepth", False) else {}),
+                **({"_prefill_records": False} if getattr(self, "_prefill_records", True) is False else {})}
 
     def to_json(self):
         return json.dumps(self.to_dict())
```

New measurement: 454.8. About the same (-0.7%).
